# ssi-research/FQSS

Hardware: AMD Instinct MI355X
Metric: QAT-step samples/sec + SI-SDR, ConvTasNet 2spk 8kHz W8A8 (higher is better)
Workload: dtype f32; 1 GPU; ConvTasNet 2spk 8 kHz W8A8 QAT step (cfg 2), batch 8 x 4 s per GPU, quantizing phase; global_batch=8, segment_samples=32000, parallelism=dp1, optimizer=adam lr 1e-3 + clip 5.0

## Files before the change

fqss_amd/csrc/fqss_dev.h:

```cpp
#pragma once
#include <hip/hip_runtime.h>
#include <stdint.h>

#include "fqss.h"

namespace fqss {

void set_error(const char* fmt, ...);
int launch_status(const char* what);

#define FQSS_REQUIRE(cond, msg)                          \
    do {                                                 \
        if (!(cond)) {                                   \
            ::fqss::set_error("%s: %s", __func__, msg);  \
            return FQSS_EINVAL;                          \
        }                                                \
    } while (0)

static inline bool aligned16(const void* p) { return (reinterpret_cast<uintptr_t>(p) & 15u) == 0; }
static inline int64_t cdiv(int64_t a, int64_t b) { return (a + b - 1) / b; }

static inline dim3 grid_rows(int64_t rows, int64_t cols, int vec, int64_t max_blocks = 8192) {
    int64_t gx = cdiv(cols, 256 * (int64_t)vec);
    if (gx < 1) gx = 1;
    if (gx > 1024) gx = 1024;
    int64_t gy = max_blocks / gx;
    if (gy < 1) gy = 1;
    if (gy > rows) gy = rows;
    if (gy > 65535) gy = 65535;
    if (gy < 1) gy = 1;
    return dim3((unsigned)gx, (unsigned)gy, 1);
}

constexpr int kXcds = 8;
static inline unsigned xcd_grid(int64_t groups, int64_t per_group) { return (unsigned)(cdiv(groups, kXcds) * kXcds * per_group); }

bool qdgrad_ring_ok(int Ci, int Co1, int Co2);
int qdgrad_ring(const char* who, const float* gz1, const float* gz2, const int8_t* wiT, const float* dw, const float* addend, float* gx, int B,
                int Ci, int Co1, int Co2, int M, int64_t ld_gz1, int64_t ld_gz2, int64_t ld_add, int64_t ld_gx, fqss_stream_t stream);

#if defined(__HIPCC__)
__device__ __forceinline__ bool xcd_tile(int groups, int per_group, int& group, int& idx) {
    const int L = blockIdx.x, xcd = L % kXcds, slot = L / kXcds;
    idx = slot % per_group;
    group = (slot / per_group) * kXcds + xcd;
    return group < groups;
}

constexpr int kWave = 64;

__device__ __forceinline__ uint32_t f2ord(float f) {
    uint32_t u = __float_as_uint(f);
    return (u & 0x80000000u) ? ~u : (u | 0x80000000u);
}
__device__ __forceinline__ float ord2f(uint32_t k) {
    uint32_t u = (k & 0x80000000u) ? (k & 0x7fffffffu) : ~k;
    return __uint_as_float(u);
}

template <int CTRL, int ROW_MASK>
__device__ __forceinline__ int dpp_i32(int v) { return __builtin_amdgcn_update_dpp(0, v, CTRL, ROW_MASK, 0xf, false); }
template <int CTRL, int ROW_MASK = 0xf, typename T>
__device__ __forceinline__ T dpp_get(T v) {
    static_assert(sizeof(T) == 4 || sizeof(T) == 8, "32- or 64-bit values");
    if constexpr (sizeof(T) == 4) {
        return __builtin_bit_cast(T, dpp_i32<CTRL, ROW_MASK>(__builtin_bit_cast(int, v)));
    } else {
        const unsigned long long b = __builtin_bit_cast(unsigned long long, v);
        const unsigned lo = (unsigned)dpp_i32<CTRL, ROW_MASK>((int)(unsigned)b), hi = (unsigned)dpp_i32<CTRL, ROW_MASK>((int)(unsigned)(b >> 32));
        return __builtin_bit_cast(T, ((unsigned long long)hi << 32) | lo);
    }
}
template <typename T>
__device__ __forceinline__ T wave_sum63(T v) {
#ifdef FQSS_NO_DPP_SUMS
#pragma unroll
    for (int o = 32; o > 0; o >>= 1) v += __shfl_xor(v, o, 64);
    return v;
#else
    v += dpp_get<0xB1>(v);
    v += dpp_get<0x4E>(v);
    v += dpp_get<0x141>(v);
    v += dpp_get<0x140>(v);
    v += dpp_get<0x142, 0xa>(v);
    v += dpp_get<0x143, 0xc>(v);
    return v;
#endif
}

template <typename T>
__device__ __forceinline__ T from_lane63(T v) {
    static_assert(sizeof(T) == 4 || sizeof(T) == 8, "32- or 64-bit values");
    if constexpr (sizeof(T) == 4) {
        return __builtin_bit_cast(T, __builtin_amdgcn_readlane(__builtin_bit_cast(int, v), 63));
    } else {
        const unsigned long long b = __builtin_bit_cast(unsigned long long, v);
        const unsigned lo = (unsigned)__builtin_amdgcn_readlane((int)(unsigned)b, 63), hi = (unsigned)__builtin_amdgcn_readlane((int)(unsigned)(b >> 32), 63);
        return __builtin_bit_cast(T, ((unsigned long long)hi << 32) | lo);
    }
}
template <typename T>
__device__ __forceinline__ T wave_sum(T v) {
    return from_lane63(wave_sum63(v));
}
template <int CTRL, int ROW_MASK>
__device__ __forceinline__ float dpp_keep(float v) {
    const int i = __float_as_int(v);
    return __int_as_float(__builtin_amdgcn_update_dpp(i, i, CTRL, ROW_MASK, 0xf, false));
}
__device__ __forceinline__ float wave_min(float v) {
    v = fminf(v, dpp_get<0xB1>(v)); v = fminf(v, dpp_get<0x4E>(v)); v = fminf(v, dpp_get<0x141>(v)); v = fminf(v, dpp_get<0x140>(v));
    v = fminf(v, dpp_keep<0x142, 0xa>(v)); v = fminf(v, dpp_keep<0x143, 0xc>(v));
    return from_lane63(v);
}
__device__ __forceinline__ float wave_max(float v) {
    v = fmaxf(v, dpp_get<0xB1>(v)); v = fmaxf(v, dpp_get<0x4E>(v)); v = fmaxf(v, dpp_get<0x141>(v)); v = fmaxf(v, dpp_get<0x140>(v));
    v = fmaxf(v, dpp_keep<0x142, 0xa>(v)); v = fmaxf(v, dpp_keep<0x143, 0xc>(v));
    return from_lane63(v);
}
template <typename T>
__device__ __forceinline__ T row16_sum(T v) {
    v += dpp_get<0xB1>(v);
    v += dpp_get<0x4E>(v);
    v += dpp_get<0x141>(v);
    v += dpp_get<0x140>(v);
    return v;
}

template <typename T, int N>
__device__ __forceinline__ void block_sum(T (&v)[N], T* smem) {
    const int lane = threadIdx.x & 63, w = threadIdx.x >> 6, nw = blockDim.x >> 6;
#pragma unroll
    for (int i = 0; i < N; ++i) v[i] = wave_sum63(v[i]);
    if (lane == 63) {
#pragma unroll
        for (int i = 0; i < N; ++i) smem[i * nw + w] = v[i];
    }
    __syncthreads();
    if (threadIdx.x == 0) {
#pragma unroll
        for (int i = 0; i < N; ++i) {
            T s = smem[i * nw];
            for (int k = 1; k < nw; ++k) s += smem[i * nw + k];
            v[i] = s;
        }
    }
    __syncthreads();
}

template <int N>
__device__ __forceinline__ void block_sum_f32w(const float (&p)[N], float* smem, double (&out)[N]) {
    const int lane = threadIdx.x & 63, w = threadIdx.x >> 6, nw = blockDim.x >> 6;
#pragma unroll
    for (int i = 0; i < N; ++i) {
        const float s = wave_sum63(p[i]);
        if (lane == 63) smem[i * nw + w] = s;
    }
    __syncthreads();
    if (threadIdx.x == 0) {
#pragma unroll
        for (int i = 0; i < N; ++i) {
            double s = (double)smem[i * nw];
            for (int k = 1; k < nw; ++k) s += (double)smem[i * nw + k];
            out[i] = s;
        }
    }
    __syncthreads();
}

struct QRange {
    float lo, delta, inv;
};
__device__ __forceinline__ QRange load_qrange(const float* qmin, const float* qmax) {
    const float lo = *qmin, hi = *qmax;
    QRange r;
    r.lo = lo;
    r.delta = (hi - lo) / 255.0f;
    r.inv = 1.0f / r.delta;
    return r;
}
__device__ __forceinline__ float div_by(float a, float b, float y) {
    const float q = a * y;
    const float r = fmaf(-b, q, a);
    return fmaf(r, y, q);
}
__device__ __forceinline__ float wq_levels(int n_bits) { return (float)((1 << n_bits) - 1); }
__device__ __forceinline__ float wq_qlo(int n_bits) { return -(float)(1 << (n_bits - 1)); }
__device__ __forceinline__ float wq_qhi(int n_bits) { return (float)((1 << (n_bits - 1)) - 1); }
template <typename T>
__device__ __forceinline__ T sgpr(T v) {
    asm("" : "+s"(v));
    return v;
}
__device__ __forceinline__ void store16(float* p, const float4& v) {
    typedef float f32x4s __attribute__((ext_vector_type(4)));
    const f32x4s t = {v.x, v.y, v.z, v.w};
    asm volatile("global_store_dwordx4 %0, %1, off\n\ts_nop 1" : : "v"(p), "v"(t) : "memory");
}
__device__ __forceinline__ float act_neg_scale(int act, float slope) {
    return act == FQSS_ACT_PRELU ? slope : (act == FQSS_ACT_RELU ? 0.0f : 1.0f);
}
__device__ __forceinline__ float act_apply(float z, int act, float slope) {
// ... 83 lines not shown
```

fqss_amd/csrc/multi.hip:

```cpp
#include "fqss_dev.h"

namespace fqss {

constexpr int kSlotsM = FQSS_GACC_SLOTS;
constexpr int kWqFields = FQSS_WQ_DESC_WORDS;

__global__ __launch_bounds__(256) void k_gacc_flush_multi(const long long* __restrict__ table) {
    __shared__ double red[3 * 4];
    const long long* t = table + 4 * (int64_t)blockIdx.x;
    double* gacc = reinterpret_cast<double*>(t[0]);
    float* gmin = reinterpret_cast<float*>(t[1]);
    float* gmax = reinterpret_cast<float*>(t[2]);
    float* gslope = reinterpret_cast<float*>(t[3]);
    double v[3] = {0.0, 0.0, 0.0};
    for (int i = threadIdx.x; i < kSlotsM; i += 256) {
#pragma unroll
        for (int k = 0; k < 3; ++k) {
            const double x = gacc[3 * i + k];
            if (x != 0.0) {
                v[k] += x;
                gacc[3 * i + k] = 0.0;
            }
        }
    }
    block_sum<double, 3>(v, red);
    if (threadIdx.x == 0) {
        if (gmin) *gmin += (float)v[0];
        if (gmax) *gmax += (float)v[1];
        if (gslope) *gslope += (float)v[2];
    }
}

__device__ __forceinline__ const long long* find_desc(const long long* table, int n, int blk) {
    int lo = 0, hi = n - 1;
    while (lo < hi) {
        const int mid = (lo + hi + 1) >> 1;
        if ((int)table[(int64_t)mid * kWqFields + 15] <= blk) lo = mid; else hi = mid - 1;
    }
    return table + (int64_t)lo * kWqFields;
}

__global__ __launch_bounds__(256) void k_wq_multi_fwd(const long long* __restrict__ table, int n) {
    __shared__ float red[4];
    const long long* d = find_desc(table, n, blockIdx.x);
    const float* w = reinterpret_cast<const float*>(d[0]);
    float* wq = reinterpret_cast<float*>(d[1]);
    signed char* idx = reinterpret_cast<signed char*>(d[2]);
    signed char* idxT = reinterpret_cast<signed char*>(d[3]);
    float* dw = reinterpret_cast<float*>(d[4]);
    float* rw = reinterpret_cast<float*>(d[5]);
    const float* qmin = reinterpret_cast<const float*>(d[6]);
    const float* qmax = reinterpret_cast<const float*>(d[7]);
    const int outer = (int)d[12], C = (int)d[13], inner = (int)d[14];
    const int c = blockIdx.x - (int)d[15];
    const int64_t ldT = d[16];
    const int n_bits = (int)d[17];
    const float L = wq_levels(n_bits), qlo = wq_qlo(n_bits), qhi = wq_qhi(n_bits);
    const float a = fmaxf(fabsf(qmin[c]), fabsf(qmax[c]));
    const float delta = (2.0f * a) / L;
    const float inv = 1.0f / delta;
    float s = 0.0f;
    const int nel = outer * inner;
    for (int e = threadIdx.x; e < nel; e += 256) {
        const int o = e / inner, i = e - o * inner;
        const int64_t k = ((int64_t)o * C + c) * inner + i;
        const float X = rintf(div_by(w[k], delta, inv));
        const float q = __builtin_amdgcn_fmed3f(X, qlo, qhi);
        wq[k] = delta * q;
        if (idx) {
            idx[(int64_t)c * nel + e] = (signed char)q;
            idxT[(int64_t)e * ldT + c] = (signed char)q;
            s += q;
        }
    }
    if (idx) {
        float v[1] = {s};
        block_sum<float, 1>(v, red);
        if (threadIdx.x == 0) {
            dw[c] = delta;
            rw[c] = v[0];
        }
    }
}

__global__ __launch_bounds__(256) void k_wq_multi_bwd(const long long* __restrict__ table, int n) {
    __shared__ double red[4];
    const long long* d = find_desc(table, n, blockIdx.x);
    const float* w = reinterpret_cast<const float*>(d[0]);
    const float* qmin = reinterpret_cast<const float*>(d[6]);
    const float* qmax = reinterpret_cast<const float*>(d[7]);
    const float* gwq = reinterpret_cast<const float*>(d[8]);
    float* gw = reinterpret_cast<float*>(d[9]);
    float* gmin = reinterpret_cast<float*>(d[10]);
    float* gmax = reinterpret_cast<float*>(d[11]);
    const int outer = (int)d[12], C = (int)d[13], inner = (int)d[14];
    const int c = blockIdx.x - (int)d[15];
    const int n_bits = (int)d[17];
    const float L = wq_levels(n_bits), qlo = wq_qlo(n_bits), qhi = wq_qhi(n_bits);
    const float lo = qmin[c], hi = qmax[c];
    const float a = fmaxf(fabsf(lo), fabsf(hi));
    const float delta = (2.0f * a) / L;
    const float inv = 1.0f / delta;
    float p = 0.0f;
    const int nel = outer * inner;
    for (int e = threadIdx.x; e < nel; e += 256) {
        const int o = e / inner, i = e - o * inner;
        const int64_t k = ((int64_t)o * C + c) * inner + i;
        const float u = div_by(w[k], delta, inv);
        const float X = rintf(u);
        const bool inr = (X >= qlo) && (X <= qhi);
        const float q = __builtin_amdgcn_fmed3f(X, qlo, qhi);
        const float gk = gwq[k];
        gw[k] += inr ? div_by(gk * delta, delta, inv) : 0.0f;
        p += gk * (inr ? (q - u) : q);
    }
    double v[1] = {(double)p};
    block_sum<double, 1>(v, red);
    if (threadIdx.x == 0) {
        const double D = v[0] * (2.0 / (double)L);
        const float al = fabsf(lo), ah = fabsf(hi);
        const double wl = al > ah ? 1.0 : (al == ah ? 0.5 : 0.0);
        const double wh = ah > al ? 1.0 : (al == ah ? 0.5 : 0.0);
        const double sl = lo > 0.0f ? 1.0 : (lo < 0.0f ? -1.0 : 0.0);
        const double sh = hi > 0.0f ? 1.0 : (hi < 0.0f ? -1.0 : 0.0);
        gmin[c] += (float)(D * wl * sl);
        gmax[c] += (float)(D * wh * sh);
    }
}

}

using namespace fqss;

extern "C" int fqss_gacc_flush_multi(const int64_t* table, int n, fqss_stream_t stream) {
    FQSS_REQUIRE(table && n >= 0, "bad args");
    if (n == 0) return FQSS_OK;
    hipLaunchKernelGGL(k_gacc_flush_multi, dim3((unsigned)n), dim3(256), 0, (hipStream_t)stream, (const long long*)table);
    return launch_status("fqss_gacc_flush_multi");
}

extern "C" int fqss_wq_table_check(const int64_t* host_table, int n) {
    FQSS_REQUIRE(n >= 0 && (host_table || n == 0), "bad args");
    for (int i = 0; i < n; ++i) {
        const int64_t* d = host_table + (int64_t)i * kWqFields;
        FQSS_REQUIRE(d[17] >= FQSS_WQ_MIN_BITS && d[17] <= FQSS_WQ_MAX_BITS, "descriptor word 17: weight width outside 2..8 bits");
        FQSS_REQUIRE(d[12] > 0 && d[13] > 0 && d[14] > 0, "descriptor words 12-14: empty weight");
    }
    return FQSS_OK;
}

extern "C" int fqss_wq_multi_fwd(const int64_t* table, int n, int total_channels, fqss_stream_t stream) {
    FQSS_REQUIRE(table && n >= 0 && total_channels >= 0, "bad args");
    if (n == 0 || total_channels == 0) return FQSS_OK;
    hipLaunchKernelGGL(k_wq_multi_fwd, dim3((unsigned)total_channels), dim3(256), 0, (hipStream_t)stream,
                       (const long long*)table, n);
    return launch_status("fqss_wq_multi_fwd");
}

extern "C" int fqss_wq_multi_bwd(const int64_t* table, int n, int total_channels, fqss_stream_t stream) {
    FQSS_REQUIRE(table && n >= 0 && total_channels >= 0, "bad args");
    if (n == 0 || total_channels == 0) return FQSS_OK;
    hipLaunchKernelGGL(k_wq_multi_bwd, dim3((unsigned)total_channels), dim3(256), 0, (hipStream_t)stream,
                       (const long long*)table, n);
    return launch_status("fqss_wq_multi_bwd");
}
```

fqss_amd/csrc/qgemm.hip:

```cpp
#include <cstdlib>
#include <type_traits>

#define FQSS_USES_GRAD_ADD
#include "fqss_dev.h"

namespace fqss {

typedef float f32x16 __attribute__((ext_vector_type(16)));
typedef __bf16 bf16x8 __attribute__((ext_vector_type(8)));
typedef short s16x4 __attribute__((ext_vector_type(4)));
typedef short s16x8 __attribute__((ext_vector_type(8)));

constexpr int QBM = 128, QBN = 64, QBK = 32;
constexpr int LDK = 40;
constexpr int LDN = 96;
constexpr int LDT = 36;
constexpr int WGRAD_BLOCKS = 256;

__device__ __forceinline__ unsigned short f2bf_trunc(float f) { return (unsigned short)(__float_as_uint(f) >> 16); }
__device__ __forceinline__ float bf_trunc(float f) { return __uint_as_float(__float_as_uint(f) & 0xFFFF0000u); }
__device__ __forceinline__ unsigned int bf_rne_word(float f) {
    const unsigned int u = __float_as_uint(f);
    return u + 0x7FFFu + ((u >> 16) & 1u);
}

__device__ __forceinline__ void split3(float g, unsigned short& b1, unsigned short& b2, unsigned short& b3) {
    const float h1 = bf_trunc(g);
    const float r1 = g - h1;
    const float h2 = bf_trunc(r1);
    const float r2 = r1 - h2;
    b1 = f2bf_trunc(h1);
    b2 = f2bf_trunc(h2);
    b3 = f2bf_trunc(r2);
}

typedef float f32x4 __attribute__((ext_vector_type(4)));
typedef uint32_t u32x4 __attribute__((ext_vector_type(4)));
typedef uint32_t u32x2 __attribute__((ext_vector_type(2)));
struct QStage {
    f32x4 a[4];
    f32x4 b[2];
    u32x2 bq;
    int kch;
};
__device__ __forceinline__ void q_load16(f32x4& d, const void* p) { asm volatile("global_load_dwordx4 %0, %1, off" : "=v"(d) : "v"(p) : "memory"); }
__device__ __forceinline__ void q_load8(u32x2& d, const void* p) { asm volatile("global_load_dwordx2 %0, %1, off" : "=v"(d) : "v"(p) : "memory"); }
template <int MODE, int N>
__device__ __forceinline__ void q_wait(QStage& st) {
    if constexpr (MODE == 0)
        asm volatile("s_waitcnt vmcnt(%2)" : "+v"(st.a[0]), "+v"(st.bq) : "n"(N) : "memory");
    else if constexpr (MODE == 1)
        asm volatile("s_waitcnt vmcnt(%3)" : "+v"(st.a[0]), "+v"(st.b[0]), "+v"(st.b[1]) : "n"(N) : "memory");
    else
        asm volatile("s_waitcnt vmcnt(%6)"
                     : "+v"(st.a[0]), "+v"(st.a[1]), "+v"(st.a[2]), "+v"(st.a[3]), "+v"(st.b[0]), "+v"(st.b[1])
                     : "n"(N)
                     : "memory");
}

__device__ __forceinline__ float dec(unsigned int c, const QRange& r) { return r.delta * (float)c + r.lo; }

struct QGemmArgs {
    const void* A;
    const void* B;
    float* C;
    int M, N, K;
    int64_t lda, ldb, ldc;
    int64_t sAb, sBb, sCb;
    const float* dw;
    const float* rw;
    const float* bias;
    const float* qmin_x;
    const float* qmax_x;
    int ksplit, kchunk;
    int tiles_m, tiles_n, batches;
    int M1;
    float* C2; int64_t ldc2, sC2b;
    const float* bias2;
    const void* A2; int64_t lda2, sA2b;
    int K1;
    const void* B2; int64_t ldb2, sB2b;
    unsigned char* Q1; unsigned char* Q2; int64_t ldq1, ldq2, sQ1b, sQ2b;
    const float *qy_min1, *qy_max1, *qy_min2, *qy_max2;
    int qact; const float* qslope;
    long long* stats;
    const unsigned char* AD1; const unsigned char* AD2; int64_t ldad1, ldad2;
    unsigned char* S1; unsigned char* S2; int64_t lds1, lds2;
    const float *ad_min1, *ad_max1, *ad_min2, *ad_max2;
    const float *s_min1, *s_max1, *s_min2, *s_max2;
    int imp_taps, imp_kw, imp_base, imp_row_step, imp_col_step, imp_cmax;
    float imp_inv_taps, imp_inv_kw;
};

template <int MODE, int GP = 3, bool IMP = false>
__global__ __launch_bounds__(256, 2) void k_qgemm(QGemmArgs g) {
    static_assert(!IMP || MODE == 1 || MODE == 3 || MODE == 4, "implicit convolution: float B operands");
    static_assert(MODE == 0 || MODE == 1 || MODE == 3 || MODE == 4, "unknown q-GEMM mode");
    static_assert(GP == 3 || (GP == 2 && MODE != 0 && MODE != 4), "two gradient pieces: dgrad only");
    constexpr bool ACODES = MODE < 2 || MODE == 4;
    constexpr int WMODE = MODE == 4 ? 1 : MODE;
    constexpr bool SIX = MODE == 3 && GP == 2;
    constexpr int NA = (MODE == 3) ? 3 : 1;
    constexpr int NB = (MODE == 1) ? GP : (MODE == 3 || MODE == 4) ? 3 : 1;
    constexpr int BROWS = QBK, BLD = LDN;
    constexpr int A_BYTES = NA * QBM * LDK * 2, B_BYTES = NB * BROWS * BLD * 2;
    constexpr int T_BYTES = 4 * 32 * LDT * 4;
    constexpr int SMEM = (A_BYTES + B_BYTES > T_BYTES) ? A_BYTES + B_BYTES : T_BYTES;
    __shared__ __attribute__((aligned(16))) unsigned char smem[SMEM];
    typedef unsigned short (*AsT)[QBM][LDK];
    typedef unsigned short (*BsT)[BROWS][BLD];
    AsT As = reinterpret_cast<AsT>(smem);
    BsT Bs = reinterpret_cast<BsT>(smem + A_BYTES);

    const int tid = threadIdx.x, lane = tid & 63;
    const int wave = __builtin_amdgcn_readfirstlane(tid >> 6);
    const int wm = wave >> 1, wn = wave & 1;
    const int lr = lane & 31, lh = lane >> 5;
    int panel, mt;
    if (!xcd_tile(g.tiles_n * g.batches, g.tiles_m, panel, mt)) return;
    const int b = panel / g.tiles_n;
    const int kbeg = 0, kend = g.K;
    const int i0 = mt * QBM, j0 = (panel % g.tiles_n) * QBN;

    f32x16 acc[2];
#pragma unroll
    for (int mi = 0; mi < 2; ++mi)
#pragma unroll
        for (int r = 0; r < 16; ++r) acc[mi][r] = 0.f;

    __shared__ float rowc[3][QBM];
    if constexpr (MODE == 0 || MODE == 3 || MODE == 4) {
        if (tid < QBM) {
            const int row = i0 + tid;
            const bool ok = row < g.M;
            rowc[0][tid] = ((MODE == 0 || MODE == 4) && ok) ? g.dw[row] : 1.0f;
            rowc[1][tid] = (MODE == 0 && ok) ? g.rw[row] : 0.0f;
            rowc[2][tid] = (ok && g.bias != nullptr) ? (row < g.M1 ? g.bias[row] : g.bias2[row - g.M1]) : 0.0f;
        }
    }

    constexpr int NLOADS = (MODE == 0) ? 2 : (WMODE == 1) ? 3 : 6;
    const int a_row = tid >> 1, a_k = (tid & 1) * 16;
    const int bk_row = tid >> 3, bk_n = (tid & 7) * 8;
    const int a_row_c = min(i0 + a_row, g.M - 1);

    __shared__ float dws[(MODE == 1) ? 1024 : 1];
    if constexpr (MODE == 1) {
        for (int k = tid; k < (IMP ? g.K / g.imp_taps : g.K); k += 256) dws[k] = g.dw[k];
    }

    constexpr int BEL = (MODE == 0) ? 1 : 4;
    const char* const gB1 = sgpr((const char*)g.B + (int64_t)b * g.sBb * BEL);
    const char* const gB2 = (MODE == 0) ? gB1 : sgpr((const char*)g.B2 + (int64_t)b * g.sB2b * BEL);
    const int64_t gldb1 = sgpr(g.ldb), gldb2 = (MODE == 0) ? gldb1 : sgpr(g.ldb2);
    auto load_tiles = [&](QStage& st, int k0) {
        if constexpr (ACODES) {
            q_load16(st.a[0], (const signed char*)g.A + (int64_t)a_row_c * g.lda + min(k0 + a_k, g.K - 16));
        } else {
            const float* A = (const float*)g.A + (int64_t)b * g.sAb + (int64_t)a_row_c * g.lda;
#pragma unroll
            for (int q = 0; q < 4; ++q) q_load16(st.a[q], A + min(k0 + a_k + 4 * q, g.K - 4));
        }
        const int kk = min(k0 + bk_row, g.K - 1);
        if constexpr (IMP) {
            int ci = (int)((float)kk * g.imp_inv_taps);
            int t = kk - ci * g.imp_taps;
            if (t < 0) { ci -= 1; t += g.imp_taps; }
            if (t >= g.imp_taps) { ci += 1; t -= g.imp_taps; }
            int th = (int)((float)t * g.imp_inv_kw);
            int tw = t - th * g.imp_kw;
            if (tw < 0) { th -= 1; tw += g.imp_kw; }
            if (tw >= g.imp_kw) { th += 1; tw -= g.imp_kw; }
            st.kch = ci;
            const float* Bp = (const float*)gB1 + (int64_t)ci * gldb1 + (g.imp_base + th * g.imp_row_step + tw * g.imp_col_step);
            const int c0 = min(j0 + bk_n, g.imp_cmax);
            q_load16(st.b[0], Bp + c0);
            q_load16(st.b[1], Bp + c0 + 4);
        } else if constexpr (MODE == 0) {
            const unsigned char* Bp = (const unsigned char*)gB1 + (int64_t)kk * gldb1;
            q_load8(st.bq, Bp + min(j0 + bk_n, (int)gldb1 - 8));
        } else {
            const bool h1 = kk < g.K1;
            const int ldk = (int)(h1 ? gldb1 : gldb2);
            const float* Bp = (const float*)(h1 ? gB1 : gB2) + (int64_t)(h1 ? kk : kk - g.K1) * ldk;
            q_load16(st.b[0], Bp + min(j0 + bk_n, ldk - 4));
            q_load16(st.b[1], Bp + min(j0 + bk_n + 4, ldk - 4));
        }
    };

    auto store_codes = [&](unsigned short* dst, const unsigned int* w, auto nw_tag, bool is_signed, bool zero) {
        constexpr int NW = decltype(nw_tag)::value;
        unsigned int o[2 * NW];
#pragma unroll
        for (int q = 0; q < NW; ++q) {
            float f[4];
#pragma unroll
            for (int e = 0; e < 4; ++e) {
                const unsigned int byte = (w[q] >> (8 * e)) & 0xFFu;
                f[e] = zero ? 0.0f : (is_signed ? (float)(int)(signed char)byte : (float)byte);
            }
            o[2 * q] = __builtin_amdgcn_perm(__float_as_uint(f[1]), __float_as_uint(f[0]), 0x07060302u);
            o[2 * q + 1] = __builtin_amdgcn_perm(__float_as_uint(f[3]), __float_as_uint(f[2]), 0x07060302u);
        }
#pragma unroll
        for (int h = 0; h < NW / 2; ++h)
            *reinterpret_cast<uint4*>(dst + 8 * h) = make_uint4(o[4 * h], o[4 * h + 1], o[4 * h + 2], o[4 * h + 3]);
    };

    auto store_split3 = [&](unsigned short* d1, unsigned short* d2, unsigned short* d3, const f32x4* v, float scale,
                            bool do_scale, bool zero, auto nq_tag) {
        constexpr int NQ = decltype(nq_tag)::value;
        unsigned int o1[2 * NQ], o2[2 * NQ], o3[2 * NQ];
#pragma unroll
        for (int q = 0; q < NQ; ++q) {
            float h0[4], r1[4], r2[4];
#pragma unroll
            for (int e = 0; e < 4; ++e) {
                float t = do_scale ? scale * v[q][e] : v[q][e];
                if (zero) t = 0.0f;
                h0[e] = t;
                r1[e] = t - bf_trunc(t);
                r2[e] = r1[e] - bf_trunc(r1[e]);
            }
#pragma unroll
            for (int e = 0; e < 2; ++e) {
                o1[2 * q + e] = __builtin_amdgcn_perm(__float_as_uint(h0[2 * e + 1]), __float_as_uint(h0[2 * e]), 0x07060302u);
                o2[2 * q + e] = __builtin_amdgcn_perm(__float_as_uint(r1[2 * e + 1]), __float_as_uint(r1[2 * e]), 0x07060302u);
                o3[2 * q + e] = __builtin_amdgcn_perm(__float_as_uint(r2[2 * e + 1]), __float_as_uint(r2[2 * e]), 0x07060302u);
            }
        }
#pragma unroll
        for (int h = 0; h < NQ / 2; ++h) {
            *reinterpret_cast<uint4*>(d1 + 8 * h) = make_uint4(o1[4 * h], o1[4 * h + 1], o1[4 * h + 2], o1[4 * h + 3]);
            *reinterpret_cast<uint4*>(d2 + 8 * h) = make_uint4(o2[4 * h], o2[4 * h + 1], o2[4 * h + 2], o2[4 * h + 3]);
            *reinterpret_cast<uint4*>(d3 + 8 * h) = make_uint4(o3[4 * h], o3[4 * h + 1], o3[4 * h + 2], o3[4 * h + 3]);
        }
    };

    auto store_split2 = [&](unsigned short* d1, unsigned short* d2, const f32x4* v, float scale, bool zero) {
        unsigned int o1[4], o2[4];
#pragma unroll
        for (int q = 0; q < 2; ++q) {
            float h0[4];
            unsigned int r1[4];
#pragma unroll
            for (int e = 0; e < 4; ++e) {
                float t = scale * v[q][e];
                if (zero) t = 0.0f;
                h0[e] = t;
                r1[e] = bf_rne_word(t - bf_trunc(t));
            }
#pragma unroll
            for (int e = 0; e < 2; ++e) {
                o1[2 * q + e] = __builtin_amdgcn_perm(__float_as_uint(h0[2 * e + 1]), __float_as_uint(h0[2 * e]), 0x07060302u);
                o2[2 * q + e] = __builtin_amdgcn_perm(r1[2 * e + 1], r1[2 * e], 0x07060302u);
            }
        }
        *reinterpret_cast<uint4*>(d1) = make_uint4(o1[0], o1[1], o1[2], o1[3]);
        *reinterpret_cast<uint4*>(d2) = make_uint4(o2[0], o2[1], o2[2], o2[3]);
    };

    auto store_tiles = [&](QStage& st, int k0) {
        q_wait<WMODE, NLOADS>(st);
        const bool kz = (k0 + bk_row) >= g.K;
        if constexpr (ACODES) {
            const unsigned int w[4] = {__float_as_uint(st.a[0][0]), __float_as_uint(st.a[0][1]), __float_as_uint(st.a[0][2]),
                                       __float_as_uint(st.a[0][3])};
            store_codes(&As[0][a_row][a_k], w, std::integral_constant<int, 4>{}, true, false);
        } else {
            store_split3(&As[0][a_row][a_k], &As[1][a_row][a_k], &As[2][a_row][a_k], st.a, 1.0f, false, false,
                         std::integral_constant<int, 4>{});
        }
        if constexpr (MODE == 0) {
            const unsigned int w[2] = {st.bq[0], st.bq[1]};
            store_codes(&Bs[0][bk_row][bk_n], w, std::integral_constant<int, 2>{}, false, kz);
        } else {
            const float sc = (MODE == 1) ? dws[IMP ? st.kch : min(k0 + bk_row, g.K - 1)] : 1.0f;
            if constexpr (NB == 2)
                store_split2(&Bs[0][bk_row][bk_n], &Bs[1][bk_row][bk_n], st.b, sc, kz);
            else
                store_split3(&Bs[0][bk_row][bk_n], &Bs[1][bk_row][bk_n], &Bs[2][bk_row][bk_n], st.b, sc, MODE == 1, kz,
                             std::integral_constant<int, 2>{});
        }
    };

    const int nkt = (kend - kbeg + QBK - 1) / QBK;
    const int gq = lane >> 4, li = lane & 15, tq = li >> 2, tp = li & 3;
    auto compute_tile = [&]() {
#pragma unroll
        for (int ks = 0; ks < 2; ++ks) {
#pragma unroll
            for (int sp = 0; sp < NA * NB; ++sp) {
                const int ia = (NA == 3) ? 2 - (sp / NB) : 0, ib = (NB > 1) ? NB - 1 - (sp % NB) : 0;
                if (SIX && ia + ib >= 3) continue;
                bf16x8 af[2], bfr;
#pragma unroll
                for (int mi = 0; mi < 2; ++mi)
                    af[mi] = *reinterpret_cast<const bf16x8*>(&As[ia][wm * 64 + mi * 32 + lr][ks * 16 + 8 * lh]);
                {
                    const int kr = ks * 16 + 8 * (gq >> 1) + tq;
                    const int nc = wn * 32 + 16 * (gq & 1) + 4 * tp;
                    union { bf16x8 v; s16x4 h[2]; } u;
                    u.h[0] = __builtin_amdgcn_ds_read_tr16_b64_v4i16(
                        (s16x4 __attribute__((address_space(3)))*)(&Bs[ib][kr][nc]));
                    u.h[1] = __builtin_amdgcn_ds_read_tr16_b64_v4i16(
                        (s16x4 __attribute__((address_space(3)))*)(&Bs[ib][kr + 4][nc]));
                    bfr = u.v;
                }
#pragma unroll
                for (int mi = 0; mi < 2; ++mi)
                    acc[mi] = __builtin_amdgcn_mfma_f32_32x32x16_bf16(af[mi], bfr, acc[mi], 0, 0, 0);
            }
        }
    };
    QStage stA, stB;
    __syncthreads();
    load_tiles(stA, 0);
    load_tiles(stB, QBK);
    store_tiles(stA, 0);
    load_tiles(stA, 2 * QBK);
    __syncthreads();
    for (int kt = 0; kt < nkt; kt += 2) {
        compute_tile();
        __syncthreads();
        if (kt + 1 < nkt) {
            store_tiles(stB, (kt + 1) * QBK);
            load_tiles(stB, (kt + 3) * QBK);
            __syncthreads();
            compute_tile();
            __syncthreads();
            if (kt + 2 < nkt) {
                store_tiles(stA, (kt + 2) * QBK);
                load_tiles(stA, (kt + 4) * QBK);
                __syncthreads();
            }
        }
    }
    q_wait<WMODE, 0>(stA);
    q_wait<WMODE, 0>(stB);

    float dx = 0.f, mnx = 0.f;
    if constexpr (MODE == 0) {
        const float lo = *g.qmin_x, hi = *g.qmax_x;
        dx = (hi - lo) / 255.0f;
        mnx = lo;
    }
    float* Cb = g.C + (int64_t)b * g.sCb;
    float* C2b = (g.C2 != nullptr) ? g.C2 + (int64_t)b * g.sC2b : nullptr;
    __shared__ uint32_t Qt[(MODE == 0) ? 4 : 1][32][8];
    const bool quant = (MODE == 0) && g.Q1 != nullptr;
    unsigned int st_s = 0, st_ss = 0;
    QRange ry1{}, ry2{};
    QRange rad1{}, rad2{}, rs1{}, rs2{};
    float qslope = 0.0f;
    if (quant) {
        ry1 = load_qrange(g.qy_min1, g.qy_max1);
        ry2 = (g.Q2 != nullptr) ? load_qrange(g.qy_min2, g.qy_max2) : ry1;
        qslope = (g.qact == FQSS_ACT_PRELU) ? *g.qslope : 0.0f;
        if (g.S1 != nullptr) { rad1 = load_qrange(g.ad_min1, g.ad_max1); rs1 = load_qrange(g.s_min1, g.s_max1); }
        if (g.S2 != nullptr) { rad2 = load_qrange(g.ad_min2, g.ad_max2); rs2 = load_qrange(g.s_min2, g.s_max2); }
    }
    {
        __syncthreads();
        float(*Tt)[LDT] = reinterpret_cast<float(*)[LDT]>(smem + wave * 32 * LDT * 4);
        const bool has_bias = g.bias != nullptr;
        const float qns = act_neg_scale(g.qact, qslope);
        const int c4 = (lane & 7) * 4;
        const int col = j0 + wn * 32 + c4;
        auto tile_epilogue = [&](int mi, auto PER_ROW) {
            const int rowt = i0 + wm * 64 + mi * 32;
            const bool tfirst = rowt < g.M1;
            uint4 ad16 = make_uint4(0u, 0u, 0u, 0u);
            const unsigned char* const adp = (MODE == 0 && quant) ? (tfirst ? g.AD1 : g.AD2) : nullptr;
            if constexpr (MODE == 0) {
                if (adp != nullptr) {
                    const int64_t ldad = tfirst ? g.ldad1 : g.ldad2;
                    const int orow = rowt + (lane >> 1) - (tfirst ? 0 : g.M1), ocol = j0 + wn * 32 + 16 * (lane & 1);
                    const int rows_o = tfirst ? g.M1 : g.M - g.M1;
                    if (rowt + (lane >> 1) < g.M && ocol < ldad)
                        ad16 = *reinterpret_cast<const uint4*>(adp + ((int64_t)b * rows_o + orow) * ldad + ocol);
                }
            }
#pragma unroll
            for (int r = 0; r < 16; ++r) {
                const int rl = (r & 3) + 8 * (r >> 2) + 4 * lh;
                const int rb = wm * 64 + mi * 32 + rl;
                const float S = acc[mi][r];
                float v = S;
                if constexpr (MODE == 0) {
                    v = rowc[0][rb] * (dx * S + mnx * rowc[1][rb]);
                    if (has_bias) v = v + rowc[2][rb];
                } else if constexpr (MODE == 3) {
                    if (has_bias) v = S + rowc[2][rb];
                } else if constexpr (MODE == 4) {
                    v = rowc[0][rb] * S;
                    if (has_bias) v = v + rowc[2][rb];
                }
                Tt[rl][lr] = v;
            }
            const QRange ry = tfirst ? ry1 : ry2;
#pragma unroll
            for (int pass = 0; pass < 4; ++pass) {
                const int rl = pass * 8 + (lane >> 3);
                const int row = rowt + rl;
                float4 t = *reinterpret_cast<const float4*>(&Tt[rl][c4]);
                if constexpr (MODE == 1) {
                    if (C2b != nullptr && row < g.M && col < g.N) {
                        const float4 r = *reinterpret_cast<const float4*>(C2b + (int64_t)row * g.ldc2 + col);
                        t.x += r.x; t.y += r.y; t.z += r.z; t.w += r.w;
                    }
                }
                if (row < g.M && col < g.N) {
                    const bool first = decltype(PER_ROW)::value ? row < g.M1 : tfirst;
                    const int64_t ldc = first ? g.ldc : g.ldc2;
                    float* dst = (first ? Cb + (int64_t)row * ldc : C2b + (int64_t)(row - g.M1) * ldc) + col;
                    if (col + 3 < g.N || col + 3 < ldc) {
                        store16(dst, t);
                    } else {
                        dst[0] = t.x;
                        if (col + 1 < g.N) dst[1] = t.y;
                        if (col + 2 < g.N) dst[2] = t.z;
                    }
                }
                if constexpr (MODE == 0) {
                    if (quant) {
                        const float tv[4] = {t.x, t.y, t.z, t.w};
                        uint32_t pk = 0;
#pragma unroll
                        for (int e = 0; e < 4; ++e) pk = pack_code(fq_code(tv[e] > 0.0f ? tv[e] : qns * tv[e], ry), e, pk);
                        Qt[wave][rl][lane & 7] = pk;
                        if (g.stats != nullptr) {
                            const int nl = g.N - col;
                            const uint32_t live = (row < g.M && nl > 0) ? (nl >= 4 ? 0xFFFFFFFFu : (0xFFFFFFFFu >> (8 * (4 - nl)))) : 0u;
                            code_stats4(pk & live, st_s, st_ss);
                        }
                    }
                }
            }
            if constexpr (MODE == 0) {
                if (quant) {
                    const int rl = lane >> 1, hf = lane & 1;
                    const int qcol = j0 + wn * 32 + 16 * hf;
                    const uint4 c16 = *reinterpret_cast<const uint4*>(&Qt[wave][rl][4 * hf]);
                    const int64_t ldq = tfirst ? g.ldq1 : g.ldq2;
                    if (rowt + rl < g.M && qcol < ldq) {
                        unsigned char* qb = tfirst ? g.Q1 + (int64_t)b * g.sQ1b + (int64_t)(rowt + rl) * ldq
                                                   : g.Q2 + (int64_t)b * g.sQ2b + (int64_t)(rowt + rl - g.M1) * ldq;
                        *reinterpret_cast<uint4*>(qb + qcol) = c16;
                    }
                    if (adp != nullptr) {
                        const QRange ra = tfirst ? rad1 : rad2, rs = tfirst ? rs1 : rs2;
                        const unsigned int wa[4] = {ad16.x, ad16.y, ad16.z, ad16.w}, wy[4] = {c16.x, c16.y, c16.z, c16.w};
                        unsigned int o[4];
#pragma unroll
                        for (int w4 = 0; w4 < 4; ++w4) {
                            unsigned int pk = 0;
#pragma unroll
                            for (int e = 0; e < 4; ++e) {
                                float z = dec((wa[w4] >> (8 * e)) & 255u, ra);
                                z = z + 1.0f * dec((wy[w4] >> (8 * e)) & 255u, ry);
                                pk = pack_code(fq_code(z, rs), e, pk);
                            }
                            o[w4] = pk;
                        }
                        const int64_t lds_ = tfirst ? g.lds1 : g.lds2;
                        const int rows_o = tfirst ? g.M1 : g.M - g.M1;
                        if (rowt + rl < g.M && qcol < lds_) {
                            unsigned char* sb_ = (tfirst ? g.S1 : g.S2) + ((int64_t)b * rows_o + (rowt + rl - (tfirst ? 0 : g.M1))) * lds_;
                            *reinterpret_cast<uint4*>(sb_ + qcol) = make_uint4(o[0], o[1], o[2], o[3]);
                        }
                    }
                }
            }
        };
        if (MODE != 0 || (g.M1 & 31) == 0 || g.M1 >= g.M) {
#pragma unroll
            for (int mi = 0; mi < 2; ++mi) tile_epilogue(mi, std::false_type{});
        } else {
#pragma unroll
            for (int mi = 0; mi < 2; ++mi) tile_epilogue(mi, std::true_type{});
        }
        if constexpr (MODE == 0) {
            if (quant && g.stats != nullptr) {
                __shared__ unsigned int sst[2][4];
                st_s = wave_sum(st_s);
                st_ss = wave_sum(st_ss);
                if (lane == 0) { sst[0][wave] = st_s; sst[1][wave] = st_ss; }
                __syncthreads();
                if (tid == 0) {
                    long long* slot = g.stats + 2 * (((int64_t)b * g.tiles_m + mt) * g.tiles_n + (panel % g.tiles_n));
                    slot[0] = (long long)sst[0][0] + sst[0][1] + sst[0][2] + sst[0][3];
                    slot[1] = (long long)sst[1][0] + sst[1][1] + sst[1][2] + sst[1][3];
// ... 281 lines not shown
                const uint32_t w = st.b[f][q];
                const float f0 = (float)(w & 0xFFu), f1 = (float)((w >> 8) & 0xFFu);
                const float f2 = (float)((w >> 16) & 0xFFu), f3 = (float)(w >> 24);
                o[2 * q] = __builtin_amdgcn_perm(__float_as_uint(f1), __float_as_uint(f0), 0x07060302u);
                o[2 * q + 1] = __builtin_amdgcn_perm(__float_as_uint(f3), __float_as_uint(f2), 0x07060302u);
            }
            *reinterpret_cast<uint4*>(&Bs[buf][br + 128 * f][bc]) = make_uint4(o[0], o[1], o[2], o[3]);
            *reinterpret_cast<uint4*>(&Bs[buf][br + 128 * f][bc + 8]) = make_uint4(o[4], o[5], o[6], o[7]);
        }
        ++cr;
        ck += W2_TK;
        if (ck >= spb * W2_TK) ck = 0;
    };
    f32x16 acc[NBF];
#pragma unroll
    for (int f = 0; f < NBF; ++f)
#pragma unroll
        for (int r = 0; r < 16; ++r) acc[f][r] = 0.f;
    auto compute = [&](int buf) {
#pragma unroll
        for (int ks = 0; ks < W2_TK / 16; ++ks) {
            const int kk = ks * 16 + 8 * lh;
            bf16x8 bfr[NBF];
#pragma unroll
            for (int f = 0; f < NBF; ++f) bfr[f] = *reinterpret_cast<const bf16x8*>(&Bs[buf][wc * (32 * NBF) + 32 * f + lr][kk]);
            bf16x8 af[GP];
#pragma unroll
            for (int p = 0; p < GP; ++p) af[p] = *reinterpret_cast<const bf16x8*>(&As[buf][p][wr * 32 + lr][kk]);
#pragma unroll
            for (int p = GP - 1; p >= 0; --p)
#pragma unroll
                for (int f = 0; f < NBF; ++f) acc[f] = __builtin_amdgcn_mfma_f32_32x32x16_bf16(af[p], bfr[f], acc[f], 0, 0, 0);
        }
    };
    Stage st[W2_RING];
#pragma unroll
    for (int i = 0; i < W2_RING; ++i) load(st[i]);
    wait_oldest(st[0]);
    convert_store(st[0], 0);
    load(st[0]);
    __syncthreads();
    for (int s = 0; s < n; s += W2_RING) {
#pragma unroll
        for (int i = 0; i < W2_RING; ++i) {
            Stage& nx = st[(i + 1) % W2_RING];
            if (first_half) compute(i & 1);
            wait_oldest(nx);
            convert_store(nx, (i + 1) & 1);
            load(nx);
            if (!first_half) compute(i & 1);
            __syncthreads();
        }
    }
#pragma unroll
    for (int i = 0; i < W2_RING; ++i) wait_all(st[i]);
#pragma unroll
    for (int i = 0; i < 2; ++i) {
        float v = rs_part[i];
#pragma unroll
        for (int o = 8; o > 0; o >>= 1) v += __shfl_xor(v, o, 64);
        if ((tid & 15) == 0) rsum[ar + 32 * i] = v;
    }
    __syncthreads();
    const float lo = *J.qmin, hi = *J.qmax;
    const float dx = (hi - lo) / 255.0f, mnx = lo;
    constexpr int NV = 16 * NBF;
    float v[NV];
#pragma unroll
    for (int f = 0; f < NBF; ++f)
#pragma unroll
        for (int r = 0; r < 16; ++r) v[16 * f + r] = dx * acc[f][r] + mnx * rsum[wr * 32 + (r & 3) + 8 * (r >> 2) + 4 * lh];
    bool finish = nparts == 1;
    constexpr int SLOT = W2_TM * TN;
    if (!finish) {
        float* sl = ga.slabs + ((int64_t)(J.tile0 + tile) * ga.slots + part) * WGR_SLOT_FLOATS;
#pragma unroll
        for (int q = 0; q < NV / 4; ++q) st16_sc1(sl + ((int64_t)q * 512 + tid) * 4, f32x4{v[4 * q], v[4 * q + 1], v[4 * q + 2], v[4 * q + 3]});
        asm volatile("s_waitcnt vmcnt(0)" ::: "memory");
        __syncthreads();
        if (tid == 0) *ticket_s = __hip_atomic_fetch_add(&ga.tickets[J.tile0 + tile], 1u, __ATOMIC_RELAXED, __HIP_MEMORY_SCOPE_AGENT);
        __syncthreads();
        finish = *ticket_s == (unsigned)(nparts - 1);
        if (finish) {
            const float* s0p = ga.slabs + (int64_t)(J.tile0 + tile) * ga.slots * WGR_SLOT_FLOATS;
#pragma unroll
            for (int r = 0; r < NV; ++r) v[r] = 0.0f;
            for (int p = 0; p < nparts; ++p) {
#pragma unroll
                for (int h = 0; h < NBF; ++h) {
                    f32x4 t[4];
#pragma unroll
                    for (int q = 0; q < 4; ++q) ld16_sc1(t[q], s0p + (int64_t)p * WGR_SLOT_FLOATS + ((int64_t)(4 * h + q) * 512 + tid) * 4);
                    asm volatile("s_waitcnt vmcnt(0)" : "+v"(t[0]), "+v"(t[1]), "+v"(t[2]), "+v"(t[3]) : : "memory");
#pragma unroll
                    for (int q = 0; q < 4; ++q)
#pragma unroll
                        for (int e = 0; e < 4; ++e) v[16 * h + 4 * q + e] += t[q][e];
                }
            }
            if (tid == 0) __hip_atomic_store(&ga.tickets[J.tile0 + tile], 0u, __ATOMIC_RELAXED, __HIP_MEMORY_SCOPE_AGENT);
        }
    }
    static_assert(SLOT <= WGR_SLOT_FLOATS, "slab slots are sized for the wide tile");
    if (finish) {
        const int Mr = J.M, Nc = J.N;
        float* const Cp = J.C;
        float old[NV];
#pragma unroll
        for (int f = 0; f < NBF; ++f)
#pragma unroll
            for (int r = 0; r < 16; ++r) {
                const int row = row0 + wr * 32 + (r & 3) + 8 * (r >> 2) + 4 * lh, col = col0 + wc * (32 * NBF) + 32 * f + lr;
                old[16 * f + r] = (row < Mr && col < Nc) ? Cp[(int64_t)row * Nc + col] : 0.0f;
            }
#pragma unroll
        for (int f = 0; f < NBF; ++f)
#pragma unroll
            for (int r = 0; r < 16; ++r) {
                const int row = row0 + wr * 32 + (r & 3) + 8 * (r >> 2) + 4 * lh, col = col0 + wc * (32 * NBF) + 32 * f + lr;
                if (row < Mr && col < Nc) Cp[(int64_t)row * Nc + col] = old[16 * f + r] + v[16 * f + r];
            }
        asm volatile("s_waitcnt vmcnt(0)" ::: "memory");
    }
    __syncthreads();
}

template <int GP>
__global__ __launch_bounds__(512, 1) void k_qwgrad_group(WGroupArgs ga) {
    __shared__ __attribute__((aligned(16))) unsigned short As_raw[2 * GP * W2_TM * W2_LD];
    __shared__ __attribute__((aligned(16))) unsigned short Bs_raw[2 * 256 * W2_LD];
    __shared__ float rsum[W2_TM];
    __shared__ unsigned ticket_s;
    const int L = blockIdx.x, xcd = L % kXcds, slot = L / kXcds;
    const int team = (slot / WGR_TEAM) * kXcds + xcd, member = slot % WGR_TEAM;
    int u0 = team * ga.chunk;
    const int u1 = min(ga.total, u0 + ga.chunk);
    while (u0 < u1) {
        int jn = 0;
        for (int q = 1; q < ga.njobs; ++q) jn = (ga.j[q].ubeg <= u0) ? q : jn;
        const WJob& J = ga.j[jn];
        const int rel = u0 - J.ubeg, grp = rel / J.nstages, s0 = rel - grp * J.nstages;
        const int n = min(J.nstages - s0, u1 - u0);
        const int g0 = J.ubeg + grp * J.nstages;
        const int t_first = g0 / ga.chunk, nparts = (g0 + J.nstages - 1) / ga.chunk - t_first + 1, part = team - t_first;
        u0 += n;
        const int tile = grp * WGR_TEAM + member;
        if (tile >= J.ntiles) continue;
        if (J.wide) wgr_segment<GP, true>(ga, J, tile, s0, n, nparts, part, As_raw, Bs_raw, rsum, &ticket_s);
        else wgr_segment<GP, false>(ga, J, tile, s0, n, nparts, part, As_raw, Bs_raw, rsum, &ticket_s);
    }
}

__global__ __launch_bounds__(256) void k_wq_codes(const float* __restrict__ w, signed char* __restrict__ idx,
                                                   signed char* __restrict__ idxT, float* dw, float* rw, int Co, int Ci,
                                                   const float* __restrict__ qmin, const float* __restrict__ qmax, int n_bits) {
    __shared__ float red[4];
    const int co = blockIdx.x;
    const float L = wq_levels(n_bits), qlo = wq_qlo(n_bits), qhi = wq_qhi(n_bits);
    const float a = fmaxf(fabsf(qmin[co]), fabsf(qmax[co]));
    const float delta = (2.0f * a) / L;
    float s = 0.0f;
    for (int ci = threadIdx.x; ci < Ci; ci += 256) {
        const float X = rintf(w[(int64_t)co * Ci + ci] / delta);
        const float q = fminf(fmaxf(X, qlo), qhi);
        idx[(int64_t)co * Ci + ci] = (signed char)q;
        idxT[(int64_t)ci * Co + co] = (signed char)q;
        s += q;
    }
    float v[1] = {s};
    block_sum<float, 1>(v, red);
    if (threadIdx.x == 0) {
        dw[co] = delta;
        rw[co] = v[0];
    }
}

}

using namespace fqss;

static int grad_pieces() {
    const char* e = getenv("FQSS_GRAD_PIECES");
    return (e != nullptr && e[0] == '2') ? 2 : 3;
}

extern "C" int fqss_wq_codes_bits(const float* w, int8_t* idx, int8_t* idxT, float* dw, float* rw, int Co, int Ci,
                                  const float* qmin, const float* qmax, int n_bits, fqss_stream_t stream) {
    FQSS_REQUIRE(w && idx && idxT && dw && rw && qmin && qmax && Co > 0 && Ci > 0, "bad args");
    FQSS_REQUIRE(n_bits >= FQSS_WQ_MIN_BITS && n_bits <= FQSS_WQ_MAX_BITS, "weight width outside 2..8 bits");
    hipLaunchKernelGGL(k_wq_codes, dim3((unsigned)Co), dim3(256), 0, (hipStream_t)stream, w, (signed char*)idx,
                       (signed char*)idxT, dw, rw, Co, Ci, qmin, qmax, n_bits);
    return launch_status("fqss_wq_codes_bits");
}

extern "C" int fqss_wq_codes(const float* w, int8_t* idx, int8_t* idxT, float* dw, float* rw, int Co, int Ci,
                             const float* qmin, const float* qmax, fqss_stream_t stream) {
    return fqss_wq_codes_bits(w, idx, idxT, dw, rw, Co, Ci, qmin, qmax, 8, stream);
}

struct QpwQuant {
    int act; const float* slope; const float *min1, *max1, *min2, *max2; uint8_t *yc1, *yc2; int64_t ld1, ld2;
    long long* stats;
    const FqssAddAfter *add1, *add2;
};

static int qpw_fwd_impl(const char* who, const uint8_t* xc, const int8_t* wi, const float* dw, const float* rw, const float* bias1,
                        const float* bias2, const float* qmin_x, const float* qmax_x, float* z1, float* z2, int B, int Ci, int Co1,
                        int Co2, int M, int64_t ld_xc, int64_t ld_z1, int64_t ld_z2, fqss_stream_t stream,
                        const QpwQuant* qq = nullptr) {
    if (B == 0 || M == 0) return FQSS_OK;
    const int Co = Co1 + Co2;
    FQSS_REQUIRE(xc && wi && dw && rw && qmin_x && qmax_x && z1 && (Co2 == 0 || z2), "null tensor");
    FQSS_REQUIRE(B >= 0 && Ci > 0 && Co1 > 0 && Co2 >= 0 && M >= 0 && ld_xc >= M && ld_z1 >= M && (Co2 == 0 || ld_z2 >= M), "bad shape");
    FQSS_REQUIRE(Ci % 16 == 0 && Ci <= 512 && ld_xc % 16 == 0 && aligned16(xc) && aligned16(wi),
                 "q-GEMM needs Ci % 16 == 0, Ci <= 512 (exact fp32 integer sum) and 16-B aligned code rows");
    FQSS_REQUIRE(aligned16(z1) && ld_z1 % 4 == 0 && (Co2 == 0 || (aligned16(z2) && ld_z2 % 4 == 0)), "output rows must be 16-B aligned");
    FQSS_REQUIRE((bias1 == nullptr) == (bias2 == nullptr) || Co2 == 0, "paired layers: both or neither with bias");
    if (qq != nullptr) FQSS_REQUIRE(Co2 == 0 || Co1 % 32 == 0, "fused quantizer of a pair needs Co1 % 32 == 0");
    QGemmArgs g{};
    g.A = wi; g.B = xc; g.C = z1; g.M = Co; g.N = M; g.K = Ci;
    g.lda = Ci; g.ldb = ld_xc; g.ldc = ld_z1;
    g.sAb = 0; g.sBb = (int64_t)Ci * ld_xc; g.sCb = (int64_t)Co1 * ld_z1;
    g.M1 = Co1; g.C2 = z2; g.ldc2 = ld_z2; g.sC2b = (int64_t)Co2 * ld_z2; g.bias2 = bias2; g.K1 = Ci;
    g.dw = dw; g.rw = rw; g.bias = bias1; g.qmin_x = qmin_x; g.qmax_x = qmax_x; g.ksplit = 1; g.kchunk = Ci;
    if (qq != nullptr) {
        FQSS_REQUIRE(qq->min1 && qq->max1 && qq->yc1 && (Co2 == 0 || (qq->min2 && qq->max2 && qq->yc2)), "fused quantizer: null pointer");
        FQSS_REQUIRE(qq->ld1 % 16 == 0 && qq->ld1 >= M && aligned16(qq->yc1) && (Co2 == 0 || (qq->ld2 % 16 == 0 && qq->ld2 >= M && aligned16(qq->yc2))),
                     "output code rows must be 16-B aligned");
        FQSS_REQUIRE(qq->act != FQSS_ACT_PRELU || qq->slope, "PReLU needs a slope");
        g.Q1 = qq->yc1; g.Q2 = qq->yc2; g.ldq1 = qq->ld1; g.ldq2 = qq->ld2;
        g.sQ1b = (int64_t)Co1 * qq->ld1; g.sQ2b = (int64_t)Co2 * qq->ld2;
        g.qy_min1 = qq->min1; g.qy_max1 = qq->max1; g.qy_min2 = qq->min2; g.qy_max2 = qq->max2;
        g.qact = qq->act; g.qslope = qq->slope;
        FQSS_REQUIRE(!qq->stats || Co2 == 0, "output statistics: single-output launches only");
        g.stats = qq->stats;
        const FqssAddAfter* ad[2] = {qq->add1, qq->add2};
        for (int i = 0; i < 2; ++i) {
            const FqssAddAfter* a = ad[i];
            if (a == nullptr) continue;
            FQSS_REQUIRE(i == 0 || Co2 > 0, "fused AddQ behind a second output that does not exist");
            FQSS_REQUIRE(qq->act == FQSS_ACT_NONE, "fused AddQ: the conv in front of it has no activation (Conv1dQ)");
            FQSS_REQUIRE(a->a && a->y && a->amin && a->amax && a->qmin && a->qmax, "fused AddQ: null pointer");
            FQSS_REQUIRE(a->ld_a % 16 == 0 && a->ld_a >= M && a->ld_y % 16 == 0 && a->ld_y >= M && aligned16(a->a) && aligned16(a->y),
                         "fused AddQ: code rows must be 16-B aligned");
            if (i == 0) {
                g.AD1 = a->a; g.ldad1 = a->ld_a; g.S1 = a->y; g.lds1 = a->ld_y;
                g.ad_min1 = a->amin; g.ad_max1 = a->amax; g.s_min1 = a->qmin; g.s_max1 = a->qmax;
            } else {
                g.AD2 = a->a; g.ldad2 = a->ld_a; g.S2 = a->y; g.lds2 = a->ld_y;
                g.ad_min2 = a->amin; g.ad_max2 = a->amax; g.s_min2 = a->qmin; g.s_max2 = a->qmax;
            }
        }
    }
    g.tiles_n = (int)cdiv(M, QBN); g.tiles_m = (int)cdiv(Co, QBM); g.batches = B;
    hipLaunchKernelGGL((k_qgemm<0>), dim3(xcd_grid((int64_t)g.tiles_n * B, g.tiles_m)), dim3(256), 0, (hipStream_t)stream, g);
    return launch_status(who);
}

extern "C" int fqss_qpw_fwd(const uint8_t* xc, const int8_t* wi, const float* dw, const float* rw, const float* bias,
                            const float* qmin_x, const float* qmax_x, float* z, int B, int Ci, int Co, int M,
                            int64_t ld_xc, int64_t ld_z, fqss_stream_t stream) {
    return qpw_fwd_impl("fqss_qpw_fwd", xc, wi, dw, rw, bias, nullptr, qmin_x, qmax_x, z, nullptr, B, Ci, Co, 0, M, ld_xc, ld_z, 0, stream);
}

extern "C" int fqss_qpw_fwd2(const uint8_t* xc, const int8_t* wi, const float* dw, const float* rw, const float* bias1,
                             const float* bias2, const float* qmin_x, const float* qmax_x, float* z1, float* z2, int B, int Ci,
                             int Co1, int Co2, int M, int64_t ld_xc, int64_t ld_z1, int64_t ld_z2, fqss_stream_t stream) {
    FQSS_REQUIRE(Co2 > 0, "second layer missing");
    return qpw_fwd_impl("fqss_qpw_fwd2", xc, wi, dw, rw, bias1, bias2, qmin_x, qmax_x, z1, z2, B, Ci, Co1, Co2, M, ld_xc, ld_z1, ld_z2, stream);
}

extern "C" int fqss_qpw_fwdq(const uint8_t* xc, const int8_t* wi, const float* dw, const float* rw, const float* bias1,
                             const float* bias2, const float* qmin_x, const float* qmax_x, float* z1, float* z2, int act,
                             const float* slope, const float* qmin1, const float* qmax1, const float* qmin2, const float* qmax2,
                             uint8_t* yc1, uint8_t* yc2, int B, int Ci, int Co1, int Co2, int M, int64_t ld_xc, int64_t ld_z1,
                             int64_t ld_z2, int64_t ld_yc1, int64_t ld_yc2, int64_t* stats1, fqss_stream_t stream) {
    QpwQuant qq{act, slope, qmin1, qmax1, qmin2, qmax2, yc1, yc2, ld_yc1, ld_yc2, (long long*)stats1, nullptr, nullptr};
    return qpw_fwd_impl("fqss_qpw_fwdq", xc, wi, dw, rw, bias1, bias2, qmin_x, qmax_x, z1, z2, B, Ci, Co1, Co2, M, ld_xc, ld_z1, ld_z2,
                        stream, &qq);
}

extern "C" int fqss_qpw_fwdq_add(const uint8_t* xc, const int8_t* wi, const float* dw, const float* rw, const float* bias1,
                                 const float* bias2, const float* qmin_x, const float* qmax_x, float* z1, float* z2, const float* qmin1,
                                 const float* qmax1, const float* qmin2, const float* qmax2, uint8_t* yc1, uint8_t* yc2, int B, int Ci,
                                 int Co1, int Co2, int M, int64_t ld_xc, int64_t ld_z1, int64_t ld_z2, int64_t ld_yc1, int64_t ld_yc2,
                                 const FqssAddAfter* add1, const FqssAddAfter* add2, fqss_stream_t stream) {
    QpwQuant qq{FQSS_ACT_NONE, nullptr, qmin1, qmax1, qmin2, qmax2, yc1, yc2, ld_yc1, ld_yc2, nullptr, add1, add2};
    return qpw_fwd_impl("fqss_qpw_fwdq_add", xc, wi, dw, rw, bias1, bias2, qmin_x, qmax_x, z1, z2, B, Ci, Co1, Co2, M, ld_xc, ld_z1,
                        ld_z2, stream, &qq);
}

static int qpw_bwd_x_impl(const char* who, const float* gz1, const float* gz2, const int8_t* wiT, const float* dw, float* gx, int B,
                          int Ci, int Co1, int Co2, int M, int64_t ld_gz1, int64_t ld_gz2, int64_t ld_gx, fqss_stream_t stream,
                          const float* addend = nullptr, int64_t ld_add = 0) {
    if (B == 0 || M == 0) return FQSS_OK;
    const int Co = Co1 + Co2;
    FQSS_REQUIRE(gz1 && wiT && dw && gx && (Co2 == 0 || gz2), "null tensor");
    FQSS_REQUIRE(B >= 0 && Ci > 0 && Co1 > 0 && Co2 >= 0 && M >= 0 && ld_gz1 >= M && ld_gx >= M, "bad shape");
    FQSS_REQUIRE(Co1 % 16 == 0 && Co2 % 16 == 0 && ld_gz1 % 4 == 0 && aligned16(gz1) && aligned16(wiT) && ld_gz1 >= ((M + 3) & ~3),
                 "q-GEMM dgrad needs Co % 16 == 0 and 16-B aligned gradient rows");
    FQSS_REQUIRE(Co2 == 0 || (ld_gz2 % 4 == 0 && aligned16(gz2) && ld_gz2 >= ((M + 3) & ~3)), "second gradient: 16-B aligned rows");
    FQSS_REQUIRE(aligned16(gx) && ld_gx % 4 == 0, "output rows must be 16-B aligned");
    FQSS_REQUIRE(Co <= 1024, "dgrad stages delta_w of at most 1024 output channels in LDS");
    if (B == 0 || M == 0) return FQSS_OK;
    QGemmArgs g{};
    g.A = wiT; g.B = gz1; g.C = gx; g.M = Ci; g.N = M; g.K = Co;
    g.lda = Co; g.ldb = ld_gz1; g.ldc = ld_gx;
    g.sAb = 0; g.sBb = (int64_t)Co1 * ld_gz1; g.sCb = (int64_t)Ci * ld_gx;
    g.M1 = Ci; g.K1 = Co1; g.B2 = gz2; g.ldb2 = ld_gz2; g.sB2b = (int64_t)Co2 * ld_gz2;
    g.dw = dw; g.ksplit = 1; g.kchunk = Co;
    if (addend != nullptr) {
        FQSS_REQUIRE(aligned16(addend) && ld_add % 4 == 0 && ld_add >= ((M + 3) & ~3), "addend rows must be 16-B aligned and padded to 4");
        g.C2 = const_cast<float*>(addend); g.ldc2 = ld_add; g.sC2b = (int64_t)Ci * ld_add;
    }
    g.tiles_n = (int)cdiv(M, QBN); g.tiles_m = (int)cdiv(Ci, QBM); g.batches = B;
    if (grad_pieces() == 3)
        hipLaunchKernelGGL((k_qgemm<1, 3>), dim3(xcd_grid((int64_t)g.tiles_n * B, g.tiles_m)), dim3(256), 0, (hipStream_t)stream, g);
    else
        hipLaunchKernelGGL((k_qgemm<1, 2>), dim3(xcd_grid((int64_t)g.tiles_n * B, g.tiles_m)), dim3(256), 0, (hipStream_t)stream, g);
    return launch_status(who);
}

extern "C" int fqss_qpw_bwd_x(const float* gz, const int8_t* wiT, const float* dw, float* gx, int B, int Ci, int Co,
                              int M, int64_t ld_gz, int64_t ld_gx, fqss_stream_t stream) {
    return qpw_bwd_x_impl("fqss_qpw_bwd_x", gz, nullptr, wiT, dw, gx, B, Ci, Co, 0, M, ld_gz, 0, ld_gx, stream);
}

extern "C" int fqss_qpw_bwd_x_add(const float* gz, const int8_t* wiT, const float* dw, const float* addend, float* gx, int B, int Ci, int Co,
                                  int M, int64_t ld_gz, int64_t ld_add, int64_t ld_gx, fqss_stream_t stream) {
    FQSS_REQUIRE(addend, "null addend");
    return qpw_bwd_x_impl("fqss_qpw_bwd_x_add", gz, nullptr, wiT, dw, gx, B, Ci, Co, 0, M, ld_gz, 0, ld_gx, stream, addend, ld_add);
}

extern "C" int fqss_qpw_bwd_x2(const float* gz1, const float* gz2, const int8_t* wiT, const float* dw, float* gx, int B, int Ci,
                               int Co1, int Co2, int M, int64_t ld_gz1, int64_t ld_gz2, int64_t ld_gx, fqss_stream_t stream) {
    FQSS_REQUIRE(Co2 > 0, "second layer missing");
    return qpw_bwd_x_impl("fqss_qpw_bwd_x2", gz1, gz2, wiT, dw, gx, B, Ci, Co1, Co2, M, ld_gz1, ld_gz2, ld_gx, stream);
}

static int qpw_bwd_w_impl(const char* who, const float* gz1, const float* gz2, const uint8_t* xc, const float* qmin_x,
                          const float* qmax_x, float* gw, int B, int Ci, int Co1, int Co2, int M, int64_t ld_gz1, int64_t ld_gz2,
                          int64_t ld_xc, fqss_stream_t stream) {
    if (B == 0 || M == 0) return FQSS_OK;
    const int Co = Co1 + Co2;
    FQSS_REQUIRE(gz1 && xc && qmin_x && qmax_x && gw && (Co2 == 0 || gz2), "null tensor");
    FQSS_REQUIRE(B >= 0 && Ci > 0 && Co1 > 0 && Co2 >= 0 && M >= 0 && ld_gz1 >= M && ld_xc >= M, "bad shape");
    FQSS_REQUIRE(ld_gz1 % 4 == 0 && ld_xc % 16 == 0 && aligned16(gz1) && aligned16(xc) && ld_gz1 >= ((M + 3) & ~3),
                 "q-GEMM wgrad needs 16-B aligned gradient and code rows");
    FQSS_REQUIRE(Co2 == 0 || (ld_gz2 % 4 == 0 && aligned16(gz2) && ld_gz2 >= ((M + 3) & ~3)), "second gradient: 16-B aligned rows");
    if (B == 0 || M == 0) return FQSS_OK;
    QGemmArgs g{};
    g.A = gz1; g.B = xc; g.C = gw; g.M = Co; g.N = Ci; g.K = M;
    g.lda = ld_gz1; g.ldb = ld_xc; g.ldc = Ci;
    g.sAb = (int64_t)Co1 * ld_gz1; g.sBb = (int64_t)Ci * ld_xc; g.sCb = 0;
    g.M1 = Co1; g.A2 = gz2; g.lda2 = ld_gz2; g.sA2b = (int64_t)Co2 * ld_gz2; g.K1 = M;
    g.qmin_x = qmin_x; g.qmax_x = qmax_x;
    const int64_t tiles = cdiv(Co, 64) * cdiv(Ci, 128) * B;
    int want = (int)((WGRAD_BLOCKS + tiles / 2) / tiles);
    if (want < 1) want = 1;
    g.tiles_n = (int)cdiv(Ci, 128); g.tiles_m = (int)cdiv(Co, 64); g.batches = B;
    const int kchunk = (int)cdiv(cdiv(M, want), W2_RING * W2_TK) * W2_RING * W2_TK;
    g.kchunk = kchunk;
    g.ksplit = (int)cdiv(M, kchunk);
    if (grad_pieces() == 3)
        hipLaunchKernelGGL(k_qwgrad2<3>, dim3(xcd_grid((int64_t)B * g.ksplit, (int64_t)g.tiles_m * g.tiles_n)), dim3(512), 0, (hipStream_t)stream, g);
    else
        hipLaunchKernelGGL(k_qwgrad2<2>, dim3(xcd_grid((int64_t)B * g.ksplit, (int64_t)g.tiles_m * g.tiles_n)), dim3(512), 0, (hipStream_t)stream, g);
    return launch_status(who);
}

extern "C" int fqss_qpw_bwd_w(const float* gz, const uint8_t* xc, const float* qmin_x, const float* qmax_x, float* gw,
                              int B, int Ci, int Co, int M, int64_t ld_gz, int64_t ld_xc, fqss_stream_t stream) {
    return qpw_bwd_w_impl("fqss_qpw_bwd_w", gz, nullptr, xc, qmin_x, qmax_x, gw, B, Ci, Co, 0, M, ld_gz, 0, ld_xc, stream);
}

extern "C" int fqss_qpw_bwd_w2(const float* gz1, const float* gz2, const uint8_t* xc, const float* qmin_x, const float* qmax_x,
                               float* gw, int B, int Ci, int Co1, int Co2, int M, int64_t ld_gz1, int64_t ld_gz2, int64_t ld_xc,
                               fqss_stream_t stream) {
    FQSS_REQUIRE(Co2 > 0, "second layer missing");
    return qpw_bwd_w_impl("fqss_qpw_bwd_w2", gz1, gz2, xc, qmin_x, qmax_x, gw, B, Ci, Co1, Co2, M, ld_gz1, ld_gz2, ld_xc, stream);
}

constexpr int64_t WGR_TICKET_BYTES = 65536;
static int wgr_plan(const FqssWgradJob* jobs, int n0, int n, WGroupArgs& ga, int64_t& slab_bytes) {
    int u = 0, t = 0, max_st = 0;
    ga.njobs = n;
    for (int q = 0; q < n; ++q) {
        const FqssWgradJob& f = jobs[n0 + q];
        WJob& J = ga.j[q];
        const int Co = f.Co1 + f.Co2;
        J.A = f.gz1; J.A2 = f.gz2; J.Bc = f.xc; J.C = f.gw; J.qmin = f.qmin_x; J.qmax = f.qmax_x;
        J.lda = f.ld_gz1; J.lda2 = f.ld_gz2; J.ldb = f.ld_xc;
        J.sAb = (int64_t)f.Co1 * f.ld_gz1; J.sA2b = (int64_t)f.Co2 * f.ld_gz2; J.sBb = (int64_t)f.Ci * f.ld_xc;
        J.M = Co; J.M1 = f.Co1; J.N = f.Ci; J.K = f.M;
        static const bool no_wide = getenv("FQSS_WGRAD_WIDE") != nullptr && getenv("FQSS_WGRAD_WIDE")[0] == '0';
        J.wide = (f.Ci >= 256 && !no_wide) ? 1 : 0;
        J.tiles_n = (int)cdiv(f.Ci, J.wide ? 256 : W2_TN);
        J.ntiles = (int)cdiv(Co, W2_TM) * J.tiles_n;
        J.spb = (int)cdiv(f.M, W2_TK);
        J.nstages = f.B * J.spb;
        J.ubeg = u; J.tile0 = t;
        u += (int)cdiv(J.ntiles, WGR_TEAM) * J.nstages;
        t += J.ntiles;
        if (J.nstages > max_st) max_st = J.nstages;
    }
    ga.total = u;
    ga.chunk = (int)cdiv(u, WGR_TEAMS);
    ga.slots = (max_st - 1) / ga.chunk + 2;
    slab_bytes = (int64_t)t * ga.slots * WGR_SLOT_FLOATS * 4;
    return t;
}
static int wgr_check(const FqssWgradJob* jobs, int njobs) {
    FQSS_REQUIRE(jobs && njobs > 0, "no jobs");
    for (int q = 0; q < njobs; ++q) {
        const FqssWgradJob& f = jobs[q];
        FQSS_REQUIRE(f.gz1 && f.xc && f.qmin_x && f.qmax_x && f.gw && (f.Co2 == 0 || f.gz2), "null tensor");
        FQSS_REQUIRE(f.B > 0 && f.Ci > 0 && f.Co1 > 0 && f.Co2 >= 0 && f.M > 0 && f.ld_gz1 >= f.M && f.ld_xc >= f.M, "bad shape");
        FQSS_REQUIRE(f.ld_gz1 % 4 == 0 && f.ld_xc % 16 == 0 && aligned16(f.gz1) && aligned16(f.xc) && f.ld_gz1 >= ((f.M + 3) & ~3),
                     "q-GEMM wgrad needs 16-B aligned gradient and code rows");
        FQSS_REQUIRE(f.Co2 == 0 || (f.ld_gz2 % 4 == 0 && aligned16(f.gz2) && f.ld_gz2 >= ((f.M + 3) & ~3)), "second gradient: 16-B aligned rows");
        FQSS_REQUIRE((int64_t)f.B * cdiv(f.M, W2_TK) * cdiv(cdiv(f.Co1 + f.Co2, W2_TM) * cdiv(f.Ci, W2_TN), WGR_TEAM) < (1ll << 26), "job too large");
        for (int p = 0; p < q; ++p) FQSS_REQUIRE(jobs[p].gw != f.gw, "two jobs of one call accumulate into the same gw (plain read-modify-write)");
    }
    return FQSS_OK;
}

extern "C" int64_t fqss_qpw_bwd_w_group_ws(const FqssWgradJob* jobs, int njobs) {
    if (wgr_check(jobs, njobs) != FQSS_OK) return -1;
    int64_t need = 0;
    const int per = (int)cdiv(njobs, cdiv(njobs, WGR_MAXJOBS));
    for (int n0 = 0; n0 < njobs; n0 += per) {
        WGroupArgs ga{};
        int64_t sb = 0;
        const int t = wgr_plan(jobs, n0, njobs - n0 < per ? njobs - n0 : per, ga, sb);
        if ((int64_t)t * 4 > WGR_TICKET_BYTES) { set_error("fqss_qpw_bwd_w_group_ws: more than 16384 tiles in one launch"); return -1; }
        if (sb > need) need = sb;
    }
    return WGR_TICKET_BYTES + need;
}

extern "C" int fqss_qpw_bwd_w_group(const FqssWgradJob* jobs, int njobs, void* ws, int64_t ws_bytes, fqss_stream_t stream) {
    if (njobs == 0) return FQSS_OK;
    if (int rc = wgr_check(jobs, njobs)) return rc;
    FQSS_REQUIRE(ws && aligned16(ws), "workspace: 16-B aligned device memory (fqss_qpw_bwd_w_group_ws bytes, zero-filled when first used)");
    const int per = (int)cdiv(njobs, cdiv(njobs, WGR_MAXJOBS));
    for (int n0 = 0; n0 < njobs; n0 += per) {
        WGroupArgs ga{};
        int64_t sb = 0;
        const int t = wgr_plan(jobs, n0, njobs - n0 < per ? njobs - n0 : per, ga, sb);
        FQSS_REQUIRE((int64_t)t * 4 <= WGR_TICKET_BYTES && WGR_TICKET_BYTES + sb <= ws_bytes, "workspace too small (fqss_qpw_bwd_w_group_ws)");
        ga.tickets = (unsigned*)ws;
        ga.slabs = (float*)((char*)ws + WGR_TICKET_BYTES);
        if (grad_pieces() == 3)
            hipLaunchKernelGGL(k_qwgrad_group<3>, dim3(WGR_TEAMS * WGR_TEAM), dim3(512), 0, (hipStream_t)stream, ga);
        else
            hipLaunchKernelGGL(k_qwgrad_group<2>, dim3(WGR_TEAMS * WGR_TEAM), dim3(512), 0, (hipStream_t)stream, ga);
        if (int rc = launch_status("fqss_qpw_bwd_w_group")) return rc;
    }
    return FQSS_OK;
}

static int pwconv_fwd_x3_impl(const char* who, bool six, const float* x, const float* w, const float* bias, float* z, int B, int Ci, int Co,
                              int M, int64_t ld_x, int64_t ld_z, fqss_stream_t stream) {
    if (B == 0 || M == 0) return FQSS_OK;
    FQSS_REQUIRE(x && w && z, "null tensor");
    FQSS_REQUIRE(B >= 0 && Ci > 0 && Co > 0 && M >= 0 && ld_x >= M && ld_z >= M, "bad shape");
    FQSS_REQUIRE(Ci % 4 == 0 && ld_x % 4 == 0 && aligned16(x) && aligned16(w) && ld_x >= ((M + 3) & ~3),
                 "x3 GEMM needs Ci % 4 == 0 and 16-B aligned activation rows");
    FQSS_REQUIRE(aligned16(z) && ld_z % 4 == 0, "output rows must be 16-B aligned");
    if (B == 0 || M == 0) return FQSS_OK;
    QGemmArgs g{};
    g.A = w; g.B = x; g.C = z; g.M = Co; g.N = M; g.K = Ci;
    g.lda = Ci; g.ldb = ld_x; g.ldc = ld_z;
    g.sAb = 0; g.sBb = (int64_t)Ci * ld_x; g.sCb = (int64_t)Co * ld_z;
    g.bias = bias; g.ksplit = 1; g.kchunk = Ci; g.M1 = Co; g.K1 = Ci;
    g.tiles_n = (int)cdiv(M, QBN); g.tiles_m = (int)cdiv(Co, QBM); g.batches = B;
    if (six) hipLaunchKernelGGL((k_qgemm<3, 2>), dim3(xcd_grid((int64_t)g.tiles_n * B, g.tiles_m)), dim3(256), 0, (hipStream_t)stream, g);
    else hipLaunchKernelGGL((k_qgemm<3>), dim3(xcd_grid((int64_t)g.tiles_n * B, g.tiles_m)), dim3(256), 0, (hipStream_t)stream, g);
    return launch_status(who);
}

extern "C" int fqss_pwconv_fwd_wq(const float* x, const int8_t* wi, const float* dw, const float* bias, float* z, int B, int Ci, int Co, int M,
                                  int64_t ld_x, int64_t ld_z, fqss_stream_t stream) {
    if (B == 0 || M == 0) return FQSS_OK;
    FQSS_REQUIRE(x && wi && dw && z, "null tensor");
    FQSS_REQUIRE(B >= 0 && Ci >= 16 && Co > 0 && M >= 0 && ld_x >= M && ld_z >= M, "bad shape");
    FQSS_REQUIRE(Ci % 16 == 0 && ld_x % 4 == 0 && aligned16(x) && aligned16(wi) && ld_x >= ((M + 3) & ~3),
                 "coded-weight forward needs Ci % 16 == 0 and 16-B aligned activation rows");
    FQSS_REQUIRE(aligned16(z) && ld_z % 4 == 0, "output rows must be 16-B aligned");
    QGemmArgs g{};
// ... 74 lines not shown
```

fqss_amd/kernels.py:

```python
import torch

from . import _lib


def _h(*names):
    return tuple(_lib.CONSTANTS["FQSS_" + n] for n in names)


Q_BYPASS, Q_OBSERVE, Q_QUANT = _h("Q_BYPASS", "Q_OBSERVE", "Q_QUANT")
ACT_NONE, ACT_PRELU, ACT_RELU = _h("ACT_NONE", "ACT_PRELU", "ACT_RELU")
ACT_GELU, ACT_POST_RELU = _h("ACT_GELU", "ACT_POST_RELU")

GACC_DOUBLES = _h("GACC_SLOTS")[0] * 3
WQ_DESC_WORDS, = _h("WQ_DESC_WORDS")
WQ_BITS = _h("WQ_MIN_BITS", "WQ_MAX_BITS")
USE_X3 = True
LD_ALIGN = 16


def _p(t):
    return None if t is None else t.data_ptr()


import ctypes as _C
# ... 101 lines not shown
    return rm is not None and rm[2] % 4 == 0 and t.data_ptr() % 16 == 0 and t.dtype == torch.float32


def as_rowmat(t):
    rm = rowmat(t)
    if rm is None:
        c = empty_act(tuple(t.shape), t.device)
        c.copy_(t)
        t, rm = c, rowmat(c)
    return (t,) + rm


def empty_codes(shape, device):
    M = shape[-1]
    ld = (M + 15) // 16 * 16
    buf = torch.empty(*shape[:-1], ld, device=device, dtype=torch.uint8)
    return buf[..., :M] if ld != M else buf


def actq_fwd(z, act, slope, qmode, qmin, qmax, obs_ws, want_idx=False, dense_idx=False, write_out=True):
    _need_gpu(z, slope, qmin, qmax)
    rc = _rowmat_collapsed(z) if (z.dim() >= 3 and rowmat(z) is None) else None
    skip_out = (not write_out) and want_idx and qmode == Q_QUANT
    if rc is not None:
        rows, cols, ld_z = rc
        out = torch.empty(z.shape, device=z.device, dtype=torch.float32)
        ld_o = ld_i = cols
        idx = torch.empty(z.shape, device=z.device, dtype=torch.uint8) if want_idx else None
    else:
        z, rows, cols, ld_z = as_rowmat(z)
        out = empty_act(tuple(z.shape), z.device)
        _, _, _, ld_o = (out,) + rowmat(out)
        idx, ld_i = None, cols
        if want_idx:
            idx = torch.empty(z.shape, device=z.device, dtype=torch.uint8) if dense_idx else empty_codes(tuple(z.shape), z.device)
            ld_i = rowmat(idx)[2]
    _lib.call("fqss_actq_fwd", _p(z), None if skip_out else _p(out), _p(idx), rows, cols, ld_z, ld_o, ld_i, act,
              _p(slope), qmode, _p(qmin), _p(qmax), _p(obs_ws), _stream())
    return (out, idx) if want_idx else out


def obs_reset(obs_ws):
    _lib.call("fqss_obs_reset", _p(obs_ws), obs_ws.numel() // 2, _stream())


def observer_ema(qmin, qmax, obs_ws, alpha=0.9):
    _lib.call("fqss_observer_ema", _p(qmin), _p(qmax), _p(obs_ws), float(alpha), _stream())


def minmax(x, obs_ws):
    _need_gpu(x)
    x, rows, cols, ld = as_rowmat(x)
    _lib.call("fqss_minmax", _p(x), rows, cols, ld, _p(obs_ws), _stream())


def actq_bwd(z, g, act, slope, qmode, qmin, qmax, gacc, gbias=None, C=0, out=None):
    _need_gpu(z, g)
    rcz = rcg = None
    if gbias is None and out is None and z.dim() >= 3 and z.shape == g.shape and (rowmat(z) is None or rowmat(g) is None):
        rcz, rcg = _rowmat_collapsed(z), _rowmat_collapsed(g)
    if rcz is not None and rcg is not None and rcz[:2] == rcg[:2]:
        (rows, cols, ld_z), ld_g = rcz, rcg[2]
        gz = torch.empty(z.shape, device=z.device, dtype=torch.float32)
        ld_gz = cols
    else:
        z, rows, cols, ld_z = as_rowmat(z)
        g, r2, c2, ld_g = as_rowmat(g)
        assert (rows, cols) == (r2, c2), "actq_bwd: z/g shape mismatch"
        gz = empty_act(tuple(z.shape), z.device) if out is None else out
        rm = rowmat(gz)
        assert rm is not None and rm[:2] == (rows, cols), "actq_bwd: `out` must be a row-matrix view of z's shape"
        ld_gz = rm[2]
    _lib.call("fqss_actq_bwd", _p(z), _p(g), _p(gz), rows, cols, ld_z, ld_g, ld_gz, act, _p(slope), qmode,
              _p(qmin), _p(qmax), _p(gacc), _p(gbias), C, _stream())
    return gz


def actq_bwd_colbias(z, g, act, slope, qmode, qmin, qmax, gacc, gbias):
    _need_gpu(z, g, gbias)
    F = z.shape[-1]
    z, R, ld_z = _rows(z, F)
    g, R2, ld_g = _rows(g, F)
    assert R == R2, "actq_bwd_colbias: z/g shape mismatch"
    gz = torch.empty(*z.shape, device=z.device, dtype=torch.float32)
    _lib.call("fqss_actq_bwd_colbias", _p(z), _p(g), _p(gz), R, F, ld_z, ld_g, F, act, _p(slope), qmode, _p(qmin), _p(qmax), _p(gacc),
              _p(gbias), _stream())
    return gz


def actq2_bwd_colbias(z, g, qmin1, qmax1, qmin2, qmax2, gacc1, gacc2, gbias):
    _need_gpu(z, g, gbias)
    F = z.shape[-1]
    z, R, ld_z = _rows(z, F)
    g, R2, ld_g = _rows(g, F)
    assert R == R2, "actq2_bwd_colbias: z/g shape mismatch"
    gz = torch.empty(*z.shape, device=z.device, dtype=torch.float32)
    _lib.call("fqss_actq2_bwd_colbias", _p(z), _p(g), _p(gz), R, F, ld_z, ld_g, F, _p(qmin1), _p(qmax1), _p(qmin2), _p(qmax2), _p(gacc1), _p(gacc2),
              _p(gbias), _stream())
    return gz


def colbias_ok(F):
    return F % 4 == 0 and F <= 64 * 2048


def _w_layout(shape, axis):
    outer = 1
    for d in shape[:axis]:
        outer *= d
    inner = 1
    for d in shape[axis + 1:]:
        inner *= d
    return outer, shape[axis], inner


def wq_observe(w, axis, qmin, qmax):
    _need_gpu(w, qmin, qmax)
    o, c, i = _w_layout(w.shape, axis)
    _lib.call("fqss_wq_observe", _p(w.contiguous()), o, c, i, _p(qmin), _p(qmax), _stream())


def wq_fwd(w, axis, qmin, qmax, want_idx=False, n_bits=8):
    _need_gpu(w, qmin, qmax)
    w = w.contiguous()
    o, c, i = _w_layout(w.shape, axis)
    wq = torch.empty_like(w)
    idx = torch.empty(w.shape, device=w.device, dtype=torch.int8) if want_idx else None
    _lib.call("fqss_wq_fwd_bits", _p(w), _p(wq), _p(idx), o, c, i, _p(qmin), _p(qmax), int(n_bits), _stream())
    return (wq, idx) if want_idx else wq


def wq_bwd(w, g, axis, qmin, qmax, out=None, n_bits=8):
    _need_gpu(w, g, qmin, qmax)
    w, g = w.contiguous(), g.contiguous()
    o, c, i = _w_layout(w.shape, axis)
    if out is None:
        gw, gmin, gmax, acc = torch.empty_like(w), torch.empty_like(qmin), torch.empty_like(qmax), 0
    else:
        (gw, gmin, gmax), acc = out, 1
        assert gw.is_contiguous() and gmin.is_contiguous() and gmax.is_contiguous()
    _lib.call("fqss_wq_bwd_bits", _p(w), _p(g), _p(gw), _p(gmin), _p(gmax), o, c, i, _p(qmin), _p(qmax), acc, int(n_bits), _stream())
    return gw, gmin, gmax


def gacc_flush_multi(table):
    _lib.call("fqss_gacc_flush_multi", _p(table), table.shape[0], _stream())


def wq_table_check(rows):
    t = torch.tensor(rows, dtype=torch.int64).reshape(-1, WQ_DESC_WORDS).contiguous()
    _lib.call("fqss_wq_table_check", t.data_ptr(), t.shape[0])


def wq_multi_fwd(table, total_channels):
    _lib.call("fqss_wq_multi_fwd", _p(table), table.shape[0], total_channels, _stream())


def wq_multi_bwd(table, total_channels):
    _lib.call("fqss_wq_multi_bwd", _p(table), table.shape[0], total_channels, _stream())


def gacc_flush(gacc, gmin, gmax, gslope):
    _lib.call("fqss_gacc_flush", _p(gacc), _p(gmin), _p(gmax), _p(gslope), _stream())


def _bcm(t):
    assert t.dim() == 3, "expected [B, C, M]"
    t, rows, cols, ld = as_rowmat(t)
    return t, t.shape[0], t.shape[1], t.shape[2], ld


def pwconv_fwd(x, w, bias, six=False):
    _need_gpu(x, w, bias)
    x, B, Ci, M, ld_x = _bcm(x)
    Co = w.shape[0]
    assert w.is_contiguous() and w.numel() == Co * Ci
    z = empty_act((B, Co, M), x.device)
    fn = "fqss_pwconv_fwd" if not (USE_X3 and Ci % 4 == 0 and ld_x % 4 == 0 and x.data_ptr() % 16 == 0) else \
        "fqss_pwconv_fwd_x3s" if six else "fqss_pwconv_fwd_x3"
    _lib.call(fn, _p(x), _p(w), _p(bias), _p(z), B, Ci, Co, M, ld_x, rowmat(z)[2], _stream())
    return z


def pwconv_fwd_wq(x, wc, bias):
    _need_gpu(x, bias)
    x, B, Ci, M, ld_x = _bcm(x)
    if Ci != wc.Ci or Ci % 16 or Ci < 16 or ld_x % 4 or x.data_ptr() % 16 or not wc.idx.is_contiguous():
        return None
    z = empty_act((B, wc.Co, M), x.device)
    _lib.call("fqss_pwconv_fwd_wq", _p(x), _p(wc.idx), _p(wc.dw), _p(bias), _p(z), B, Ci, wc.Co, M, ld_x, rowmat(z)[2], _stream())
    return z


CONV_IMPLICIT_MAX_CO = 64


def conv1d_s1_ok(Ci, taps):
    return taps > 1 and (Ci * taps) % 4 == 0


def conv1d_s1_fwd(x, w2, bias, taps, dil, pad):
    _need_gpu(x, w2, bias)
    x, B, Ci, M, ld_x = _bcm(x)
    Co = w2.shape[0]
    assert w2.dim() == 2 and w2.shape[1] == Ci * taps and w2.stride(1) == 1
    if w2.stride(0) % 4 != 0 or w2.data_ptr() % 16 != 0:
        wp = torch.zeros(Co, (Ci * taps + 3) // 4 * 4, device=w2.device, dtype=torch.float32)
        wp[:, :Ci * taps] = w2
        w2 = wp[:, :Ci * taps]
    Mo = M + 2 * pad - dil * (taps - 1)
    z = empty_act((B, Co, Mo), x.device)
    _lib.call("fqss_conv1d_s1_fwd", _p(x), _p(w2), _p(bias), _p(z), B, Ci, Co, M, Mo, taps, dil, pad, ld_x, w2.stride(0), rowmat(z)[2], _stream())
    return z


def conv1d_s1_bwd_w(gz, x, gw, taps, dil, pad):
    _need_gpu(gz, x, gw)
    gz, B, Co, Mo, ld_gz = _bcm(gz)
    x, _, Ci, M, ld_x = _bcm(x)
    assert gw.is_contiguous() and gw.numel() == Co * Ci * taps and Mo == M + 2 * pad - dil * (taps - 1)
    _lib.call("fqss_conv1d_s1_bwd_w", _p(gz), _p(x), _p(gw), B, Ci, Co, M, Mo, taps, dil, pad, ld_gz, ld_x, _stream())


def pwconv_bwd_x(gz, w, Ci):
    _need_gpu(gz, w)
    gz, B, Co, M, ld_gz = _bcm(gz)
    gx = empty_act((B, Ci, M), gz.device)
    _lib.call("fqss_pwconv_bwd_x", _p(gz), _p(w), _p(gx), B, Ci, Co, M, ld_gz, rowmat(gx)[2], _stream())
    return gx


def pwconv_bwd_w(gz, x, gw):
    _need_gpu(gz, x, gw)
    gz, B, Co, M, ld_gz = _bcm(gz)
    x, _, Ci, _, ld_x = _bcm(x)
    assert gw.is_contiguous() and gw.numel() == Co * Ci
    _lib.call("fqss_pwconv_bwd_w", _p(gz), _p(x), _p(gw), B, Ci, Co, M, ld_gz, ld_x, _stream())


class WCodes:
    __slots__ = ("idx", "idxT", "dw", "rw", "Co", "Ci")


def wq_codes(w, qmin, qmax, n_bits=8):
    _need_gpu(w, qmin, qmax)
    Co, Ci = w.shape[0], w.shape[1]
    assert w.numel() == Co * Ci and w.is_contiguous()
    c = WCodes()
    c.Co, c.Ci = Co, Ci
    c.idx = torch.empty(Co, Ci, device=w.device, dtype=torch.int8)
    c.idxT = torch.empty(Ci, Co, device=w.device, dtype=torch.int8)
    c.dw = torch.empty(Co, device=w.device, dtype=torch.float32)
    c.rw = torch.empty(Co, device=w.device, dtype=torch.float32)
    _lib.call("fqss_wq_codes_bits", _p(w), _p(c.idx), _p(c.idxT), _p(c.dw), _p(c.rw), Co, Ci, _p(qmin), _p(qmax), int(n_bits), _stream())
    return c


def q_eligible(Ci, Co):
    return _lib.BACKEND != "cpu" and Ci % 16 == 0 and Co % 16 == 0 and Ci <= 512


def qpw_fwd(xc, wc, bias, qmin_x, qmax_x):
    B, Ci, M = xc.shape
    rm = rowmat(xc)
    assert rm is not None and rm[2] % 16 == 0
    z = empty_act((B, wc.Co, M), xc.device)
    _lib.call("fqss_qpw_fwd", _p(xc), _p(wc.idx), _p(wc.dw), _p(wc.rw), _p(bias), _p(qmin_x), _p(qmax_x), _p(z),
              B, Ci, wc.Co, M, rm[2], rowmat(z)[2], _stream())
    return z


def qpw_bwd_x(gz, wc, add=None):
    assert wc.idxT is not None, "this layer's codes live in a concatenated pair image: use qpw_bwd_x2"
    gz, B, Co, M, ld_gz = _bcm(gz)
    if ld_gz % 4 != 0 or gz.data_ptr() % 16 != 0:
        c = empty_act(tuple(gz.shape), gz.device)
        c.copy_(gz)
        gz, ld_gz = c, rowmat(c)[2]
    gx = empty_act((B, wc.Ci, M), gz.device)
    if add is not None:
        assert tuple(add.shape) == (B, wc.Ci, M)
        add, ld_add = _aligned_grad(add)
        _lib.call("fqss_qpw_bwd_x_add", _p(gz), _p(wc.idxT), _p(wc.dw), _p(add), _p(gx), B, wc.Ci, Co, M, ld_gz, ld_add, rowmat(gx)[2], _stream())
    else:
        _lib.call("fqss_qpw_bwd_x", _p(gz), _p(wc.idxT), _p(wc.dw), _p(gx), B, wc.Ci, Co, M, ld_gz, rowmat(gx)[2], _stream())
    return gx


def qpw_bwd_w(gz, xc, qmin_x, qmax_x, gw):
    gz, B, Co, M, ld_gz = _bcm(gz)
    if ld_gz % 4 != 0 or gz.data_ptr() % 16 != 0:
        c = empty_act(tuple(gz.shape), gz.device)
        c.copy_(gz)
        gz, ld_gz = c, rowmat(c)[2]
    Ci = xc.shape[1]
    _lib.call("fqss_qpw_bwd_w", _p(gz), _p(xc), _p(qmin_x), _p(qmax_x), _p(gw), B, Ci, Co, M, ld_gz, rowmat(xc)[2], _stream())


def qpw_fwd2(xc, wc, bias1, bias2, qmin_x, qmax_x, Co1):
    B, Ci, M = xc.shape
    rm = rowmat(xc)
    assert rm is not None and Ci == wc.Ci and 0 < Co1 < wc.Co
    z1, z2 = empty_act((B, Co1, M), xc.device), empty_act((B, wc.Co - Co1, M), xc.device)
    _lib.call("fqss_qpw_fwd2", _p(xc), _p(wc.idx), _p(wc.dw), _p(wc.rw), _p(bias1), _p(bias2), _p(qmin_x), _p(qmax_x), _p(z1), _p(z2),
              B, Ci, Co1, wc.Co - Co1, M, rm[2], rowmat(z1)[2], rowmat(z2)[2], _stream())
    return z1, z2


def qpw_fwdq(xc, wc, bias1, bias2, qmin_x, qmax_x, Co1, act, slope, r1, r2=None, stats=None, adds=None):
    B, Ci, M = xc.shape
    rm = rowmat(xc)
    Co2 = wc.Co - Co1
    assert rm is not None and Ci == wc.Ci and Co2 >= 0 and (Co2 == 0) == (r2 is None)
    z1, yc1 = empty_act((B, Co1, M), xc.device), empty_codes((B, Co1, M), xc.device)
    z2 = yc2 = None
    if Co2:
        z2, yc2 = empty_act((B, Co2, M), xc.device), empty_codes((B, Co2, M), xc.device)
    if adds is not None and any(a is not None for a in adds):
        assert act == ACT_NONE and stats is None and (adds[1] is None or Co2)
        sums, recs = [], []
        for a, Co in zip(adds, (Co1, Co2)):
            if a is None:
                sums.append(None); recs.append(None)
                continue
            ac, amin, amax, qmin, qmax = a
            assert tuple(ac.shape) == (B, Co, M) and rowmat(ac) is not None
            sc = empty_codes((B, Co, M), xc.device)
            r = _lib.FqssAddAfter()
            r.a, r.ld_a, r.amin, r.amax, r.qmin, r.qmax, r.y, r.ld_y = _p(ac), rowmat(ac)[2], _p(amin), _p(amax), _p(qmin), _p(qmax), _p(sc), rowmat(sc)[2]
            sums.append(sc); recs.append(r)
        _lib.call("fqss_qpw_fwdq_add", _p(xc), _p(wc.idx), _p(wc.dw), _p(wc.rw), _p(bias1), _p(bias2), _p(qmin_x), _p(qmax_x), _p(z1), _p(z2),
                  _p(r1[0]), _p(r1[1]), _p(r2[0]) if r2 else None, _p(r2[1]) if r2 else None, _p(yc1), _p(yc2),
                  B, Ci, Co1, Co2, M, rm[2], rowmat(z1)[2], rowmat(z2)[2] if Co2 else 0, rowmat(yc1)[2], rowmat(yc2)[2] if Co2 else 0,
                  _ref(recs[0]) if recs[0] is not None else None, _ref(recs[1]) if recs[1] is not None else None, _stream())
        return ((z1, z2, yc1, yc2) if Co2 else (z1, yc1)) + (tuple(sums),)
    w = _lib.FqssWCodes()
    w.idx, w.idxT, w.dw, w.rw, w.Co, w.Ci = _p(wc.idx), _p(wc.idxT), _p(wc.dw), _p(wc.rw), wc.Co, wc.Ci
    dx, dz1, dz2, dy1, dy2 = _desc(xc), _desc(z1), _desc(z2), _desc(yc1), _desc(yc2)
    qx, q1 = _qparams(qmin_x, qmax_x), _qparams(r1[0], r1[1], act, slope)
    q2 = _qparams(r2[0], r2[1], act, slope) if r2 else None
    ws, nws = (_p(stats.ws), stats.ws.numel() * stats.ws.element_size()) if stats is not None else (None, 0)
    _lib.call("fqss_pwconv_fq_fwd", _ref(dx), _ref(qx), _ref(w), _p(bias1), _p(bias2), _ref(dz1), _ref(dz2), _ref(dy1), _ref(dy2),
              _ref(q1), _ref(q2), ws, nws, _stream())
    return (z1, z2, yc1, yc2) if Co2 else (z1, yc1)


def qpw_bwd_x2(gz1, gz2, wc):
    gz1, ld1 = _aligned_grad(gz1)
    gz2, ld2 = _aligned_grad(gz2)
    B, Co1, M = gz1.shape
    Co2 = gz2.shape[1]
    assert Co1 + Co2 == wc.Co and gz2.shape[0] == B and gz2.shape[2] == M
    gx = empty_act((B, wc.Ci, M), gz1.device)
    _lib.call("fqss_qpw_bwd_x2", _p(gz1), _p(gz2), _p(wc.idxT), _p(wc.dw), _p(gx), B, wc.Ci, Co1, Co2, M, ld1, ld2, rowmat(gx)[2], _stream())
    return gx


def qpw_bwd_w2(gz1, gz2, xc, qmin_x, qmax_x, gw):
    gz1, ld1 = _aligned_grad(gz1)
    gz2, ld2 = _aligned_grad(gz2)
    B, Co1, M = gz1.shape
    Co2 = gz2.shape[1]
    Ci = xc.shape[1]
    assert gw.is_contiguous() and gw.numel() == (Co1 + Co2) * Ci
    _lib.call("fqss_qpw_bwd_w2", _p(gz1), _p(gz2), _p(xc), _p(qmin_x), _p(qmax_x), _p(gw), B, Ci, Co1, Co2, M, ld1, ld2, rowmat(xc)[2],
              _stream())


class WgradQueue:

    def __init__(self):
        self.jobs, self.ws = [], None

    def push(self, gz1, gz2, xc, qmin_x, qmax_x, gw):
        gz1, ld1 = _aligned_grad(gz1)
        ld2 = 0
        if gz2 is not None:
            gz2, ld2 = _aligned_grad(gz2)
        assert gw.is_contiguous()
        if any(j[5].data_ptr() == gw.data_ptr() for j in self.jobs):
            if gz2 is not None:
                qpw_bwd_w2(gz1, gz2, xc, qmin_x, qmax_x, gw)
            else:
                qpw_bwd_w(gz1, xc, qmin_x, qmax_x, gw)
            return
        self.jobs.append((gz1, gz2, xc, qmin_x, qmax_x, gw, ld1, ld2))

    def flush(self):
        if not self.jobs:
            return
        n = len(self.jobs)
        arr = (_lib.FqssWgradJob * n)()
        for j, (gz1, gz2, xc, lo, hi, gw, ld1, ld2) in zip(arr, self.jobs):
            B, Co1, M = gz1.shape
            j.gz1, j.gz2, j.xc, j.qmin_x, j.qmax_x, j.gw = _p(gz1), _p(gz2), _p(xc), _p(lo), _p(hi), _p(gw)
            j.B, j.Ci, j.Co1, j.Co2, j.M = B, xc.shape[1], Co1, (gz2.shape[1] if gz2 is not None else 0), M
            j.ld_gz1, j.ld_gz2, j.ld_xc = ld1, ld2, rowmat(xc)[2]
            assert gw.numel() == (j.Co1 + j.Co2) * j.Ci
        need = _lib.query("fqss_qpw_bwd_w_group_ws", arr, n)
        if need < 0:
            raise _lib.FqssError("fqss_qpw_bwd_w_group_ws: " + _lib.load().fqss_last_error().decode())
        if self.ws is None or self.ws.numel() < need:
            self.ws = torch.zeros(need, dtype=torch.uint8, device=self.jobs[0][0].device)
        _lib.call("fqss_qpw_bwd_w_group", arr, n, _p(self.ws), self.ws.numel(), _stream())
        self.jobs = []


def _codes3(xc):
    rm = rowmat(xc)
    assert xc.dim() == 3 and rm is not None and rm[2] % 16 == 0 and xc.data_ptr() % 16 == 0, "bad code layout"
    return xc.shape[0], xc.shape[1], xc.shape[2], rm[2]


def decode(xc, qmin, qmax):
    rm = rowmat(xc)
    out = empty_act(tuple(xc.shape), xc.device)
    _lib.call("fqss_decode", _p(xc), _p(out), rm[0], rm[1], rm[2], rowmat(out)[2], _p(qmin), _p(qmax), _stream())
    return out


class CodeStats:
    __slots__ = ("ws", "nslots")

    def __init__(self, ws, nslots):
        self.ws, self.nslots = ws, nslots


_STAT_SLOTS = {}


def stat_slots(kind, C, M):
    key = (kind, C, M)
    v = _STAT_SLOTS.get(key)
    if v is None:
        v = _STAT_SLOTS[key] = _lib.query("fqss_qpw_stat_slots" if kind == "qpw" else "fqss_dwq_stat_slots", C, M)
    return v


def new_stats(kind, B, C, M, device):
    n = stat_slots(kind, C, M)
    return CodeStats(torch.empty(B * n * 2, device=device, dtype=torch.int64), n) if n else None


def gnq_fwd(xc, qmin_x, qmax_x, gamma, beta, eps, qmin, qmax, write_out, stats=None):
    B, C, M, ld_xc = _codes3(xc)
    yc = empty_codes((B, C, M), xc.device)
    out = empty_act((B, C, M), xc.device)
    mean_rstd = torch.empty(B, 2, device=xc.device, dtype=torch.float32)
    ws = torch.empty(2 * 64 * B, device=xc.device, dtype=torch.int64) if stats is None else None
    _lib.call("fqss_gnq_fwd", _p(xc), _p(qmin_x), _p(qmax_x), _p(gamma), _p(beta), _p(yc), _p(out) if write_out else None,
              _p(mean_rstd), B, C, M, ld_xc, rowmat(yc)[2], rowmat(out)[2], float(eps), _p(qmin), _p(qmax), _p(ws),
              _p(stats.ws) if stats is not None else None, stats.nslots if stats is not None else 0, _stream())
    return out, yc, mean_rstd


def _aligned_grad(g):
    g, _, _, ld = as_rowmat(g)
    if ld % 4 != 0 or g.data_ptr() % 16 != 0:
        c = empty_act(tuple(g.shape), g.device)
        c.copy_(g)
        g, ld = c, rowmat(c)[2]
    return g, ld


def gnq_bwd(xc, qmin_x, qmax_x, g, gamma, beta, mean_rstd, qmin, qmax, gacc, ggamma, gbeta, producer=None):
    B, C, M, ld_xc = _codes3(xc)
    g, ld_g = _aligned_grad(g)
    gx = empty_act((B, C, M), xc.device)
    ws = torch.empty(2 * B * C + 2 * B, device=xc.device, dtype=torch.float64)
    if producer is None:
        _lib.call("fqss_gnq_bwd", _p(xc), _p(qmin_x), _p(qmax_x), _p(g), _p(gamma), _p(beta), _p(mean_rstd), _p(gx),
                  _p(ggamma), _p(gbeta), B, C, M, ld_xc, ld_g, rowmat(gx)[2], _p(qmin), _p(qmax), _p(gacc), _p(ws), _stream())
    else:
        pz, pact, pslope, pgacc, pgbias = producer
        rz = rowmat(pz)
        assert tuple(pz.shape) == (B, C, M) and rz is not None
        _lib.call("fqss_gnq_bwd_p", _p(xc), _p(qmin_x), _p(qmax_x), _p(g), _p(gamma), _p(beta), _p(mean_rstd), _p(gx),
                  _p(ggamma), _p(gbeta), B, C, M, ld_xc, ld_g, rowmat(gx)[2], _p(qmin), _p(qmax), _p(gacc), _p(ws),
                  _p(pz), rz[2], pact, _p(pslope), _p(pgacc), _p(pgbias), _stream())
    return gx


def gnq_bwd_rows(xc, qmin_x, qmax_x, g, gamma, beta, mean_rstd, qmin, qmax, gacc):
    B, C, M, ld_xc = _codes3(xc)
    g, ld_g = _aligned_grad(g)
    ws = torch.empty(2 * B * C, device=xc.device, dtype=torch.float64)
    _lib.call("fqss_gnq_bwd_rows", _p(xc), _p(qmin_x), _p(qmax_x), _p(g), _p(gamma), _p(beta), _p(mean_rstd), B, C, M, ld_xc, ld_g,
              _p(qmin), _p(qmax), _p(gacc), _p(ws), _stream())
    return g, ws


def gnq_bwd_apply(xc, qmin_x, qmax_x, g, gamma, beta, mean_rstd, qmin, qmax, ws, ggamma, gbeta, producer=None):
    B, C, M, ld_xc = _codes3(xc)
    g, ld_g = _aligned_grad(g)
    gx = empty_act((B, C, M), xc.device)
    pz, pact, pslope, pgacc, pgbias = producer if producer is not None else (None, 0, None, None, None)
    ld_pz = 0
    if pz is not None:
        rz = rowmat(pz)
        assert tuple(pz.shape) == (B, C, M) and rz is not None
        ld_pz = rz[2]
    _lib.call("fqss_gnq_bwd_apply", _p(xc), _p(qmin_x), _p(qmax_x), _p(g), _p(gamma), _p(beta), _p(mean_rstd), _p(gx), _p(ggamma),
              _p(gbeta), B, C, M, ld_xc, ld_g, rowmat(gx)[2], _p(qmin), _p(qmax), _p(ws), _p(pz), ld_pz, pact, _p(pslope), _p(pgacc),
              _p(pgbias), _stream())
    return gx


# ... 1896 lines not shown
```

fqss_amd/runtime.py:

```python
import os

import torch

from . import _lib
from . import kernels as K
from . import ops
from . import ops_dp


class ParamArena:
    def __init__(self, params, align=64):
        params = [p for p in params if p.requires_grad]
        assert params, "no trainable parameters"
        dev = params[0].device
        assert dev.type == ("cpu" if _lib.BACKEND == "cpu" else "cuda"), "ParamArena: parameters must live where the selected backend computes"
        offs, n = [], 0
        for p in params:
            offs.append(n)
            n += (p.numel() + align - 1) // align * align
        self.params, self.offsets, self.numel = params, offs, n
        self.flat_p = torch.zeros(n, device=dev)
        self.flat_g = torch.zeros(n, device=dev)
        self.exp_avg = torch.zeros(n, device=dev)
        self.exp_avg_sq = torch.zeros(n, device=dev)
# ... 85 lines not shown


class TeacherRunner:

    def __init__(self, fmodel):
        import torch.nn as nn
        from .quantization.qat.models.convtasnetq import ConvBlock, ConvTasNetQ
        self.fmodel = fmodel
        self.ok = False
        m = fmodel
        try:
            ok = isinstance(m, ConvTasNetQ) and type(m.encoder) is nn.Conv1d and type(m.decoder) is nn.ConvTranspose1d
            mk = m.masker
            ok = ok and type(mk.bottleneck[0]) is nn.GroupNorm and type(mk.bottleneck[1]) is nn.Conv1d
            ok = ok and type(mk.mask_net[0]) is nn.PReLU and type(mk.mask_net[1]) is nn.Conv1d and type(mk.mask_net[2]) is nn.ReLU
            for blk in mk.TCN:
                sb = blk.shared_block
                ok = ok and isinstance(blk, ConvBlock) and [type(t) for t in sb] == [nn.Conv1d, nn.PReLU, nn.GroupNorm, nn.Conv1d,
                                                                                   nn.PReLU, nn.GroupNorm]
                ok = ok and type(blk.res_conv) is nn.Conv1d and type(blk.skip_conv) is nn.Conv1d and sb[3].kernel_size[0] <= 8
                ok = ok and sb[0].in_channels % 8 == 0 and sb[0].out_channels % 8 == 0
            ok = ok and m.n_splitter == 1 and m.n_combiner == 1 and m.encoder.bias is None and m.decoder.bias is None
            ok = ok and m.decoder.out_channels == 1 and m.encoder.in_channels == 1 and m.encoder.kernel_size[0] in (16, 32)
            self.ok = bool(ok)
        except AttributeError:
            self.ok = False
        self._planes = None

    def _prepare(self):
        mk = self.fmodel.masker
        P = lambda conv: K.split3_planes(conv.weight.detach().reshape(conv.out_channels, conv.in_channels))
        blocks = []
        for blk in mk.TCN:
            sb = blk.shared_block
            rs_w = torch.cat([blk.res_conv.weight.detach(), blk.skip_conv.weight.detach()], 0)
            rs_b = torch.cat([blk.res_conv.bias.detach(), blk.skip_conv.bias.detach()], 0).contiguous()
            blocks.append((P(sb[0]), K.split3_planes(rs_w.reshape(rs_w.shape[0], rs_w.shape[1])), rs_b))
        self._planes = dict(bn=P(mk.bottleneck[1]), mask=P(mk.mask_net[1]), blocks=blocks)

    @torch.no_grad()
    def __call__(self, x):
        if not self.ok or (x.shape[-1] - self.fmodel.encoder.kernel_size[0]) // self.fmodel.encoder.stride[0] + 1 > 12 * 1024:
            return self.fmodel(x)
        if self._planes is None:
            self._prepare()
        m, mk, pl = self.fmodel, self.fmodel.masker, self._planes
        if x.dim() == 2:
            x = x.unsqueeze(1)
        B = x.shape[0]
        stride = m.encoder.stride[0]
        feats = K.frames_conv_fwd(x, m.encoder.weight, stride)
        nb = len(mk.TCN)
        st = K.tstat_buffer(1 + 2 * nb, B, x.device)
        K.tstats(feats, st[0])
        gn0, bn = mk.bottleneck[0], mk.bottleneck[1]
        h = K.tgemm(pl["bn"], feats, bn.bias, pro=1, pro_stats=st[0], pro_gamma=gn0.weight, pro_beta=gn0.bias, pro_eps=gn0.eps)
        acc = None
        nfeat = h.shape[1]
        for i, blk in enumerate(mk.TCN):
            sb = blk.shared_block
            p_c1, p_rs, b_rs = pl["blocks"][i]
            y1 = K.tgemm(p_c1, h, sb[0].bias, act=K.ACT_PRELU, slope=sb[1].weight, stats_out=st[1 + 2 * i])
            y3 = K.tdw(y1, st[1 + 2 * i], sb[2].weight, sb[2].bias, sb[2].eps, sb[3].weight, sb[3].bias, sb[4].weight,
                       st[2 + 2 * i], sb[3].dilation[0], sb[3].padding[0])
            h, acc = K.tgemm(p_rs, y3, b_rs, pro=1, pro_stats=st[2 + 2 * i], pro_gamma=sb[5].weight, pro_beta=sb[5].bias,
                             pro_eps=sb[5].eps, M1=nfeat, r1=h, r2=acc)
        mask = K.tgemm(pl["mask"], acc, mk.mask_net[1].bias, act=K.ACT_RELU, pro=2, pro_slope=mk.mask_net[0].weight)
        F_ = feats.shape[1]
        if K.ola_convtr_ok(m.decoder.weight, stride):
            dec = K.ola_convtr_mul_fwd(mask.reshape(B, m.n_srcs, F_, -1), feats, m.decoder.weight, stride)
        else:
            masked = K.mul_bcast_fwd(mask.reshape(B, m.n_srcs, F_, -1), feats)
            dec = K.ola_convtr_fwd(masked.reshape(B * m.n_srcs, F_, -1), m.decoder.weight, stride)
        return dec.reshape(B, m.n_srcs, -1)


class _LinearPair:
    __slots__ = ("wc", "gw", "Co1", "partner")


class QuantTables:

    def __init__(self, model, arena, segments=None):
        import torch.nn as nn
        from .quantization.qat.qat_layers import LayerQ
        from .quantization.qat.qat_quant import GradientActivationFakeQuantize, GradientWeightFakeQuantize
        dev = arena.flat_p.device
        aqs = [m for m in model.modules() if isinstance(m, GradientActivationFakeQuantize)]
        slope_of = {}
        for layer in model.modules():
            if isinstance(layer, LayerQ) and isinstance(getattr(layer, "nl", None), nn.PReLU):
                slope_of[id(layer.activation_fake_quantize)] = layer.nl.weight
        self.gacc = torch.zeros(len(aqs), K.GACC_DOUBLES, dtype=torch.float64, device=dev)
        rows = []
        for i, m in enumerate(aqs):
            m._buffers["_gacc"] = self.gacc[i]
            m._fqss_deferred = True
            sl = slope_of.get(id(m))
            rows.append([self.gacc[i].data_ptr(), m.min_range.grad.data_ptr(), m.max_range.grad.data_ptr(),
                         sl.grad.data_ptr() if sl is not None else 0])
        self.flush_table = torch.tensor(rows, dtype=torch.int64, device=dev)
        self.aqs = aqs
        from .quantization.qat.qat_layers import LSTMQ, MultiheadAttentionQ

        def fits(wqm, w):
            return isinstance(wqm, GradientWeightFakeQuantize) and isinstance(w, torch.nn.Parameter) and tuple(wqm.min_range.shape) == tuple(
                1 if d != wqm.axis else w.shape[d] for d in range(w.dim()))

        owners = []
        for layer in model.modules():
            wqm = getattr(layer, "weight_fake_quantize", None)
            if isinstance(wqm, GradientWeightFakeQuantize):
                for cand in ("conv1d", "convTr1d", "residual_encoder", "linear", "conv2d"):
                    conv = getattr(layer, cand, None)
                    if conv is not None and fits(wqm, getattr(conv, "weight", None)):
                        owners.append((wqm, conv.weight))
                        break
            if isinstance(layer, MultiheadAttentionQ):
                for wqm, w in ((layer.weight_fake_quantize_in, layer.mha.in_proj_weight), (layer.weight_fake_quantize_out, layer.mha.out_proj.weight)):
                    if fits(wqm, w):
                        owners.append((wqm, w))
            if isinstance(layer, LSTMQ):
                for name, wqm in layer.weight_quantizers_dict.items():
                    if fits(wqm, getattr(layer.lstm, name, None)):
                        owners.append((wqm, getattr(layer.lstm, name)))
        partner = {}
        for mod in model.modules():
            for n1, n2 in getattr(mod, "fqss_linear_pairs", ()):
                l1, l2 = getattr(mod, n1, None), getattr(mod, n2, None)
                w1 = getattr(getattr(l1, "conv1d", None), "weight", None)
                w2 = getattr(getattr(l2, "conv1d", None), "weight", None)
                own = {id(w) for _, w in owners}
                if w1 is None or w2 is None or id(w1) not in own or id(w2) not in own:
                    continue
                ok = w1.dim() == 3 and w1.shape[2] == 1 and w2.shape[1:] == w1.shape[1:] and K.q_eligible(w1.shape[1], w1.shape[0]) \
                    and K.q_eligible(w2.shape[1], w2.shape[0]) and (w1.numel() % 64 == 0) \
                    and (l1.conv1d.bias is None) == (l2.conv1d.bias is None)
                if ok:
                    partner[id(w1)] = w2
        second = {id(w2) for w2 in partner.values()}
        by_id = {id(w): (wqm, w) for wqm, w in owners}
        ordered = []
        for wqm, w in owners:
            if id(w) in second:
                continue
            ordered.append((wqm, w))
            if id(w) in partner:
                ordered.append(by_id[id(partner[id(w)])])
        owners = ordered
        n_gwq = sum((w.numel() + 63) // 64 * 64 for _, w in owners)
        self.gwq = torch.zeros(n_gwq, device=dev)
        self.wq_store = torch.empty(n_gwq, device=dev)
        rows, off, blk = [], 0, 0
        self.weights = []
        self.pairs = []
        pending = None
        for wqm, w in owners:
            shape, axis = tuple(w.shape), wqm.axis
            outer = 1
            for d in shape[:axis]:
                outer *= d
            inner = 1
            for d in shape[axis + 1:]:
                inner *= d
            C = shape[axis]
            wq = self.wq_store[off:off + w.numel()].view(shape)
            gwq = self.gwq[off:off + w.numel()].view(shape)
            pw = axis == 0 and w.dim() == 3 and shape[2] == 1 and K.q_eligible(shape[1], shape[0])
            pw = pw or (axis == 0 and w.dim() == 2 and ops_dp.QROW and K.qrow_eligible(shape[1]))
            fr = (not pw) and axis == 0 and w.dim() in (3, 4) and shape[0] % 16 == 0 and shape[0] <= 1024
            wc = None
            ldT = C
            if pw and id(w) in partner:
                w2 = partner[id(w)]
                Co1, Co2, Ci = shape[0], w2.shape[0], shape[1]
                pc = K.WCodes()
                pc.Co, pc.Ci = Co1 + Co2, Ci
                pc.idx = torch.empty(Co1 + Co2, Ci, device=dev, dtype=torch.int8)
                pc.idxT = torch.empty(Ci, Co1 + Co2, device=dev, dtype=torch.int8)
                pc.dw = torch.empty(Co1 + Co2, device=dev)
                pc.rw = torch.empty(Co1 + Co2, device=dev)
                pair = _LinearPair()
                pair.wc, pair.Co1 = pc, Co1
                pair.gw = self.gwq[off:off + w.numel() + w2.numel()].view(Co1 + Co2, Ci)
                pending = (pair, wq, 0)
            if pw and pending is not None:
                pair, wq_first, _ = pending
                pc = pair.wc
                r0 = 0 if wq_first is wq else pair.Co1
                wc = K.WCodes()
                wc.Co, wc.Ci = shape[0], shape[1]
                wc.idx = pc.idx[r0:r0 + shape[0]]
                wc.idxT = None
                wc.dw, wc.rw = pc.dw[r0:r0 + shape[0]], pc.rw[r0:r0 + shape[0]]
                ldT = pc.Co
                idxT_ptr = pc.idxT.data_ptr() + r0
                if wq_first is not wq:
                    pair.partner = wq
                    wq_first._fqss_pair = pair
                    self.pairs.append(pair)
                    pending = None
            elif pw or fr:
                wc = K.WCodes()
                wc.Co, wc.Ci = shape[0], (inner if fr else shape[1])
                wc.idx = torch.empty(wc.Co, wc.Ci, device=dev, dtype=torch.int8)
                wc.idxT = torch.empty(wc.Ci, wc.Co, device=dev, dtype=torch.int8)
                wc.dw = torch.empty(shape[0], device=dev)
                wc.rw = torch.empty(shape[0], device=dev)
                idxT_ptr = wc.idxT.data_ptr()
            coded = pw or fr
            rows.append([w.data_ptr(), wq.data_ptr(), wc.idx.data_ptr() if coded else 0, idxT_ptr if coded else 0,
                         wc.dw.data_ptr() if coded else 0, wc.rw.data_ptr() if coded else 0, wqm.min_range.data_ptr(),
                         wqm.max_range.data_ptr(), gwq.data_ptr(), w.grad.data_ptr(), wqm.min_range.grad.data_ptr(),
                         wqm.max_range.grad.data_ptr(), outer, C, inner, blk, ldT, int(wqm.n_bits)])
            wq._fqss_gwq = gwq
            if pw:
                wq._fqss_wcodes = wc
            elif fr:
                wq._fqss_wcodes_dgrad = wc
            w._fqss_wq = wq
            self.weights.append((wqm, w, wq, wc))
            off += (w.numel() + 63) // 64 * 64
            blk += C
        assert pending is None
        K.wq_table_check(rows)
        self.wq_table = torch.tensor(rows, dtype=torch.int64, device=dev)
        self.total_channels = blk
        self.det = None
        grouped = os.environ.get("FQSS_GROUP_WGRAD", "1") != "0"
        self.wgrad_queue = K.WgradQueue() if grouped else None
        self.row_wgrad_queue = K.RowWgradQueue() if grouped else None
        self.seg_tables = None
        if segments is not None and len(segments) > 1:
            self.seg_tables = []
            flush_rows = self.flush_table.tolist()
            for ids in segments:
                wrows, b0, members = [], 0, []
                for r, (wqm, w, _, _) in zip(rows, self.weights):
                    if id(w) in ids:
                        r = list(r)
                        r[15] = b0
                        b0 += r[13]
                        wrows.append(r)
                        members.append((wqm, w))
                frows = [r for r, m in zip(flush_rows, aqs) if id(m.min_range) in ids]
                self.seg_tables.append((torch.tensor(wrows, dtype=torch.int64, device=dev).reshape(-1, len(rows[0])), b0,
                                        torch.tensor(frows, dtype=torch.int64, device=dev).reshape(-1, 4), members))
            assert sum(t[0].shape[0] for t in self.seg_tables) == len(rows), "a weight quantizer belongs to no backward segment"
            assert sum(t[2].shape[0] for t in self.seg_tables) == len(flush_rows), "an activation quantizer belongs to no backward segment"

    def weights_forward(self):
        K.wq_multi_fwd(self.wq_table, self.total_channels)
        if self.wgrad_queue is not None:
            self.wgrad_queue.jobs = []
        if self.row_wgrad_queue is not None:
            self.row_wgrad_queue.jobs = []

    def finish_backward(self, seg=None):
        if self.wgrad_queue is not None:
            self.wgrad_queue.flush()
        if self.row_wgrad_queue is not None:
            self.row_wgrad_queue.flush()
        if self.det is not None:
            self.det.finish(1)
        if seg is None or self.seg_tables is None:
            K.wq_multi_bwd(self.wq_table, self.total_channels)
            K.gacc_flush_multi(self.flush_table)
            members = [(wqm, w) for wqm, w, _, _ in self.weights]
        else:
            wt, nch, ft, members = self.seg_tables[seg]
            if wt.shape[0]:
                K.wq_multi_bwd(wt, nch)
            if ft.shape[0]:
                K.gacc_flush_multi(ft)
        for wqm, w in members:
            w._fqss_touched = wqm.min_range._fqss_touched = wqm.max_range._fqss_touched = True


class KDTrainStep:

    def __init__(self, model, fmodel, kd_lambda=0.1, lr=1e-3, clip=5.0, comm=None, loss="sisdr_pit", source_weights=None,
                 batched_quantizers=True, fast=True, coded=True, buckets=None, sync_observer_ranges=True,
                 betas=(0.9, 0.999), loss_threshold=None, teacher_ahead=False):
        self.model, self.fmodel = model, fmodel
        self.cpu = _lib.BACKEND == "cpu"
        if self.cpu:
            batched_quantizers = fast = coded = teacher_ahead = False
        self.teacher_ahead = bool(teacher_ahead)
        self.grad_at = None
        self._ahead = None
        self._tgraph = None
        self.loss_kind, self.source_weights, self.batched_quantizers = loss, source_weights, batched_quantizers
        if loss not in ("sisdr_pit", "sisdr_pit_per_sample", "l1_sdr"):
            raise ValueError(f"unknown loss {loss!r}")
        self.loss_threshold = loss_threshold
        self.fast, self.coded = bool(fast and coded), bool(coded)
        self._graphs = None
        self.kd_lambda, self.lr, self.clip, self.betas = kd_lambda, lr, clip, tuple(betas)
        self.comm = comm
        self.segments = None
        self._seg_ids = None
        self._sync_ranges = bool(sync_observer_ranges)
        self._ranges_synced = not (sync_observer_ranges and self._exchange())
        params = list(model.parameters())
        force_b = os.environ.get("FQSS_FORCE_BUCKETS", "0") == "1" and self._exchange()
        nb = (4 if buckets is None else int(buckets)) if (self._world() > 1 or force_b) else (int(buckets) if buckets else 1)
        if nb > 1 and hasattr(model, "fqss_segments"):
            segs = model.fqss_segments(nb)
            if len(segs) > 1:
                seen, ordered, self._seg_ids = set(), [], []
                for mods in segs:
                    ids = set()
                    for m in mods:
                        for p in m.parameters():
                            if id(p) not in seen:
                                seen.add(id(p))
                                ordered.append(p)
                            ids.add(id(p))
                    self._seg_ids.append(ids)
                rest = [p for p in params if id(p) not in seen]
                self._seg_ids[0] |= {id(p) for p in rest}
                params = rest + ordered
        self.arena = ParamArena(params)
        name_of = {id(p): n for n, p in model.named_parameters()}
        self.arena.names = [name_of[id(p)] for p in self.arena.params]
        self.det = None
        if os.environ.get("FQSS_DETERMINISTIC", "0") == "1" and not self.cpu:
            self.det = K.DetMode()
            self.det.attach(0, self.arena.flat_g)
        if self._seg_ids is not None:
            off = {id(p): (o, o + (p.numel() + 63) // 64 * 64) for p, o in zip(self.arena.params, self.arena.offsets)}
            self.segments = []
            for ids in self._seg_ids:
                spans = [off[i] for i in ids if i in off]
                self.segments.append((min(a for a, _ in spans), max(b for _, b in spans)))
            assert all(self.segments[k][1] == self.segments[k + 1][0] for k in range(len(self.segments) - 1)), self.segments
        self._cstream = None
        self.comm_events = None
        for p in fmodel.parameters():
            p.requires_grad_(False)
        self.teacher = TeacherRunner(fmodel)
        if self.cpu:
            self.teacher.ok = False
        self._tstream = None
        self.last = None
        self.tables = None
        self._eager_q = 0
        self.use_graph = not self.cpu
        self._sx = self._st = None

    @property
    def lr(self):
        return self._lr

    @lr.setter
    def lr(self, value):
        if getattr(self, "_lr", None) != value:
            self._graphs = None
        self._lr = value

    def _quantizers(self):
        from .quantization.qat.qat_quant import GradientActivationFakeQuantize, GradientWeightFakeQuantize
        named = list(self.model.named_modules())
        return ([(n, m) for n, m in named if isinstance(m, GradientActivationFakeQuantize)],
                [(n, m) for n, m in named if isinstance(m, GradientWeightFakeQuantize)])

    def _ranks_differ(self):
        return self._world() > 1 and (not self._sync_ranges or not self._ranges_synced)

    def state_dict(self):
        aqs, wqs = self._quantizers()
        c = lambda t: t.detach().cpu().clone()
        held = {id(p) for p in self.arena.params}
        rank_ranges = None
        if self._ranks_differ() and aqs:
            mine = torch.stack([torch.cat([m.min_range.data.reshape(1), m.max_range.data.reshape(1)]).view(torch.int32) for _, m in aqs])
            mine = torch.cat([mine.cpu(), torch.tensor([[int(m.n_iter)] for _, m in aqs], dtype=torch.int32)], 1)
            rank_ranges = torch.stack(self.comm.all_gather(mine))
        return {"arena": self.arena.state_dict(),
                "act_quantizers": {n: {"n_iter": int(m.n_iter), "observer_mode": bool(m.observer_mode), "sign": bool(m.sign)} for n, m in aqs},
                "weight_quantizers": {n: {"observer_mode": bool(m.observer_mode)} for n, m in wqs},
                "ranges_synced": bool(self._ranges_synced), "lr": float(self.lr), "world": int(self._world()),
                "rank_ranges": rank_ranges,
                "buffers": {n: c(b) for n, b in self.model.named_buffers()},
                "frozen": {n: c(p) for n, p in self.model.named_parameters() if id(p) not in held}}

    def load_state_dict(self, sd):
        aqs, wqs = self._quantizers()
        for kind, have, want in (("activation", aqs, sd["act_quantizers"]), ("weight", wqs, sd["weight_quantizers"])):
            if [n for n, _ in have] != list(want):
                odd = sorted(set(want) ^ {n for n, _ in have})
                raise ValueError(f"KDTrainStep.load_state_dict: the stored {kind} quantizers are not this model's "
                                 f"({len(want)} in the file, {len(have)} here; e.g. {odd[:3]})")
        rr = sd.get("rank_ranges")
        if rr is not None and int(sd["world"]) != self._world():
            raise ValueError(f"KDTrainStep.load_state_dict: this state was written at world size {int(sd['world'])} while the ranks still "
                             f"held their own observer ranges; it resumes at that world size only, not at {self._world()}")
        buffers, frozen = dict(self.model.named_buffers()), {n: p for n, p in self.model.named_parameters()}
        for kind, have, want in (("buffers", buffers, sd["buffers"]), ("frozen parameters", frozen, sd["frozen"])):
            bad = [n for n, t in want.items() if n not in have or have[n].shape != t.shape]
            if bad or (kind == "buffers" and set(have) != set(want)):
                raise ValueError(f"KDTrainStep.load_state_dict: the stored {kind} are not this model's (e.g. {(bad or sorted(set(have) ^ set(want)))[:3]})")
        self.arena.load_state_dict(sd["arena"])
        with torch.no_grad():
            for n, t in sd["buffers"].items():
# ... 383 lines not shown
```

include/fqss.h:

```cpp
#ifndef FQSS_H
#define FQSS_H

#include <stddef.h>
#include <stdint.h>

#ifdef __cplusplus
extern "C" {
#endif

#define FQSS_VERSION 100

#define FQSS_OK 0
#define FQSS_EINVAL (-22)
#define FQSS_ELAUNCH (-5)

#define FQSS_Q_BYPASS 0
#define FQSS_Q_OBSERVE 1
#define FQSS_Q_QUANT 2

#define FQSS_ACT_NONE 0
#define FQSS_ACT_PRELU 1
#define FQSS_ACT_RELU 2
#define FQSS_ACT_GELU 3
#define FQSS_ACT_POST_RELU 4
#define FQSS_ACT_RELU_Q 5

typedef void* fqss_stream_t;

int fqss_version(void);
const char* fqss_last_error(void);
int fqss_selftest_div(const float* a, int64_t n, float b, uint64_t* mismatches, fqss_stream_t stream);


int fqss_actq_fwd(const float* z, float* out, uint8_t* idx, int64_t rows, int64_t cols,
                  int64_t ld_z, int64_t ld_out, int64_t ld_idx, int act, const float* slope, int qmode,
                  const float* qmin, const float* qmax, uint32_t* obs_ws, fqss_stream_t stream);

int fqss_obs_reset(uint32_t* obs_ws, int64_t n_pairs, fqss_stream_t stream);

int fqss_observer_ema(float* qmin, float* qmax, uint32_t* obs_ws, double alpha, fqss_stream_t stream);

#define FQSS_GACC_SLOTS 2048
int fqss_actq_bwd(const float* z, const float* g, float* gz, int64_t rows, int64_t cols,
                  int64_t ld_z, int64_t ld_g, int64_t ld_gz, int act, const float* slope, int qmode,
                  const float* qmin, const float* qmax, double* gacc, float* gbias, int64_t C,
                  fqss_stream_t stream);
int fqss_gluq_fwd(const float* z, float* out, int64_t B, int64_t C, int64_t M, int64_t ld_z, int64_t ld_out, int qmode,
                  const float* qmin, const float* qmax, uint32_t* obs_ws, fqss_stream_t stream);
int fqss_gluq_bwd(const float* z, const float* g, float* gz, int64_t B, int64_t C, int64_t M, int64_t ld_z, int64_t ld_g,
                  int64_t ld_gz, int qmode, const float* qmin, const float* qmax, double* gacc, fqss_stream_t stream);

int fqss_gacc_flush(double* gacc, float* gmin, float* gmax, float* gslope, fqss_stream_t stream);

int fqss_actq_bwd_colbias(const float* z, const float* g, float* gz, int64_t R, int F, int64_t ld_z, int64_t ld_g,
                          int64_t ld_gz, int act, const float* slope, int qmode, const float* qmin,
                          const float* qmax, double* gacc, float* gbias, fqss_stream_t stream);
int fqss_actq2_bwd_colbias(const float* z, const float* g, float* gz, int64_t R, int F, int64_t ld_z, int64_t ld_g, int64_t ld_gz,
                           const float* qmin1, const float* qmax1, const float* qmin2, const float* qmax2, double* gacc1, double* gacc2,
                           float* gbias, fqss_stream_t stream);

int fqss_minmax(const float* x, int64_t rows, int64_t cols, int64_t ld, uint32_t* obs_ws,
                fqss_stream_t stream);

#define FQSS_WQ_MIN_BITS 2
#define FQSS_WQ_MAX_BITS 8
int fqss_wq_observe(const float* w, int64_t outer, int64_t C, int64_t inner, float* qmin,
                    float* qmax, fqss_stream_t stream);
int fqss_wq_fwd(const float* w, float* wq, int8_t* idx, int64_t outer, int64_t C, int64_t inner,
                const float* qmin, const float* qmax, fqss_stream_t stream);
int fqss_wq_fwd_bits(const float* w, float* wq, int8_t* idx, int64_t outer, int64_t C, int64_t inner,
                     const float* qmin, const float* qmax, int n_bits, fqss_stream_t stream);
int fqss_wq_bwd(const float* w, const float* g, float* gw, float* gmin, float* gmax,
                int64_t outer, int64_t C, int64_t inner, const float* qmin, const float* qmax,
                int accumulate, fqss_stream_t stream);
int fqss_wq_bwd_bits(const float* w, const float* g, float* gw, float* gmin, float* gmax,
                     int64_t outer, int64_t C, int64_t inner, const float* qmin, const float* qmax,
                     int accumulate, int n_bits, fqss_stream_t stream);

#define FQSS_WQ_DESC_WORDS 18
int fqss_wq_table_check(const int64_t* host_table, int n);
int fqss_gacc_flush_multi(const int64_t* table, int n, fqss_stream_t stream);
int fqss_wq_multi_fwd(const int64_t* table, int n, int total_channels, fqss_stream_t stream);
int fqss_wq_multi_bwd(const int64_t* table, int n, int total_channels, fqss_stream_t stream);

int fqss_pwconv_fwd(const float* x, const float* w, const float* bias, float* z, int B, int Ci,
                    int Co, int M, int64_t ld_x, int64_t ld_z, fqss_stream_t stream);
int fqss_pwconv_fwd_x3(const float* x, const float* w, const float* bias, float* z, int B, int Ci,
                       int Co, int M, int64_t ld_x, int64_t ld_z, fqss_stream_t stream);
int fqss_pwconv_fwd_x3s(const float* x, const float* w, const float* bias, float* z, int B, int Ci,
                        int Co, int M, int64_t ld_x, int64_t ld_z, fqss_stream_t stream);
int fqss_pwconv_fwd_wq(const float* x, const int8_t* wi, const float* dw, const float* bias, float* z, int B, int Ci, int Co, int M,
                       int64_t ld_x, int64_t ld_z, fqss_stream_t stream);
int fqss_conv1d_s1_fwd(const float* x, const float* w, const float* bias, float* z, int B, int Ci, int Co, int M, int Mo, int taps,
                       int dil, int pad, int64_t ld_x, int64_t ld_w, int64_t ld_z, fqss_stream_t stream);
int fqss_conv1d_s1_bwd_w(const float* gz, const float* x, float* gw, int B, int Ci, int Co, int M, int Mo, int taps, int dil,
                         int pad, int64_t ld_gz, int64_t ld_x, fqss_stream_t stream);
int fqss_halo_pack(const float* x, float* xp, int64_t B, int64_t C, int64_t H, int64_t W, int64_t sb, int64_t sc, int64_t sh,
                   int ph, int pw, int64_t Wp, int64_t plane, fqss_stream_t stream);
int fqss_phase_pack(const float* x, float* xp, int64_t B, int64_t C, int64_t H, int64_t W, int64_t sb, int64_t sc, int64_t sh, int axis,
                    int s, int p, int64_t Wp, int64_t plane, fqss_stream_t stream);
int fqss_phase_unpack(const float* gy, float* gx, int64_t B, int64_t C, int64_t H, int64_t W, int64_t sb, int64_t sc, int64_t sh, int axis,
                      int s, int p, int64_t Hy, int64_t Wp, int64_t plane, int off, const float* bias, fqss_stream_t stream);
int fqss_conv2_fwd_wq(const float* xp, const int8_t* wi, const float* dw, const float* bias, float* z, int B, int Ci, int Co, int taps,
                      int kw, int base, int row_step, int col_step, int64_t N, int64_t plane_in, int64_t plane_out, fqss_stream_t stream);
int fqss_conv2_fwd_x3s(const float* xp, const float* w, const float* bias, float* z, int B, int Ci, int Co, int taps, int kw, int base,
                       int row_step, int col_step, int64_t N, int64_t plane_in, int64_t plane_out, fqss_stream_t stream);
int fqss_conv2_bwd_x_wq(const float* gzp, const int8_t* wiT, const float* dw, float* gx, int B, int Ci, int Co, int taps, int kw,
                        int base, int row_step, int col_step, int64_t N, int64_t plane_in, int64_t plane_out, fqss_stream_t stream);
int fqss_conv2_bwd_w(const float* gzp, const float* xp, float* gw, int B, int Ci, int Co, int taps, int kw, int row_step, int col_step,
                     int off, int64_t plane_g, int64_t plane_x, fqss_stream_t stream);
int fqss_pwconv_bwd_x(const float* gz, const float* w, float* gx, int B, int Ci, int Co, int M,
                      int64_t ld_gz, int64_t ld_gx, fqss_stream_t stream);
int fqss_pwconv_bwd_w(const float* gz, const float* x, float* gw, int B, int Ci, int Co, int M,
                      int64_t ld_gz, int64_t ld_x, fqss_stream_t stream);

int fqss_wq_codes(const float* w, int8_t* idx, int8_t* idxT, float* dw, float* rw, int Co, int Ci,
                  const float* qmin, const float* qmax, fqss_stream_t stream);
int fqss_wq_codes_bits(const float* w, int8_t* idx, int8_t* idxT, float* dw, float* rw, int Co, int Ci,
                       const float* qmin, const float* qmax, int n_bits, fqss_stream_t stream);
int fqss_qpw_fwd(const uint8_t* xc, const int8_t* wi, const float* dw, const float* rw,
                 const float* bias, const float* qmin_x, const float* qmax_x, float* z, int B, int Ci,
                 int Co, int M, int64_t ld_xc, int64_t ld_z, fqss_stream_t stream);
int fqss_qpw_bwd_x(const float* gz, const int8_t* wiT, const float* dw, float* gx, int B, int Ci,
                   int Co, int M, int64_t ld_gz, int64_t ld_gx, fqss_stream_t stream);
int fqss_qpw_bwd_w(const float* gz, const uint8_t* xc, const float* qmin_x, const float* qmax_x,
                   float* gw, int B, int Ci, int Co, int M, int64_t ld_gz, int64_t ld_xc,
                   fqss_stream_t stream);
int fqss_qpw_bwd_x_add(const float* gz, const int8_t* wiT, const float* dw, const float* addend, float* gx, int B, int Ci,
                       int Co, int M, int64_t ld_gz, int64_t ld_add, int64_t ld_gx, fqss_stream_t stream);
int fqss_qpw_fwd2(const uint8_t* xc, const int8_t* wi, const float* dw, const float* rw, const float* bias1,
                  const float* bias2, const float* qmin_x, const float* qmax_x, float* z1, float* z2, int B,
                  int Ci, int Co1, int Co2, int M, int64_t ld_xc, int64_t ld_z1, int64_t ld_z2,
                  fqss_stream_t stream);
int fqss_qpw_bwd_x2(const float* gz1, const float* gz2, const int8_t* wiT, const float* dw, float* gx, int B,
                    int Ci, int Co1, int Co2, int M, int64_t ld_gz1, int64_t ld_gz2, int64_t ld_gx,
                    fqss_stream_t stream);
int fqss_qpw_bwd_w2(const float* gz1, const float* gz2, const uint8_t* xc, const float* qmin_x,
                    const float* qmax_x, float* gw, int B, int Ci, int Co1, int Co2, int M, int64_t ld_gz1,
                    int64_t ld_gz2, int64_t ld_xc, fqss_stream_t stream);

typedef struct FqssWgradJob {
    const float* gz1; const float* gz2;
    const uint8_t* xc;
    const float* qmin_x; const float* qmax_x;
    float* gw;
    int32_t B, Ci, Co1, Co2, M;
    int64_t ld_gz1, ld_gz2, ld_xc;
} FqssWgradJob;
int64_t fqss_qpw_bwd_w_group_ws(const FqssWgradJob* jobs, int njobs);
int fqss_qpw_bwd_w_group(const FqssWgradJob* jobs, int njobs, void* ws, int64_t ws_bytes, fqss_stream_t stream);
int fqss_qpw_fwdq(const uint8_t* xc, const int8_t* wi, const float* dw, const float* rw, const float* bias1,
                  const float* bias2, const float* qmin_x, const float* qmax_x, float* z1, float* z2, int act,
                  const float* slope, const float* qmin1, const float* qmax1, const float* qmin2,
                  const float* qmax2, uint8_t* yc1, uint8_t* yc2, int B, int Ci, int Co1, int Co2, int M,
                  int64_t ld_xc, int64_t ld_z1, int64_t ld_z2, int64_t ld_yc1, int64_t ld_yc2,
                  int64_t* stats1, fqss_stream_t stream);
int fqss_qpw_stat_slots(int Co, int M);
int fqss_dwq_stat_slots(int C, int M);
typedef struct {
    const uint8_t* a; int64_t ld_a;
    const float *amin, *amax, *qmin, *qmax;
    uint8_t* y; int64_t ld_y;
} FqssAddAfter;
int fqss_qpw_fwdq_add(const uint8_t* xc, const int8_t* wi, const float* dw, const float* rw, const float* bias1,
                      const float* bias2, const float* qmin_x, const float* qmax_x, float* z1, float* z2, const float* qmin1,
                      const float* qmax1, const float* qmin2, const float* qmax2, uint8_t* yc1, uint8_t* yc2, int B, int Ci,
                      int Co1, int Co2, int M, int64_t ld_xc, int64_t ld_z1, int64_t ld_z2, int64_t ld_yc1, int64_t ld_yc2,
                      const FqssAddAfter* add1, const FqssAddAfter* add2, fqss_stream_t stream);

int fqss_dwconv_fwd(const float* x, const float* w, const float* bias, float* z, int B, int C,
                    int M, int K, int dil, int pad, int64_t ld_x, int64_t ld_z, fqss_stream_t stream);
int fqss_dwconv_bwd_x(const float* gz, const float* w, float* gx, int B, int C, int M, int K,
                      int dil, int pad, int64_t ld_gz, int64_t ld_gx, fqss_stream_t stream);
int fqss_dwconv_bwd_w(const float* gz, const float* x, float* gw, int B, int C, int M, int K,
                      int dil, int pad, int64_t ld_gz, int64_t ld_x, fqss_stream_t stream);

int fqss_gn_fwd(const float* x, const float* gamma, const float* beta, float* z, float* mean_rstd,
                int B, int C, int M, int64_t ld_x, int64_t ld_z, float eps, double* ws,
                fqss_stream_t stream);
int fqss_gn_fwd_tail(const float* x, const float* gamma, const float* beta, float* y, int B, int C, int M, int64_t ld_x, int64_t ld_y,
                     float eps, double* ws, int tail, const float* ls, const float* res, int64_t ld_res, fqss_stream_t stream);
int fqss_gn_bwd(const float* gz, const float* x, const float* gamma, const float* mean_rstd,
                float* gx, float* ggamma, float* gbeta, int B, int C, int M, int64_t ld_gz,
                int64_t ld_x, int64_t ld_gx, double* ws, fqss_stream_t stream);
int fqss_gnq_fwd_f(const float* x, const float* gamma, const float* beta, float* y, uint8_t* yc , float* mean_rstd,
                   int B, int C, int M, int64_t ld_x, int64_t ld_y, int64_t ld_yc, float eps, double* ws, const float* qmin, const float* qmax,
                   fqss_stream_t stream);
int fqss_gnq_bwd_f(const float* g, const float* x, const float* gamma, const float* beta, const float* mean_rstd, float* gx, float* ggamma,
                   float* gbeta, int B, int C, int M, int64_t ld_g, int64_t ld_x, int64_t ld_gx, double* ws, const float* qmin,
                   const float* qmax, double* gacc, fqss_stream_t stream);

int fqss_decode(const uint8_t* codes, float* out, int64_t rows, int64_t cols, int64_t ld_c,
                int64_t ld_out, const float* qmin, const float* qmax, fqss_stream_t stream);
int fqss_gnq_fwd(const uint8_t* xc, const float* qmin_x, const float* qmax_x, const float* gamma,
                 const float* beta, uint8_t* yc, float* yout, float* mean_rstd, int B, int C, int M,
                 int64_t ld_xc, int64_t ld_yc, int64_t ld_out, float eps, const float* qmin,
                 const float* qmax, void* ws, const int64_t* stats, int nslots, fqss_stream_t stream);
int fqss_gnq_bwd(const uint8_t* xc, const float* qmin_x, const float* qmax_x, const float* g,
                 const float* gamma, const float* beta, const float* mean_rstd, float* gx,
                 float* ggamma, float* gbeta, int B, int C, int M, int64_t ld_xc, int64_t ld_g,
                 int64_t ld_gx, const float* qmin, const float* qmax, double* gacc, double* ws,
                 fqss_stream_t stream);
int fqss_gnq_bwd_p(const uint8_t* xc, const float* qmin_x, const float* qmax_x, const float* g,
                   const float* gamma, const float* beta, const float* mean_rstd, float* gz, float* ggamma,
                   float* gbeta, int B, int C, int M, int64_t ld_xc, int64_t ld_g, int64_t ld_gz,
                   const float* qmin, const float* qmax, double* gacc, double* ws, const float* pz,
                   int64_t ld_pz, int pact, const float* pslope, double* pgacc, float* pgbias,
                   fqss_stream_t stream);

int fqss_dwq_fwd(const uint8_t* xc, const float* qmin_x, const float* qmax_x, const float* w,
                 const float* bias, uint8_t* yc, float* yout, int B, int C, int M, int K, int dil,
                 int pad, int64_t ld_xc, int64_t ld_yc, int64_t ld_out, int act, const float* slope,
                 const float* qmin, const float* qmax, int64_t* stats, fqss_stream_t stream);
int fqss_dwq_bwd_z(const uint8_t* xc, const float* qmin_x, const float* qmax_x, const float* w,
                   const float* bias, const float* g, float* gz, int B, int C, int M, int K, int dil,
                   int pad, int64_t ld_xc, int64_t ld_g, int64_t ld_gz, int act, const float* slope,
                   const float* qmin, const float* qmax, double* gacc, float* gbias,
                   fqss_stream_t stream);
int fqss_ewq_fwd(const uint8_t* ac, const float* amin, const float* amax, const uint8_t* bc,
                 const float* bmin, const float* bmax, const float* bf, float sb, uint8_t* yc, float* yout,
                 int64_t rows, int64_t cols, int64_t ld_a, int64_t ld_b, int64_t ld_bf, int64_t ld_y,
                 int64_t ld_out, int act, const float* slope, const float* qmin, const float* qmax,
                 fqss_stream_t stream);
int fqss_ewq_bwd(const uint8_t* ac, const float* amin, const float* amax, const uint8_t* bc,
                 const float* bmin, const float* bmax, const float* bf, float sb, const float* g, float* gz,
                 int64_t rows, int64_t cols, int64_t ld_a, int64_t ld_b, int64_t ld_bf, int64_t ld_g,
                 int64_t ld_gz, int act, const float* slope, const float* qmin, const float* qmax,
                 double* gacc, fqss_stream_t stream);
int fqss_ewq_bwd_p(const uint8_t* ac, const float* amin, const float* amax, const uint8_t* bc,
                   const float* bmin, const float* bmax, float sb, const float* g, float* gz, int64_t rows,
                   int64_t cols, int64_t ld_a, int64_t ld_b, int64_t ld_g, int64_t ld_gz, int act,
                   const float* slope, const float* qmin, const float* qmax, double* gacc, int C,
                   const float* pa_z, int64_t ld_paz, int pa_act, const float* pa_slope, double* pa_gacc,
                   float* pa_gbias, float* pa_out, int64_t ld_pa_out, const float* pb_z, int64_t ld_pbz,
                   int pb_act, const float* pb_slope, double* pb_gacc, float* pb_gbias, float* pb_out,
                   int64_t ld_pb_out, fqss_stream_t stream);
int fqss_mulq_fwd(const uint8_t* mc, const float* mmin, const float* mmax, const uint8_t* fc, const float* fmin,
                  const float* fmax, uint8_t* yc, float* yout, int B, int S, int C, int M, int64_t ld_m, int64_t ld_f,
                  int64_t ld_y, int64_t ld_out, const float* qmin, const float* qmax, fqss_stream_t stream);
int fqss_mulq_bwd(const uint8_t* mc, const float* mmin, const float* mmax, const uint8_t* fc, const float* fmin,
                  const float* fmax, const float* g, float* gmask, float* gfeat, int B, int S, int C, int M, int64_t ld_m,
                  int64_t ld_f, int64_t ld_g, int64_t ld_gm, int64_t ld_gf, const float* qmin, const float* qmax,
                  double* gacc, const float* pz, int64_t ld_pz, int pact, const float* pslope, double* pgacc,
                  float* pgbias, fqss_stream_t stream);
int fqss_dwq_bwd_w(const float* gz, const uint8_t* xc, const float* qmin_x, const float* qmax_x,
                   float* gw, int B, int C, int M, int K, int dil, int pad, int64_t ld_gz,
                   int64_t ld_xc, fqss_stream_t stream);
int fqss_dwq_bwd(const uint8_t* xc, const float* qmin_x, const float* qmax_x, const float* w,
                 const float* bias, const float* g, float* gx, float* gw, int B, int C, int M, int K,
                 int dil, int pad, int64_t ld_xc, int64_t ld_g, int64_t ld_gx, int act, const float* slope,
                 const float* qmin, const float* qmax, double* gacc, float* gbias, fqss_stream_t stream);

typedef struct FqssGnAfter {
    const float* gamma; const float* beta; const float* mean_rstd;
    const double* ws;
    const float* qmin; const float* qmax;
    float* ggamma; float* gbeta;
} FqssGnAfter;
typedef struct FqssGnBefore {
    const uint8_t* xc0; int64_t ld_xc0; const float* qmin0; const float* qmax0;
    const float* gamma; const float* beta; const float* mean_rstd;
    double* ws;
    double* gacc;
} FqssGnBefore;
int fqss_gnq_bwd_rows(const uint8_t* xc, const float* qmin_x, const float* qmax_x, const float* g, const float* gamma,
                      const float* beta, const float* mean_rstd, int B, int C, int M, int64_t ld_xc, int64_t ld_g,
                      const float* qmin, const float* qmax, double* gacc, double* ws, fqss_stream_t stream);
int fqss_gnq_bwd_apply(const uint8_t* xc, const float* qmin_x, const float* qmax_x, const float* g, const float* gamma,
                       const float* beta, const float* mean_rstd, float* gx, float* ggamma, float* gbeta, int B, int C, int M,
                       int64_t ld_xc, int64_t ld_g, int64_t ld_gx, const float* qmin, const float* qmax, const double* ws,
                       const float* pz, int64_t ld_pz, int pact, const float* pslope, double* pgacc, float* pgbias,
                       fqss_stream_t stream);
int fqss_dwq_bwd_gn(const uint8_t* xc, const float* qmin_x, const float* qmax_x, const float* w, const float* bias,
                    const float* g, float* gx, float* gw, int B, int C, int M, int K, int dil, int pad, int64_t ld_xc,
                    int64_t ld_g, int64_t ld_gx, int act, const float* slope, const float* qmin, const float* qmax,
                    double* gacc, float* gbias, const FqssGnAfter* after, const FqssGnBefore* before, fqss_stream_t stream);

#define FQSS_TSTAT_SLOTS 32
#define FQSS_TSTAT_STRIDE 16
int fqss_split3_planes(const float* w, uint16_t* planes, int64_t n, fqss_stream_t stream);
int fqss_tgemm(const uint16_t* planes, const float* x, int B, int Ci, int Co, int M, int64_t ld_x, int pro,
               const double* pro_stats, const float* pro_gamma, const float* pro_beta, float pro_eps,
               const float* pro_slope, const float* bias, int act, const float* slope, double* stats_out,
               int M1, float* c1, const float* r1, int64_t ld_c1, float* c2, const float* r2,
               int64_t ld_c2, fqss_stream_t stream);
int fqss_tgemm_tiled_ok(int Ci, int Co, int M1);
int fqss_split3_tiles(const float* w, uint16_t* tiles, int Co, int Ci, fqss_stream_t stream);
int fqss_tgemm_tiled(const uint16_t* tiles, const float* x, int B, int Ci, int Co, int M, int64_t ld_x, int pro,
                     const double* pro_stats, const float* pro_gamma, const float* pro_beta, float pro_eps,
                     const float* pro_slope, const float* bias, int act, const float* slope, double* stats_out,
                     int M1, float* c1, const float* r1, int64_t ld_c1, float* c2, const float* r2,
                     int64_t ld_c2, fqss_stream_t stream);
int fqss_tdw(const float* x, const double* stats_in, const float* gamma, const float* beta, float eps,
             const float* w, const float* bias, const float* slope, float* y, double* stats_out, int B,
             int C, int M, int K, int dil, int pad, int64_t ld_x, int64_t ld_y, fqss_stream_t stream);
int fqss_tstats(const float* x, int B, int C, int M, int64_t ld, double* ws, fqss_stream_t stream);

int fqss_bn_moments(const float* x, double* out, int B, int C, int M, int64_t ld_x, fqss_stream_t stream);
int fqss_bn_apply(const float* x, const float* a, const float* b, float* y, int B, int C, int M, int64_t ld_x,
                  int64_t ld_y, fqss_stream_t stream);
int fqss_bn_bwd_reduce(const float* g, const float* x, double* out, int B, int C, int M, int64_t ld_g, int64_t ld_x,
                       fqss_stream_t stream);
int fqss_bn_bwd_apply(const float* g, const float* x, const float* c1, const float* c2, const float* c3, float* gx,
                      int B, int C, int M, int64_t ld_g, int64_t ld_x, int64_t ld_gx, fqss_stream_t stream);

int fqss_axpby(const float* a, const float* b, float sa, float sb, float* z, int64_t rows,
               int64_t cols, int64_t ld_a, int64_t ld_b, int64_t ld_z, fqss_stream_t stream);
int fqss_mul_bcast_fwd(const float* mask, const float* feat, float* z, int B, int S, int C, int M,
                       int64_t ld_mask, int64_t ld_feat, int64_t ld_z, fqss_stream_t stream);
int fqss_mul_bcast_bwd(const float* gz, const float* mask, const float* feat, float* gmask,
                       float* gfeat, int B, int S, int C, int M, int64_t ld_gz, int64_t ld_mask,
                       int64_t ld_feat, int64_t ld_gmask, int64_t ld_gfeat, fqss_stream_t stream);

int fqss_splitter2(const float* x, float* out, int B, int64_t T, const uint32_t* obs_ws,
                   fqss_stream_t stream);
int fqss_splitter2_rows(const float* x, float* out, int B, int64_t T, uint32_t* row_max, fqss_stream_t stream);
int fqss_splitter2_raw(const float* x, float* out, int B, int64_t T, const uint32_t* obs_ws, fqss_stream_t stream);
int fqss_frames_conv_fwd(const float* x, const float* w, float* z, int N, int Ci, int Co,
                         int64_t T, int K, int stride, int M, int64_t ld_z, fqss_stream_t stream);
int fqss_frames_conv_add_fwd(const float* x, const float* w, const float* add, int64_t ld_add, float* z, int N, int Ci,
                             int Co, int64_t T, int K, int stride, int M, int64_t ld_z, fqss_stream_t stream);
// ... 323 lines not shown
```

Before: 628.1 samples/s.

## Pre-pack quantized 1x1 weights into tiled bf16 images for q-GEMM A loads

```diff
diff --git a/fqss_amd/csrc/fqss_dev.h b/fqss_amd/csrc/fqss_dev.h
--- a/fqss_amd/csrc/fqss_dev.h
+++ b/fqss_amd/csrc/fqss_dev.h
@@ -48,6 +48,9 @@
 }
 
 constexpr int kWave = 64;
+
+__device__ __forceinline__ int64_t wimg_at(int r, int k, int rpad) { return ((int64_t)(k >> 5) * rpad + r) * 32 + (k & 31); }
+__device__ __forceinline__ unsigned short wimg_bf16(float q) { return (unsigned short)(__float_as_uint(q) >> 16); }
 
 __device__ __forceinline__ uint32_t f2ord(float f) {
     uint32_t u = __float_as_uint(f);
diff --git a/fqss_amd/csrc/multi.hip b/fqss_amd/csrc/multi.hip
--- a/fqss_amd/csrc/multi.hip
+++ b/fqss_amd/csrc/multi.hip
@@ -40,9 +40,13 @@
     return table + (int64_t)lo * kWqFields;
 }
 
-__global__ __launch_bounds__(256) void k_wq_multi_fwd(const long long* __restrict__ table, int n) {
+__global__ __launch_bounds__(256) void k_wq_multi_fwd(const long long* __restrict__ table, const long long* __restrict__ img_table, int n) {
     __shared__ float red[4];
     const long long* d = find_desc(table, n, blockIdx.x);
+    const long long* im = img_table != nullptr ? img_table + 3 * ((d - table) / kWqFields) : nullptr;
+    unsigned short* img = im != nullptr ? reinterpret_cast<unsigned short*>(im[0]) : nullptr;
+    unsigned short* imgT = im != nullptr ? reinterpret_cast<unsigned short*>(im[1]) : nullptr;
+    const int irow = im != nullptr ? (int)im[2] + (blockIdx.x - (int)d[15]) : 0;
     const float* w = reinterpret_cast<const float*>(d[0]);
     float* wq = reinterpret_cast<float*>(d[1]);
     signed char* idx = reinterpret_cast<signed char*>(d[2]);
@@ -70,6 +74,10 @@
         if (idx) {
             idx[(int64_t)c * nel + e] = (signed char)q;
             idxT[(int64_t)e * ldT + c] = (signed char)q;
+            if (img) {
+                img[wimg_at(irow, e, ((int)ldT + 127) & ~127)] = wimg_bf16(q);
+                imgT[wimg_at(e, irow, (nel + 127) & ~127)] = wimg_bf16(q);
+            }
             s += q;
         }
     }
@@ -153,8 +161,16 @@
     FQSS_REQUIRE(table && n >= 0 && total_channels >= 0, "bad args");
     if (n == 0 || total_channels == 0) return FQSS_OK;
     hipLaunchKernelGGL(k_wq_multi_fwd, dim3((unsigned)total_channels), dim3(256), 0, (hipStream_t)stream,
-                       (const long long*)table, n);
+                       (const long long*)table, (const long long*)nullptr, n);
     return launch_status("fqss_wq_multi_fwd");
+}
+
+extern "C" int fqss_wq_multi_fwd_img(const int64_t* table, const int64_t* img_table, int n, int total_channels, fqss_stream_t stream) {
+    FQSS_REQUIRE(table && img_table && n >= 0 && total_channels >= 0, "bad args");
+    if (n == 0 || total_channels == 0) return FQSS_OK;
+    hipLaunchKernelGGL(k_wq_multi_fwd, dim3((unsigned)total_channels), dim3(256), 0, (hipStream_t)stream,
+                       (const long long*)table, (const long long*)img_table, n);
+    return launch_status("fqss_wq_multi_fwd_img");
 }
 
 extern "C" int fqss_wq_multi_bwd(const int64_t* table, int n, int total_channels, fqss_stream_t stream) {
diff --git a/fqss_amd/csrc/qgemm.hip b/fqss_amd/csrc/qgemm.hip
--- a/fqss_amd/csrc/qgemm.hip
+++ b/fqss_amd/csrc/qgemm.hip
@@ -45,9 +45,13 @@
 };
 __device__ __forceinline__ void q_load16(f32x4& d, const void* p) { asm volatile("global_load_dwordx4 %0, %1, off" : "=v"(d) : "v"(p) : "memory"); }
 __device__ __forceinline__ void q_load8(u32x2& d, const void* p) { asm volatile("global_load_dwordx2 %0, %1, off" : "=v"(d) : "v"(p) : "memory"); }
-template <int MODE, int N>
+template <int MODE, int N, bool AIMG = false>
 __device__ __forceinline__ void q_wait(QStage& st) {
-    if constexpr (MODE == 0)
+    if constexpr (MODE == 0 && AIMG)
+        asm volatile("s_waitcnt vmcnt(%3)" : "+v"(st.a[0]), "+v"(st.a[1]), "+v"(st.bq) : "n"(N) : "memory");
+    else if constexpr (MODE == 1 && AIMG)
+        asm volatile("s_waitcnt vmcnt(%4)" : "+v"(st.a[0]), "+v"(st.a[1]), "+v"(st.b[0]), "+v"(st.b[1]) : "n"(N) : "memory");
+    else if constexpr (MODE == 0)
         asm volatile("s_waitcnt vmcnt(%2)" : "+v"(st.a[0]), "+v"(st.bq) : "n"(N) : "memory");
     else if constexpr (MODE == 1)
         asm volatile("s_waitcnt vmcnt(%3)" : "+v"(st.a[0]), "+v"(st.b[0]), "+v"(st.b[1]) : "n"(N) : "memory");
@@ -92,8 +96,9 @@
     float imp_inv_taps, imp_inv_kw;
 };
 
-template <int MODE, int GP = 3, bool IMP = false>
+template <int MODE, int GP = 3, bool IMP = false, bool AIMG = false>
 __global__ __launch_bounds__(256, 2) void k_qgemm(QGemmArgs g) {
+    static_assert(!AIMG || ((MODE == 0 || MODE == 1) && !IMP), "weight image: forward / dgrad of the 1x1 convolutions");
     static_assert(!IMP || MODE == 1 || MODE == 3 || MODE == 4, "implicit convolution: float B operands");
     static_assert(MODE == 0 || MODE == 1 || MODE == 3 || MODE == 4, "unknown q-GEMM mode");
     static_assert(GP == 3 || (GP == 2 && MODE != 0 && MODE != 4), "two gradient pieces: dgrad only");
@@ -139,7 +144,7 @@
         }
     }
 
-    constexpr int NLOADS = (MODE == 0) ? 2 : (WMODE == 1) ? 3 : 6;
+    constexpr int NLOADS = ((MODE == 0) ? 2 : (WMODE == 1) ? 3 : 6) + (AIMG ? 1 : 0);
     const int a_row = tid >> 1, a_k = (tid & 1) * 16;
     const int bk_row = tid >> 3, bk_n = (tid & 7) * 8;
     const int a_row_c = min(i0 + a_row, g.M - 1);
@@ -153,8 +158,14 @@
     const char* const gB1 = sgpr((const char*)g.B + (int64_t)b * g.sBb * BEL);
     const char* const gB2 = (MODE == 0) ? gB1 : sgpr((const char*)g.B2 + (int64_t)b * g.sB2b * BEL);
     const int64_t gldb1 = sgpr(g.ldb), gldb2 = (MODE == 0) ? gldb1 : sgpr(g.ldb2);
+    const char* const a_img = AIMG ? (const char*)g.A + ((int64_t)(i0 + a_row) * QBK + a_k) * 2 : nullptr;
+    const int64_t a_img_step = (int64_t)g.tiles_m * QBM * QBK * 2;
     auto load_tiles = [&](QStage& st, int k0) {
-        if constexpr (ACODES) {
+        if constexpr (AIMG) {
+            const char* p = a_img + min(k0 / QBK, (g.K - 1) / QBK) * a_img_step;
+            q_load16(st.a[0], p);
+            q_load16(st.a[1], p + 16);
+        } else if constexpr (ACODES) {
             q_load16(st.a[0], (const signed char*)g.A + (int64_t)a_row_c * g.lda + min(k0 + a_k, g.K - 16));
         } else {
             const float* A = (const float*)g.A + (int64_t)b * g.sAb + (int64_t)a_row_c * g.lda;
@@ -261,9 +272,12 @@
     };
 
     auto store_tiles = [&](QStage& st, int k0) {
-        q_wait<WMODE, NLOADS>(st);
+        q_wait<WMODE, NLOADS, AIMG>(st);
         const bool kz = (k0 + bk_row) >= g.K;
-        if constexpr (ACODES) {
+        if constexpr (AIMG) {
+            *reinterpret_cast<f32x4*>(&As[0][a_row][a_k]) = st.a[0];
+            *reinterpret_cast<f32x4*>(&As[0][a_row][a_k + 8]) = st.a[1];
+        } else if constexpr (ACODES) {
             const unsigned int w[4] = {__float_as_uint(st.a[0][0]), __float_as_uint(st.a[0][1]), __float_as_uint(st.a[0][2]),
                                        __float_as_uint(st.a[0][3])};
             store_codes(&As[0][a_row][a_k], w, std::integral_constant<int, 4>{}, true, false);
@@ -336,8 +350,8 @@
             }
         }
     }
-    q_wait<WMODE, 0>(stA);
-    q_wait<WMODE, 0>(stB);
+    q_wait<WMODE, 0, AIMG>(stA);
+    q_wait<WMODE, 0, AIMG>(stB);
 
     float dx = 0.f, mnx = 0.f;
     if constexpr (MODE == 0) {
@@ -925,7 +939,8 @@
 }
 
 __global__ __launch_bounds__(256) void k_wq_codes(const float* __restrict__ w, signed char* __restrict__ idx,
-                                                   signed char* __restrict__ idxT, float* dw, float* rw, int Co, int Ci,
+                                                   signed char* __restrict__ idxT, unsigned short* __restrict__ img,
+                                                   unsigned short* __restrict__ imgT, float* dw, float* rw, int Co, int Ci,
                                                    const float* __restrict__ qmin, const float* __restrict__ qmax, int n_bits) {
     __shared__ float red[4];
     const int co = blockIdx.x;
@@ -938,6 +953,10 @@
         const float q = fminf(fmaxf(X, qlo), qhi);
         idx[(int64_t)co * Ci + ci] = (signed char)q;
         idxT[(int64_t)ci * Co + co] = (signed char)q;
+        if (img != nullptr) {
+            img[wimg_at(co, ci, (Co + 127) & ~127)] = wimg_bf16(q);
+            imgT[wimg_at(ci, co, (Ci + 127) & ~127)] = wimg_bf16(q);
+        }
         s += q;
     }
     float v[1] = {s};
@@ -957,13 +976,25 @@
     return (e != nullptr && e[0] == '2') ? 2 : 3;
 }
 
+static int wq_codes_impl(const char* who, const float* w, int8_t* idx, int8_t* idxT, uint16_t* img, uint16_t* imgT, float* dw, float* rw,
+                         int Co, int Ci, const float* qmin, const float* qmax, int n_bits, fqss_stream_t stream) {
+    FQSS_REQUIRE(w && idx && idxT && dw && rw && qmin && qmax && Co > 0 && Ci > 0, "bad args");
+    FQSS_REQUIRE(n_bits >= FQSS_WQ_MIN_BITS && n_bits <= FQSS_WQ_MAX_BITS, "weight width outside 2..8 bits");
+    FQSS_REQUIRE((img == nullptr) == (imgT == nullptr) && aligned16(img) && aligned16(imgT), "weight images: both or neither, 16-B aligned");
+    hipLaunchKernelGGL(k_wq_codes, dim3((unsigned)Co), dim3(256), 0, (hipStream_t)stream, w, (signed char*)idx,
+                       (signed char*)idxT, (unsigned short*)img, (unsigned short*)imgT, dw, rw, Co, Ci, qmin, qmax, n_bits);
+    return launch_status(who);
+}
+
 extern "C" int fqss_wq_codes_bits(const float* w, int8_t* idx, int8_t* idxT, float* dw, float* rw, int Co, int Ci,
                                   const float* qmin, const float* qmax, int n_bits, fqss_stream_t stream) {
-    FQSS_REQUIRE(w && idx && idxT && dw && rw && qmin && qmax && Co > 0 && Ci > 0, "bad args");
-    FQSS_REQUIRE(n_bits >= FQSS_WQ_MIN_BITS && n_bits <= FQSS_WQ_MAX_BITS, "weight width outside 2..8 bits");
-    hipLaunchKernelGGL(k_wq_codes, dim3((unsigned)Co), dim3(256), 0, (hipStream_t)stream, w, (signed char*)idx,
-                       (signed char*)idxT, dw, rw, Co, Ci, qmin, qmax, n_bits);
-    return launch_status("fqss_wq_codes_bits");
+    return wq_codes_impl("fqss_wq_codes_bits", w, idx, idxT, nullptr, nullptr, dw, rw, Co, Ci, qmin, qmax, n_bits, stream);
+}
+
+extern "C" int fqss_wq_codes_img(const float* w, int8_t* idx, int8_t* idxT, uint16_t* img, uint16_t* imgT, float* dw, float* rw, int Co,
+                                 int Ci, const float* qmin, const float* qmax, int n_bits, fqss_stream_t stream) {
+    FQSS_REQUIRE(img && imgT, "null image");
+    return wq_codes_impl("fqss_wq_codes_img", w, idx, idxT, img, imgT, dw, rw, Co, Ci, qmin, qmax, n_bits, stream);
 }
 
 extern "C" int fqss_wq_codes(const float* w, int8_t* idx, int8_t* idxT, float* dw, float* rw, int Co, int Ci,
@@ -980,7 +1011,7 @@
 static int qpw_fwd_impl(const char* who, const uint8_t* xc, const int8_t* wi, const float* dw, const float* rw, const float* bias1,
                         const float* bias2, const float* qmin_x, const float* qmax_x, float* z1, float* z2, int B, int Ci, int Co1,
                         int Co2, int M, int64_t ld_xc, int64_t ld_z1, int64_t ld_z2, fqss_stream_t stream,
-                        const QpwQuant* qq = nullptr) {
+                        const QpwQuant* qq = nullptr, bool img = false) {
     if (B == 0 || M == 0) return FQSS_OK;
     const int Co = Co1 + Co2;
     FQSS_REQUIRE(xc && wi && dw && rw && qmin_x && qmax_x && z1 && (Co2 == 0 || z2), "null tensor");
@@ -1026,7 +1057,10 @@
         }
     }
     g.tiles_n = (int)cdiv(M, QBN); g.tiles_m = (int)cdiv(Co, QBM); g.batches = B;
-    hipLaunchKernelGGL((k_qgemm<0>), dim3(xcd_grid((int64_t)g.tiles_n * B, g.tiles_m)), dim3(256), 0, (hipStream_t)stream, g);
+    if (img)
+        hipLaunchKernelGGL((k_qgemm<0, 3, false, true>), dim3(xcd_grid((int64_t)g.tiles_n * B, g.tiles_m)), dim3(256), 0, (hipStream_t)stream, g);
+    else
+        hipLaunchKernelGGL((k_qgemm<0>), dim3(xcd_grid((int64_t)g.tiles_n * B, g.tiles_m)), dim3(256), 0, (hipStream_t)stream, g);
     return launch_status(who);
 }
 
@@ -1065,7 +1099,7 @@
 
 static int qpw_bwd_x_impl(const char* who, const float* gz1, const float* gz2, const int8_t* wiT, const float* dw, float* gx, int B,
                           int Ci, int Co1, int Co2, int M, int64_t ld_gz1, int64_t ld_gz2, int64_t ld_gx, fqss_stream_t stream,
-                          const float* addend = nullptr, int64_t ld_add = 0) {
+                          const float* addend = nullptr, int64_t ld_add = 0, bool img = false) {
     if (B == 0 || M == 0) return FQSS_OK;
     const int Co = Co1 + Co2;
     FQSS_REQUIRE(gz1 && wiT && dw && gx && (Co2 == 0 || gz2), "null tensor");
@@ -1087,10 +1121,12 @@
         g.C2 = const_cast<float*>(addend); g.ldc2 = ld_add; g.sC2b = (int64_t)Ci * ld_add;
     }
     g.tiles_n = (int)cdiv(M, QBN); g.tiles_m = (int)cdiv(Ci, QBM); g.batches = B;
-    if (grad_pieces() == 3)
-        hipLaunchKernelGGL((k_qgemm<1, 3>), dim3(xcd_grid((int64_t)g.tiles_n * B, g.tiles_m)), dim3(256), 0, (hipStream_t)stream, g);
-    else
-        hipLaunchKernelGGL((k_qgemm<1, 2>), dim3(xcd_grid((int64_t)g.tiles_n * B, g.tiles_m)), dim3(256), 0, (hipStream_t)stream, g);
+    const dim3 grid(xcd_grid((int64_t)g.tiles_n * B, g.tiles_m));
+    const bool three = grad_pieces() == 3;
+    if (img && three) hipLaunchKernelGGL((k_qgemm<1, 3, false, true>), grid, dim3(256), 0, (hipStream_t)stream, g);
+    else if (img) hipLaunchKernelGGL((k_qgemm<1, 2, false, true>), grid, dim3(256), 0, (hipStream_t)stream, g);
+    else if (three) hipLaunchKernelGGL((k_qgemm<1, 3>), grid, dim3(256), 0, (hipStream_t)stream, g);
+    else hipLaunchKernelGGL((k_qgemm<1, 2>), grid, dim3(256), 0, (hipStream_t)stream, g);
     return launch_status(who);
 }
 
@@ -1109,6 +1145,62 @@
                                int Co1, int Co2, int M, int64_t ld_gz1, int64_t ld_gz2, int64_t ld_gx, fqss_stream_t stream) {
     FQSS_REQUIRE(Co2 > 0, "second layer missing");
     return qpw_bwd_x_impl("fqss_qpw_bwd_x2", gz1, gz2, wiT, dw, gx, B, Ci, Co1, Co2, M, ld_gz1, ld_gz2, ld_gx, stream);
+}
+
+extern "C" int fqss_qpw_fwd_img(const uint8_t* xc, const uint16_t* wimg, const float* dw, const float* rw, const float* bias,
+                                const float* qmin_x, const float* qmax_x, float* z, int B, int Ci, int Co, int M, int64_t ld_xc,
+                                int64_t ld_z, fqss_stream_t stream) {
+    return qpw_fwd_impl("fqss_qpw_fwd_img", xc, (const int8_t*)wimg, dw, rw, bias, nullptr, qmin_x, qmax_x, z, nullptr, B, Ci, Co, 0, M, ld_xc,
+                        ld_z, 0, stream, nullptr, true);
+}
+
+extern "C" int fqss_qpw_fwd2_img(const uint8_t* xc, const uint16_t* wimg, const float* dw, const float* rw, const float* bias1,
+                                 const float* bias2, const float* qmin_x, const float* qmax_x, float* z1, float* z2, int B, int Ci,
+                                 int Co1, int Co2, int M, int64_t ld_xc, int64_t ld_z1, int64_t ld_z2, fqss_stream_t stream) {
+    FQSS_REQUIRE(Co2 > 0, "second layer missing");
+    return qpw_fwd_impl("fqss_qpw_fwd2_img", xc, (const int8_t*)wimg, dw, rw, bias1, bias2, qmin_x, qmax_x, z1, z2, B, Ci, Co1, Co2, M, ld_xc,
+                        ld_z1, ld_z2, stream, nullptr, true);
+}
+
+extern "C" int fqss_qpw_fwdq_img(const uint8_t* xc, const uint16_t* wimg, const float* dw, const float* rw, const float* bias1,
+                                 const float* bias2, const float* qmin_x, const float* qmax_x, float* z1, float* z2, int act,
+                                 const float* slope, const float* qmin1, const float* qmax1, const float* qmin2, const float* qmax2,
+                                 uint8_t* yc1, uint8_t* yc2, int B, int Ci, int Co1, int Co2, int M, int64_t ld_xc, int64_t ld_z1,
+                                 int64_t ld_z2, int64_t ld_yc1, int64_t ld_yc2, int64_t* stats1, fqss_stream_t stream) {
+    QpwQuant qq{act, slope, qmin1, qmax1, qmin2, qmax2, yc1, yc2, ld_yc1, ld_yc2, (long long*)stats1, nullptr, nullptr};
+    return qpw_fwd_impl("fqss_qpw_fwdq_img", xc, (const int8_t*)wimg, dw, rw, bias1, bias2, qmin_x, qmax_x, z1, z2, B, Ci, Co1, Co2, M, ld_xc,
+                        ld_z1, ld_z2, stream, &qq, true);
+}
+
+extern "C" int fqss_qpw_fwdq_add_img(const uint8_t* xc, const uint16_t* wimg, const float* dw, const float* rw, const float* bias1,
+                                     const float* bias2, const float* qmin_x, const float* qmax_x, float* z1, float* z2,
+                                     const float* qmin1, const float* qmax1, const float* qmin2, const float* qmax2, uint8_t* yc1,
+                                     uint8_t* yc2, int B, int Ci, int Co1, int Co2, int M, int64_t ld_xc, int64_t ld_z1, int64_t ld_z2,
+                                     int64_t ld_yc1, int64_t ld_yc2, const FqssAddAfter* add1, const FqssAddAfter* add2,
+                                     fqss_stream_t stream) {
+    QpwQuant qq{FQSS_ACT_NONE, nullptr, qmin1, qmax1, qmin2, qmax2, yc1, yc2, ld_yc1, ld_yc2, nullptr, add1, add2};
+    return qpw_fwd_impl("fqss_qpw_fwdq_add_img", xc, (const int8_t*)wimg, dw, rw, bias1, bias2, qmin_x, qmax_x, z1, z2, B, Ci, Co1, Co2, M,
+                        ld_xc, ld_z1, ld_z2, stream, &qq, true);
+}
+
+extern "C" int fqss_qpw_bwd_x_img(const float* gz, const uint16_t* wimgT, const float* dw, float* gx, int B, int Ci, int Co, int M,
+                                  int64_t ld_gz, int64_t ld_gx, fqss_stream_t stream) {
+    return qpw_bwd_x_impl("fqss_qpw_bwd_x_img", gz, nullptr, (const int8_t*)wimgT, dw, gx, B, Ci, Co, 0, M, ld_gz, 0, ld_gx, stream, nullptr, 0,
+                          true);
+}
+
+extern "C" int fqss_qpw_bwd_x_add_img(const float* gz, const uint16_t* wimgT, const float* dw, const float* addend, float* gx, int B,
+                                      int Ci, int Co, int M, int64_t ld_gz, int64_t ld_add, int64_t ld_gx, fqss_stream_t stream) {
+    FQSS_REQUIRE(addend, "null addend");
+    return qpw_bwd_x_impl("fqss_qpw_bwd_x_add_img", gz, nullptr, (const int8_t*)wimgT, dw, gx, B, Ci, Co, 0, M, ld_gz, 0, ld_gx, stream, addend,
+                          ld_add, true);
+}
+
+extern "C" int fqss_qpw_bwd_x2_img(const float* gz1, const float* gz2, const uint16_t* wimgT, const float* dw, float* gx, int B, int Ci,
+                                   int Co1, int Co2, int M, int64_t ld_gz1, int64_t ld_gz2, int64_t ld_gx, fqss_stream_t stream) {
+    FQSS_REQUIRE(Co2 > 0, "second layer missing");
+    return qpw_bwd_x_impl("fqss_qpw_bwd_x2_img", gz1, gz2, (const int8_t*)wimgT, dw, gx, B, Ci, Co1, Co2, M, ld_gz1, ld_gz2, ld_gx, stream,
+                          nullptr, 0, true);
 }
 
 static int qpw_bwd_w_impl(const char* who, const float* gz1, const float* gz2, const uint8_t* xc, const float* qmin_x,
diff --git a/fqss_amd/kernels.py b/fqss_amd/kernels.py
--- a/fqss_amd/kernels.py
+++ b/fqss_amd/kernels.py
@@ -277,8 +277,12 @@
     _lib.call("fqss_wq_table_check", t.data_ptr(), t.shape[0])
 
 
-def wq_multi_fwd(table, total_channels):
-    _lib.call("fqss_wq_multi_fwd", _p(table), table.shape[0], total_channels, _stream())
+def wq_multi_fwd(table, total_channels, img_table=None):
+    if img_table is not None:
+        assert img_table.shape == (table.shape[0], 3) and img_table.is_contiguous()
+        _lib.call("fqss_wq_multi_fwd_img", _p(table), _p(img_table), table.shape[0], total_channels, _stream())
+    else:
+        _lib.call("fqss_wq_multi_fwd", _p(table), table.shape[0], total_channels, _stream())
 
 
 def wq_multi_bwd(table, total_channels):
@@ -364,10 +368,23 @@
 
 
 class WCodes:
-    __slots__ = ("idx", "idxT", "dw", "rw", "Co", "Ci")
-
-
-def wq_codes(w, qmin, qmax, n_bits=8):
+    __slots__ = ("idx", "idxT", "dw", "rw", "Co", "Ci", "img", "imgT")
+
+    def __init__(self):
+        self.img = self.imgT = None
+
+
+def new_wimg(R, Kd, device):
+    return torch.zeros((Kd + 31) // 32, (R + 127) // 128 * 128, 32, device=device, dtype=torch.bfloat16)
+
+
+def wimg_codes(img, R, Kd):
+    full = img.permute(1, 0, 2).reshape(img.shape[1], -1)
+    pad_zero = bool((full[R:] == 0).all()) and bool((full[:, Kd:] == 0).all())
+    return full[:R, :Kd], pad_zero
+
+
+def wq_codes(w, qmin, qmax, n_bits=8, images=True):
     _need_gpu(w, qmin, qmax)
     Co, Ci = w.shape[0], w.shape[1]
     assert w.numel() == Co * Ci and w.is_contiguous()
@@ -377,25 +394,35 @@
     c.idxT = torch.empty(Ci, Co, device=w.device, dtype=torch.int8)
     c.dw = torch.empty(Co, device=w.device, dtype=torch.float32)
     c.rw = torch.empty(Co, device=w.device, dtype=torch.float32)
-    _lib.call("fqss_wq_codes_bits", _p(w), _p(c.idx), _p(c.idxT), _p(c.dw), _p(c.rw), Co, Ci, _p(qmin), _p(qmax), int(n_bits), _stream())
+    if images and _lib.BACKEND == "hip":
+        c.img, c.imgT = new_wimg(Co, Ci, w.device), new_wimg(Ci, Co, w.device)
+        _lib.call("fqss_wq_codes_img", _p(w), _p(c.idx), _p(c.idxT), _p(c.img), _p(c.imgT), _p(c.dw), _p(c.rw), Co, Ci, _p(qmin), _p(qmax),
+                  int(n_bits), _stream())
+    else:
+        _lib.call("fqss_wq_codes_bits", _p(w), _p(c.idx), _p(c.idxT), _p(c.dw), _p(c.rw), Co, Ci, _p(qmin), _p(qmax), int(n_bits), _stream())
     return c
+
+
+def _wsel(name, codes, img, int8):
+    return (name + "_img", img) if (img is not None and not int8) else (name, codes)
 
 
 def q_eligible(Ci, Co):
     return _lib.BACKEND != "cpu" and Ci % 16 == 0 and Co % 16 == 0 and Ci <= 512
 
 
-def qpw_fwd(xc, wc, bias, qmin_x, qmax_x):
+def qpw_fwd(xc, wc, bias, qmin_x, qmax_x, int8=False):
     B, Ci, M = xc.shape
     rm = rowmat(xc)
     assert rm is not None and rm[2] % 16 == 0
     z = empty_act((B, wc.Co, M), xc.device)
-    _lib.call("fqss_qpw_fwd", _p(xc), _p(wc.idx), _p(wc.dw), _p(wc.rw), _p(bias), _p(qmin_x), _p(qmax_x), _p(z),
+    fn, wa = _wsel("fqss_qpw_fwd", wc.idx, wc.img, int8)
+    _lib.call(fn, _p(xc), _p(wa), _p(wc.dw), _p(wc.rw), _p(bias), _p(qmin_x), _p(qmax_x), _p(z),
               B, Ci, wc.Co, M, rm[2], rowmat(z)[2], _stream())
     return z
 
 
-def qpw_bwd_x(gz, wc, add=None):
+def qpw_bwd_x(gz, wc, add=None, int8=False):
     assert wc.idxT is not None, "this layer's codes live in a concatenated pair image: use qpw_bwd_x2"
     gz, B, Co, M, ld_gz = _bcm(gz)
     if ld_gz % 4 != 0 or gz.data_ptr() % 16 != 0:
@@ -406,9 +433,11 @@
     if add is not None:
         assert tuple(add.shape) == (B, wc.Ci, M)
         add, ld_add = _aligned_grad(add)
-        _lib.call("fqss_qpw_bwd_x_add", _p(gz), _p(wc.idxT), _p(wc.dw), _p(add), _p(gx), B, wc.Ci, Co, M, ld_gz, ld_add, rowmat(gx)[2], _stream())
+        fn, wa = _wsel("fqss_qpw_bwd_x_add", wc.idxT, wc.imgT, int8)
+        _lib.call(fn, _p(gz), _p(wa), _p(wc.dw), _p(add), _p(gx), B, wc.Ci, Co, M, ld_gz, ld_add, rowmat(gx)[2], _stream())
     else:
-        _lib.call("fqss_qpw_bwd_x", _p(gz), _p(wc.idxT), _p(wc.dw), _p(gx), B, wc.Ci, Co, M, ld_gz, rowmat(gx)[2], _stream())
+        fn, wa = _wsel("fqss_qpw_bwd_x", wc.idxT, wc.imgT, int8)
+        _lib.call(fn, _p(gz), _p(wa), _p(wc.dw), _p(gx), B, wc.Ci, Co, M, ld_gz, rowmat(gx)[2], _stream())
     return gx
 
 
@@ -422,17 +451,18 @@
     _lib.call("fqss_qpw_bwd_w", _p(gz), _p(xc), _p(qmin_x), _p(qmax_x), _p(gw), B, Ci, Co, M, ld_gz, rowmat(xc)[2], _stream())
 
 
-def qpw_fwd2(xc, wc, bias1, bias2, qmin_x, qmax_x, Co1):
+def qpw_fwd2(xc, wc, bias1, bias2, qmin_x, qmax_x, Co1, int8=False):
     B, Ci, M = xc.shape
     rm = rowmat(xc)
     assert rm is not None and Ci == wc.Ci and 0 < Co1 < wc.Co
     z1, z2 = empty_act((B, Co1, M), xc.device), empty_act((B, wc.Co - Co1, M), xc.device)
-    _lib.call("fqss_qpw_fwd2", _p(xc), _p(wc.idx), _p(wc.dw), _p(wc.rw), _p(bias1), _p(bias2), _p(qmin_x), _p(qmax_x), _p(z1), _p(z2),
+    fn, wa = _wsel("fqss_qpw_fwd2", wc.idx, wc.img, int8)
+    _lib.call(fn, _p(xc), _p(wa), _p(wc.dw), _p(wc.rw), _p(bias1), _p(bias2), _p(qmin_x), _p(qmax_x), _p(z1), _p(z2),
               B, Ci, Co1, wc.Co - Co1, M, rm[2], rowmat(z1)[2], rowmat(z2)[2], _stream())
     return z1, z2
 
 
-def qpw_fwdq(xc, wc, bias1, bias2, qmin_x, qmax_x, Co1, act, slope, r1, r2=None, stats=None, adds=None):
+def qpw_fwdq(xc, wc, bias1, bias2, qmin_x, qmax_x, Co1, act, slope, r1, r2=None, stats=None, adds=None, int8=False):
     B, Ci, M = xc.shape
     rm = rowmat(xc)
     Co2 = wc.Co - Co1
@@ -454,11 +484,21 @@
             r = _lib.FqssAddAfter()
             r.a, r.ld_a, r.amin, r.amax, r.qmin, r.qmax, r.y, r.ld_y = _p(ac), rowmat(ac)[2], _p(amin), _p(amax), _p(qmin), _p(qmax), _p(sc), rowmat(sc)[2]
             sums.append(sc); recs.append(r)
-        _lib.call("fqss_qpw_fwdq_add", _p(xc), _p(wc.idx), _p(wc.dw), _p(wc.rw), _p(bias1), _p(bias2), _p(qmin_x), _p(qmax_x), _p(z1), _p(z2),
+        fn, wa = _wsel("fqss_qpw_fwdq_add", wc.idx, wc.img, int8)
+        _lib.call(fn, _p(xc), _p(wa), _p(wc.dw), _p(wc.rw), _p(bias1), _p(bias2), _p(qmin_x), _p(qmax_x), _p(z1), _p(z2),
                   _p(r1[0]), _p(r1[1]), _p(r2[0]) if r2 else None, _p(r2[1]) if r2 else None, _p(yc1), _p(yc2),
                   B, Ci, Co1, Co2, M, rm[2], rowmat(z1)[2], rowmat(z2)[2] if Co2 else 0, rowmat(yc1)[2], rowmat(yc2)[2] if Co2 else 0,
                   _ref(recs[0]) if recs[0] is not None else None, _ref(recs[1]) if recs[1] is not None else None, _stream())
         return ((z1, z2, yc1, yc2) if Co2 else (z1, yc1)) + (tuple(sums),)
+    if wc.img is not None and not int8:
+        st = None
+        if stats is not None and not Co2:
+            assert stats.nslots == stat_slots("qpw", Co1, M) and stats.ws.numel() >= B * stats.nslots * 2
+            st = _p(stats.ws)
+        _lib.call("fqss_qpw_fwdq_img", _p(xc), _p(wc.img), _p(wc.dw), _p(wc.rw), _p(bias1), _p(bias2), _p(qmin_x), _p(qmax_x), _p(z1), _p(z2),
+                  int(act), _p(slope), _p(r1[0]), _p(r1[1]), _p(r2[0]) if r2 else None, _p(r2[1]) if r2 else None, _p(yc1), _p(yc2),
+                  B, Ci, Co1, Co2, M, rm[2], rowmat(z1)[2], rowmat(z2)[2] if Co2 else 0, rowmat(yc1)[2], rowmat(yc2)[2] if Co2 else 0, st, _stream())
+        return (z1, z2, yc1, yc2) if Co2 else (z1, yc1)
     w = _lib.FqssWCodes()
     w.idx, w.idxT, w.dw, w.rw, w.Co, w.Ci = _p(wc.idx), _p(wc.idxT), _p(wc.dw), _p(wc.rw), wc.Co, wc.Ci
     dx, dz1, dz2, dy1, dy2 = _desc(xc), _desc(z1), _desc(z2), _desc(yc1), _desc(yc2)
@@ -470,14 +510,15 @@
     return (z1, z2, yc1, yc2) if Co2 else (z1, yc1)
 
 
-def qpw_bwd_x2(gz1, gz2, wc):
+def qpw_bwd_x2(gz1, gz2, wc, int8=False):
     gz1, ld1 = _aligned_grad(gz1)
     gz2, ld2 = _aligned_grad(gz2)
     B, Co1, M = gz1.shape
     Co2 = gz2.shape[1]
     assert Co1 + Co2 == wc.Co and gz2.shape[0] == B and gz2.shape[2] == M
     gx = empty_act((B, wc.Ci, M), gz1.device)
-    _lib.call("fqss_qpw_bwd_x2", _p(gz1), _p(gz2), _p(wc.idxT), _p(wc.dw), _p(gx), B, wc.Ci, Co1, Co2, M, ld1, ld2, rowmat(gx)[2], _stream())
+    fn, wa = _wsel("fqss_qpw_bwd_x2", wc.idxT, wc.imgT, int8)
+    _lib.call(fn, _p(gz1), _p(gz2), _p(wa), _p(wc.dw), _p(gx), B, wc.Ci, Co1, Co2, M, ld1, ld2, rowmat(gx)[2], _stream())
     return gx
 
 
diff --git a/fqss_amd/runtime.py b/fqss_amd/runtime.py
--- a/fqss_amd/runtime.py
+++ b/fqss_amd/runtime.py
@@ -261,6 +261,7 @@
         self.gwq = torch.zeros(n_gwq, device=dev)
         self.wq_store = torch.empty(n_gwq, device=dev)
         rows, off, blk = [], 0, 0
+        img_rows = []
         self.weights = []
         self.pairs = []
         pending = None
@@ -280,6 +281,7 @@
             fr = (not pw) and axis == 0 and w.dim() in (3, 4) and shape[0] % 16 == 0 and shape[0] <= 1024
             wc = None
             ldT = C
+            img_row = [0, 0, 0]
             if pw and id(w) in partner:
                 w2 = partner[id(w)]
                 Co1, Co2, Ci = shape[0], w2.shape[0], shape[1]
@@ -289,6 +291,7 @@
                 pc.idxT = torch.empty(Ci, Co1 + Co2, device=dev, dtype=torch.int8)
                 pc.dw = torch.empty(Co1 + Co2, device=dev)
                 pc.rw = torch.empty(Co1 + Co2, device=dev)
+                pc.img, pc.imgT = K.new_wimg(Co1 + Co2, Ci, dev), K.new_wimg(Ci, Co1 + Co2, dev)
                 pair = _LinearPair()
                 pair.wc, pair.Co1 = pc, Co1
                 pair.gw = self.gwq[off:off + w.numel() + w2.numel()].view(Co1 + Co2, Ci)
@@ -304,6 +307,7 @@
                 wc.dw, wc.rw = pc.dw[r0:r0 + shape[0]], pc.rw[r0:r0 + shape[0]]
                 ldT = pc.Co
                 idxT_ptr = pc.idxT.data_ptr() + r0
+                img_row = [pc.img.data_ptr(), pc.imgT.data_ptr(), r0]
                 if wq_first is not wq:
                     pair.partner = wq
                     wq_first._fqss_pair = pair
@@ -317,11 +321,15 @@
                 wc.dw = torch.empty(shape[0], device=dev)
                 wc.rw = torch.empty(shape[0], device=dev)
                 idxT_ptr = wc.idxT.data_ptr()
+                if pw and w.dim() == 3:
+                    wc.img, wc.imgT = K.new_wimg(wc.Co, wc.Ci, dev), K.new_wimg(wc.Ci, wc.Co, dev)
+                    img_row = [wc.img.data_ptr(), wc.imgT.data_ptr(), 0]
             coded = pw or fr
             rows.append([w.data_ptr(), wq.data_ptr(), wc.idx.data_ptr() if coded else 0, idxT_ptr if coded else 0,
                          wc.dw.data_ptr() if coded else 0, wc.rw.data_ptr() if coded else 0, wqm.min_range.data_ptr(),
                          wqm.max_range.data_ptr(), gwq.data_ptr(), w.grad.data_ptr(), wqm.min_range.grad.data_ptr(),
                          wqm.max_range.grad.data_ptr(), outer, C, inner, blk, ldT, int(wqm.n_bits)])
+            img_rows.append(img_row)
             wq._fqss_gwq = gwq
             if pw:
                 wq._fqss_wcodes = wc
@@ -334,6 +342,7 @@
         assert pending is None
         K.wq_table_check(rows)
         self.wq_table = torch.tensor(rows, dtype=torch.int64, device=dev)
+        self.wq_img_table = torch.tensor(img_rows, dtype=torch.int64, device=dev).reshape(-1, 3) if any(r[0] for r in img_rows) else None
         self.total_channels = blk
         self.det = None
         grouped = os.environ.get("FQSS_GROUP_WGRAD", "1") != "0"
@@ -359,7 +368,7 @@
             assert sum(t[2].shape[0] for t in self.seg_tables) == len(flush_rows), "an activation quantizer belongs to no backward segment"
 
     def weights_forward(self):
-        K.wq_multi_fwd(self.wq_table, self.total_channels)
+        K.wq_multi_fwd(self.wq_table, self.total_channels, self.wq_img_table)
         if self.wgrad_queue is not None:
             self.wgrad_queue.jobs = []
         if self.row_wgrad_queue is not None:
diff --git a/include/fqss.h b/include/fqss.h
--- a/include/fqss.h
+++ b/include/fqss.h
@@ -82,6 +82,7 @@
 int fqss_gacc_flush_multi(const int64_t* table, int n, fqss_stream_t stream);
 int fqss_wq_multi_fwd(const int64_t* table, int n, int total_channels, fqss_stream_t stream);
 int fqss_wq_multi_bwd(const int64_t* table, int n, int total_channels, fqss_stream_t stream);
+int fqss_wq_multi_fwd_img(const int64_t* table, const int64_t* img_table, int n, int total_channels, fqss_stream_t stream);
 
 int fqss_pwconv_fwd(const float* x, const float* w, const float* bias, float* z, int B, int Ci,
                     int Co, int M, int64_t ld_x, int64_t ld_z, fqss_stream_t stream);
@@ -118,6 +119,8 @@
                   const float* qmin, const float* qmax, fqss_stream_t stream);
 int fqss_wq_codes_bits(const float* w, int8_t* idx, int8_t* idxT, float* dw, float* rw, int Co, int Ci,
                        const float* qmin, const float* qmax, int n_bits, fqss_stream_t stream);
+int fqss_wq_codes_img(const float* w, int8_t* idx, int8_t* idxT, uint16_t* img, uint16_t* imgT, float* dw, float* rw, int Co, int Ci,
+                      const float* qmin, const float* qmax, int n_bits, fqss_stream_t stream);
 int fqss_qpw_fwd(const uint8_t* xc, const int8_t* wi, const float* dw, const float* rw,
                  const float* bias, const float* qmin_x, const float* qmax_x, float* z, int B, int Ci,
                  int Co, int M, int64_t ld_xc, int64_t ld_z, fqss_stream_t stream);
@@ -167,6 +170,29 @@
                       const float* qmax1, const float* qmin2, const float* qmax2, uint8_t* yc1, uint8_t* yc2, int B, int Ci,
                       int Co1, int Co2, int M, int64_t ld_xc, int64_t ld_z1, int64_t ld_z2, int64_t ld_yc1, int64_t ld_yc2,
                       const FqssAddAfter* add1, const FqssAddAfter* add2, fqss_stream_t stream);
+
+int fqss_qpw_fwd_img(const uint8_t* xc, const uint16_t* wimg, const float* dw, const float* rw, const float* bias,
+                     const float* qmin_x, const float* qmax_x, float* z, int B, int Ci, int Co, int M, int64_t ld_xc, int64_t ld_z,
+                     fqss_stream_t stream);
+int fqss_qpw_fwd2_img(const uint8_t* xc, const uint16_t* wimg, const float* dw, const float* rw, const float* bias1,
+                      const float* bias2, const float* qmin_x, const float* qmax_x, float* z1, float* z2, int B, int Ci, int Co1,
+                      int Co2, int M, int64_t ld_xc, int64_t ld_z1, int64_t ld_z2, fqss_stream_t stream);
+int fqss_qpw_fwdq_img(const uint8_t* xc, const uint16_t* wimg, const float* dw, const float* rw, const float* bias1,
+                      const float* bias2, const float* qmin_x, const float* qmax_x, float* z1, float* z2, int act, const float* slope,
+                      const float* qmin1, const float* qmax1, const float* qmin2, const float* qmax2, uint8_t* yc1, uint8_t* yc2, int B,
+                      int Ci, int Co1, int Co2, int M, int64_t ld_xc, int64_t ld_z1, int64_t ld_z2, int64_t ld_yc1, int64_t ld_yc2,
+                      int64_t* stats1, fqss_stream_t stream);
+int fqss_qpw_fwdq_add_img(const uint8_t* xc, const uint16_t* wimg, const float* dw, const float* rw, const float* bias1,
+                          const float* bias2, const float* qmin_x, const float* qmax_x, float* z1, float* z2, const float* qmin1,
+                          const float* qmax1, const float* qmin2, const float* qmax2, uint8_t* yc1, uint8_t* yc2, int B, int Ci,
+                          int Co1, int Co2, int M, int64_t ld_xc, int64_t ld_z1, int64_t ld_z2, int64_t ld_yc1, int64_t ld_yc2,
+                          const FqssAddAfter* add1, const FqssAddAfter* add2, fqss_stream_t stream);
+int fqss_qpw_bwd_x_img(const float* gz, const uint16_t* wimgT, const float* dw, float* gx, int B, int Ci, int Co, int M, int64_t ld_gz,
+                       int64_t ld_gx, fqss_stream_t stream);
+int fqss_qpw_bwd_x_add_img(const float* gz, const uint16_t* wimgT, const float* dw, const float* addend, float* gx, int B, int Ci,
+                           int Co, int M, int64_t ld_gz, int64_t ld_add, int64_t ld_gx, fqss_stream_t stream);
+int fqss_qpw_bwd_x2_img(const float* gz1, const float* gz2, const uint16_t* wimgT, const float* dw, float* gx, int B, int Ci, int Co1,
+                        int Co2, int M, int64_t ld_gz1, int64_t ld_gz2, int64_t ld_gx, fqss_stream_t stream);
 
 int fqss_dwconv_fwd(const float* x, const float* w, const float* bias, float* z, int B, int C,
                     int M, int K, int dil, int pad, int64_t ld_x, int64_t ld_z, fqss_stream_t stream);
```

Result: no change. 626.5 samples/s (-0.3%).
